# JunkyByte/easy_ViTPose

Hardware: AMD Instinct MI355X
Metric: persons_per_sec (higher is better)
Workload: dtype fp16; 1 GPU; ViTPose-B coco K=17, batch 256 x 256x192 crops per GPU (f32 input resident in HBM) -> (y,x,conf) keypoints in HBM; global_batch=256, weights=seeded random init (no checkpoint offline)

## Files before the change

easy_vitpose_amd/_capi.py:

```python
from __future__ import annotations

import ctypes as C
import os

LIB_PATH = os.path.join(os.path.dirname(os.path.abspath(__file__)), '_lib', 'libvitpose_hip.so')

VP_OK, VP_ERR_INVALID, VP_ERR_HIP, VP_ERR_STATE, VP_ERR_MISSING_TENSOR, VP_ERR_SHAPE = range(6)
VP_DTYPE_F16, VP_DTYPE_BF16, VP_DTYPE_FP8 = 0, 1, 2
VP_INPUT_F32_NCHW, VP_INPUT_U8_NHWC = 0, 1
VP_PROF_NAMES = ['gemm_proj', 'gemm_fc1', 'gemm_qkv', 'gemm_patch', 'gemm_deconv', 'gemm_final',
                 'attention', 'layernorm', 'im2col', 'decode', 'gemm_fc2']
VP_PROF_COUNT = len(VP_PROF_NAMES)
DTYPES = {'fp16': VP_DTYPE_F16, 'f16': VP_DTYPE_F16, 'bf16': VP_DTYPE_BF16, 'fp8': VP_DTYPE_FP8}

SYMBOLS = ['vp_abi_version', 'vp_create', 'vp_load_weights', 'vp_infer', 'vp_infer_device', 'vp_infer_device_stream', 'vp_host_alloc', 'vp_host_free',
           'vp_infer_submit', 'vp_infer_wait', 'vp_group_create', 'vp_group_size', 'vp_group_member', 'vp_group_load_weights', 'vp_group_infer',
           'vp_group_infer_allgather', 'vp_group_destroy', 'vp_group_last_error', 'vp_infer_frame', 'vp_infer_flip', 'vp_infer_heatmaps',
           'vp_infer_tokens', 'vp_decode_only', 'vp_stream', 'vp_synchronize', 'vp_set_profiling',
           'vp_reset_profile', 'vp_get_profile', 'vp_profile_kernel', 'vp_group_peer_access_missing', 'vp_destroy', 'vp_last_error',
           'vp_dbg_gemm', 'vp_dbg_attention', 'vp_dbg_layernorm', 'vp_dbg_deconv', 'vp_dbg_gemm_case', 'vp_dbg_crop_prep',
           'vp_dbg_group_plan', 'vp_dbg_group_trace', 'vp_dbg_gemm8_pick', 'vp_dbg_gemm2_pick', 'vp_dbg_splitk_pick', 'vp_dbg_run_batch', 'vp_dbg_fp8_gemm', 'vp_dbg_mx_gemm', 'vp_dbg_host_e4m3', 'vp_dbg_gemm_fp8_case', 'vp_dbg_qkvattn',
           'vp_expert_info', 'vp_set_expert', 'vp_infer_experts', 'vp_dbg_expert_tile', 'vp_infer_frames', 'vp_dbg_frame_plan',
           'vp_dbg_chunk_plan', 'vp_infer_boxes_stream', 'vp_dbg_box_geometry',
           'vp_set_flip_test', 'vp_clear_flip_test', 'vp_flip_test_enabled', 'vp_group_set_flip_test', 'vp_group_clear_flip_test',
           'vp_dbg_flip_partner', 'vp_dbg_flip_layout', 'vp_dbg_decode_flip',
           'vp_infer_experts_device_stream', 'vp_infer_frames_experts', 'vp_infer_boxes_experts_stream', 'vp_dbg_mix_plan', 'vp_dbg_decode_mix',
           'vp_set_flip_test_experts', 'vp_dbg_mix_plan_flip', 'vp_dbg_decode_flip_mix']


class HipExtensionMissing(RuntimeError):
    pass


class VpError(RuntimeError):
    def __init__(self, code: int, msg: str):
        super().__init__(f'[vitpose_hip status {code}] {msg}')
        self.code = code
        self.msg = msg


class vp_config(C.Structure):
    _fields_ = [('embed_dim', C.c_int32), ('depth', C.c_int32), ('num_heads', C.c_int32),
                ('num_keypoints', C.c_int32), ('dtype', C.c_int32), ('device_id', C.c_int32),
                ('max_batch', C.c_int32)]


class vp_tensor_desc(C.Structure):
    _fields_ = [('name', C.c_char_p), ('data', C.POINTER(C.c_float)), ('numel', C.c_int64)]


class vp_frame(C.Structure):
    _fields_ = [('data', C.c_void_p), ('h', C.c_int32), ('w', C.c_int32)]


class vp_profile(C.Structure):
    _fields_ = [('ms', C.c_double * VP_PROF_COUNT), ('flops', C.c_double * VP_PROF_COUNT),
                ('bytes', C.c_double * VP_PROF_COUNT), ('launches', C.c_int64 * VP_PROF_COUNT)]


_lib = None


def load_library():
    global _lib
    if _lib is not None:
        return _lib
    lib_path = os.environ.get('VP_HIP_LIB', LIB_PATH)
    if not os.path.exists(lib_path):
        raise HipExtensionMissing(
            f'{lib_path} not found. Build it with `python -m easy_vitpose_amd.build` '
            '(needs hipcc). There is no CPU fallback for the ViTPose path.')
    try:
        lib = C.CDLL(lib_path)
    except OSError as e:
        raise HipExtensionMissing(f'cannot load {lib_path}: {e}') from e
    H = C.c_void_p
    lib.vp_abi_version.restype = C.c_int
    lib.vp_create.argtypes = [C.POINTER(H), C.POINTER(vp_config)]
    lib.vp_load_weights.argtypes = [H, C.POINTER(vp_tensor_desc), C.c_int32]
    lib.vp_infer.argtypes = [H, C.c_void_p, C.c_int32, C.c_int32, C.c_void_p, C.c_void_p]
    lib.vp_infer_device.argtypes = [H, C.c_void_p, C.c_int32, C.c_int32, C.c_void_p, C.c_void_p, C.c_int32]
    lib.vp_infer_device_stream.argtypes = [H, C.c_void_p, C.c_int32, C.c_int32, C.c_void_p, C.c_void_p, C.c_void_p]
    lib.vp_host_alloc.argtypes = [C.c_size_t]
    lib.vp_host_alloc.restype = C.c_void_p
    lib.vp_host_free.argtypes = [C.c_void_p]
    lib.vp_host_free.restype = None
    lib.vp_infer_submit.argtypes = [H, C.c_void_p, C.c_int32, C.c_int32, C.c_void_p, C.c_void_p, C.POINTER(C.c_int32)]
    lib.vp_infer_wait.argtypes = [H, C.c_int32]
    lib.vp_group_create.argtypes = [C.POINTER(H), C.POINTER(vp_config), C.POINTER(C.c_int32), C.c_int32]
    lib.vp_group_size.argtypes = [H]
    lib.vp_group_member.argtypes = [H, C.c_int32]
    lib.vp_group_member.restype = C.c_void_p
    lib.vp_group_load_weights.argtypes = [H, C.POINTER(vp_tensor_desc), C.c_int32]
    lib.vp_group_infer.argtypes = [H, C.c_void_p, C.c_int32, C.c_int32, C.c_void_p, C.c_void_p]
    lib.vp_group_infer_allgather.argtypes = [H, C.c_void_p, C.c_int32, C.c_int32, C.c_void_p, C.POINTER(C.c_void_p), C.c_void_p]
    lib.vp_group_destroy.argtypes = [H]
    lib.vp_group_last_error.argtypes = [H]
    lib.vp_group_last_error.restype = C.c_char_p
    lib.vp_infer_frame.argtypes = [H, C.c_void_p, C.c_int32, C.c_int32, C.c_void_p, C.c_int32, C.c_void_p]
    lib.vp_infer_frames.argtypes = [H, C.POINTER(vp_frame), C.c_int32, C.c_int32, C.c_void_p, C.c_int32, C.c_void_p]
    lib.vp_dbg_frame_plan.argtypes = [C.POINTER(vp_frame), C.c_int32, C.c_void_p, C.c_int32, C.c_void_p]
    lib.vp_infer_boxes_stream.argtypes = [H, C.POINTER(vp_frame), C.c_int32, C.c_void_p, C.c_int32, C.c_void_p, C.c_int32, C.c_int32,
                                          C.c_void_p, C.c_void_p, C.c_void_p, C.c_void_p]
    lib.vp_dbg_box_geometry.argtypes = [C.c_void_p, C.c_int32, C.c_void_p, C.c_void_p, C.c_int32, C.c_int32, C.c_int32, C.c_void_p, C.c_void_p]
    lib.vp_dbg_crop_prep.argtypes = [C.c_int32, C.c_void_p, C.c_int32, C.c_int32, C.c_void_p, C.c_int32, C.c_void_p]
    lib.vp_infer_heatmaps.argtypes = [H, C.c_void_p, C.c_int32, C.c_int32, C.c_void_p]
    lib.vp_infer_tokens.argtypes = [H, C.c_void_p, C.c_int32, C.c_int32, C.c_void_p]
    lib.vp_decode_only.argtypes = [C.c_int32, C.c_void_p, C.c_int32, C.c_int32, C.c_void_p, C.c_void_p]
    lib.vp_stream.argtypes = [H]
    lib.vp_stream.restype = C.c_void_p
    lib.vp_synchronize.argtypes = [H]
    lib.vp_set_profiling.argtypes = [H, C.c_int32]
    lib.vp_reset_profile.argtypes = [H]
    lib.vp_get_profile.argtypes = [H, C.POINTER(vp_profile)]
    lib.vp_destroy.argtypes = [H]
    lib.vp_last_error.argtypes = [H]
    lib.vp_last_error.restype = C.c_char_p
    lib.vp_dbg_gemm.argtypes = [C.c_int32] * 6 + [C.c_void_p] * 5
    lib.vp_dbg_attention.argtypes = [C.c_int32] * 5 + [C.c_void_p] * 2
    lib.vp_dbg_layernorm.argtypes = [C.c_int32] * 4 + [C.c_void_p] * 5
    lib.vp_dbg_deconv.argtypes = [C.c_int32] * 6 + [C.c_void_p, C.POINTER(vp_tensor_desc), C.c_int32, C.c_void_p]
    lib.vp_infer_flip.argtypes = [C.c_void_p, C.c_void_p, C.c_int32, C.c_int32, C.c_void_p, C.c_void_p, C.c_int32, C.c_int32,
                                  C.c_void_p, C.c_void_p]
    lib.vp_dbg_gemm_case.argtypes = [C.c_int32] * 9 + [C.c_void_p] * 8
    if hasattr(lib, 'vp_dbg_gemm8_timeline'):
        lib.vp_dbg_gemm8_timeline.argtypes = [C.c_int32] * 9 + [C.POINTER(C.c_uint64), C.c_int32]
        lib.vp_dbg_gemm_timeline.argtypes = [C.c_int32] * 6 + [C.POINTER(C.c_uint64), C.c_int32]
        lib.vp_dbg_gemm8_timeline.restype = lib.vp_dbg_gemm_timeline.restype = C.c_int
        lib.vp_dbg_gemm_bench.argtypes = [C.c_int32] * 9 + [C.POINTER(C.c_float)]
        lib.vp_dbg_gemm_bench2.argtypes = [C.c_int32] * 10 + [C.POINTER(C.c_float)]
        lib.vp_dbg_gemm_compare.argtypes = [C.c_int32] * 13 + [C.POINTER(C.c_uint64), C.POINTER(C.c_double)]
        lib.vp_dbg_peak.argtypes = [C.c_int32, C.c_int32, C.POINTER(C.c_double)]
        for n_ in ('vp_dbg_gemm_bench', 'vp_dbg_gemm_bench2', 'vp_dbg_gemm_compare', 'vp_dbg_peak'):
            getattr(lib, n_).restype = C.c_int
    lib.vp_profile_kernel.argtypes = [H, C.c_int32, C.c_char_p, C.c_int32]
    lib.vp_group_peer_access_missing.argtypes = [H]
    lib.vp_dbg_group_plan.argtypes = [C.c_int32] * 3 + [C.c_void_p, C.c_void_p, C.c_int32]
    lib.vp_dbg_gemm8_pick.argtypes = [C.c_int32] * 4 + [C.c_void_p]
    lib.vp_dbg_gemm2_pick.argtypes = [C.c_int32] * 4 + [C.c_void_p]
    lib.vp_dbg_splitk_pick.argtypes = [C.c_int32] * 3 + [C.c_void_p]
    lib.vp_dbg_run_batch.argtypes = [C.c_int32] * 3
    lib.vp_dbg_group_trace.argtypes = [C.c_int32] * 3 + [C.c_void_p, C.c_int32]
    lib.vp_dbg_fp8_gemm.argtypes = [C.c_int32] * 4 + [C.c_void_p] * 7
    lib.vp_dbg_mx_gemm.argtypes = [C.c_int32] * 4 + [C.c_void_p] * 7
    lib.vp_dbg_host_e4m3.argtypes = [C.c_void_p, C.c_void_p, C.c_int64]
    lib.vp_dbg_gemm_fp8_case.argtypes = [C.c_int32] * 5 + [C.c_void_p] * 8
    lib.vp_expert_info.argtypes = [H, C.c_void_p, C.c_void_p, C.c_void_p]
    lib.vp_set_expert.argtypes = [H, C.c_int32]
    lib.vp_infer_experts.argtypes = [H, C.c_void_p, C.c_int32, C.c_int32, C.c_void_p, C.c_void_p, C.c_void_p]
    lib.vp_dbg_expert_tile.argtypes = [C.c_int32] * 4 + [C.c_void_p, C.c_int32]
    lib.vp_infer_experts_device_stream.argtypes = [H, C.c_void_p, C.c_int32, C.c_int32, C.c_void_p, C.c_void_p, C.c_void_p, C.c_void_p]
    lib.vp_infer_frames_experts.argtypes = [H, C.POINTER(vp_frame), C.c_int32, C.c_int32, C.c_void_p, C.c_int32, C.c_void_p, C.c_void_p]
    lib.vp_infer_boxes_experts_stream.argtypes = [H, C.POINTER(vp_frame), C.c_int32, C.c_void_p, C.c_int32, C.c_void_p, C.c_int32, C.c_int32,
                                                  C.c_void_p, C.c_void_p, C.c_void_p, C.c_void_p, C.c_void_p]
    lib.vp_dbg_mix_plan.argtypes = [C.c_void_p, C.c_int32, C.c_int32, C.c_int32] + [C.c_void_p] * 6
    lib.vp_dbg_decode_mix.argtypes = [C.c_int32, C.c_void_p, C.c_int32, C.c_int32, C.c_int32, C.c_void_p, C.c_void_p, C.c_void_p]
    lib.vp_dbg_chunk_plan.argtypes = [C.POINTER(vp_config), C.c_int32, C.c_void_p, C.c_int32]
    lib.vp_dbg_qkvattn.argtypes = [C.c_int32] * 5 + [C.c_void_p] * 4
    lib.vp_set_flip_test.argtypes = [H, C.c_void_p, C.c_int32, C.c_int32]
    lib.vp_clear_flip_test.argtypes = [H]
    lib.vp_flip_test_enabled.argtypes = [H]
    lib.vp_group_set_flip_test.argtypes = [H, C.c_void_p, C.c_int32, C.c_int32]
    lib.vp_group_clear_flip_test.argtypes = [H]
    lib.vp_set_flip_test_experts.argtypes = [H, C.c_void_p, C.c_void_p, C.c_int32]
    lib.vp_dbg_mix_plan_flip.argtypes = [C.c_void_p, C.c_int32, C.c_int32, C.c_int32] + [C.c_void_p] * 6
    lib.vp_dbg_decode_flip_mix.argtypes = [C.c_int32, C.c_void_p, C.c_int32, C.c_int32, C.c_int32, C.c_void_p, C.c_void_p, C.c_int32, C.c_int32, C.c_void_p, C.c_void_p]
    lib.vp_dbg_flip_partner.argtypes = [C.c_int32, C.c_void_p, C.c_int32, C.c_void_p]
    lib.vp_dbg_flip_layout.argtypes = [C.c_int32, C.c_int32, C.c_void_p, C.c_void_p]
    lib.vp_dbg_decode_flip.argtypes = [C.c_int32, C.c_void_p, C.c_int32, C.c_int32, C.c_void_p, C.c_int32, C.c_int32, C.c_void_p, C.c_void_p]
    for name in SYMBOLS:
        if name not in ('vp_stream', 'vp_last_error', 'vp_host_alloc', 'vp_host_free', 'vp_group_member', 'vp_group_last_error'):
            getattr(lib, name).restype = C.c_int
    _lib = lib
    return lib


def last_error(handle=None) -> str:
    lib = load_library()
    s = lib.vp_last_error(handle)
    return s.decode('utf-8', 'replace') if s else ''


def check(code: int, handle=None):
    if code != VP_OK:
        raise VpError(code, last_error(handle))
```

easy_vitpose_amd/csrc/api_internal.h:

```cpp
#pragma once
#include <hip/hip_runtime.h>

#include <algorithm>
#include <cmath>
#include <cstdio>
#include <cstdlib>
#include <cstring>
#include <string>
#include <unordered_map>
#include <vector>

#include "../../include/vitpose_hip.h"
#ifdef VP_TOOLS
#include "../../include/vitpose_hip_tools.h"
#endif
#include "kernels.h"
#include "mx8.h"

namespace vpi {

struct Block {
    float *ln1_g, *ln1_b, *ln2_g, *ln2_b;
    uint16_t *w_qkv, *w_proj, *w_fc1, *w_fc2;
    float *b_qkv, *b_proj, *b_fc1, *b_fc2;
    float *s_qkv, *s_fc1;
    uint16_t* w_qkvh = nullptr;
    float *b_qkvh = nullptr, *s_qkvh = nullptr;
    uint8_t *w_qkv8 = nullptr, *w_fc18 = nullptr, *w_fc28 = nullptr, *w_proj8 = nullptr;
    float *ws_qkv = nullptr, *ws_fc1 = nullptr, *ws_fc2 = nullptr, *ws_proj = nullptr;
};

struct Switches {
    int g8_stagger = 0;
    int gemm8_mask = 0x7;
    long g8_min_tiles = 448;
    bool persist_gemm = true;
    int order_mask = 8;
    bool blocked_hid = true;
    bool blocked_qkv = true;
    bool fuse_ln = true;
    bool fuse_qkv_attn = true;
    bool qa_min_set = false;
    long qa_min_tiles = 108;
    long qa80_min_tiles = 192;
    int qa80_group = 8;
    int attn_qsplit = 128;
    int g8_bm192 = 3;
    bool pad_batch = true;
    bool g8_cost_model = true;
    bool deconv_parity_fast = true;
    bool fuse_head = true;
    bool fp8_proj16 = false;
    int graph_max_n = 16;
    bool graph_null = true;
    int caller_stream_max_n = 16;
    bool fold_rule = true;
    int graph_max_n_stats = 8;
    bool splitk_on = true;
    int splitk_force[2][2] = {{0, 0}, {0, 0}};
    int gemm_variant[VP_PROF_COUNT] = {-1, -1, -1, -1, -1, -1, -1, -1, -1, -1, -1};
    int gemm_group_m[VP_PROF_COUNT] = {0};
    int fam_ablate[VP_PROF_COUNT] = {0};
};

}

namespace vpi {
struct MixPlan {
    int nb = 0;
    std::vector<int32_t> order, ids;
    std::vector<int> seg_e, seg_s;
    uint64_t pattern = 0;
};
}

struct vp_ctx {
    vp_config cfg;
    vpi::Switches sw;
    int D, L, heads, Kp, dtype, maxb;
    hipStream_t stream = nullptr;
    std::string err;
    bool loaded = false;
    std::vector<void*> allocs;
    uint16_t* w_patch = nullptr;
    float* pos = nullptr;
    std::vector<vpi::Block> blocks;
    float *lnf_g = nullptr, *lnf_b = nullptr;
    uint16_t *w_d1 = nullptr, *w_d2 = nullptr, *w_fin = nullptr;
    size_t fin_rows = 0;
    float *b_d1 = nullptr, *b_d2 = nullptr, *b_fin = nullptr, *b_zero = nullptr;
    uint16_t* zero = nullptr;
    void* in_stage = nullptr;
    int32_t* wh_stage = nullptr;
    float* x = nullptr;
    uint16_t *y = nullptr, *qkv = nullptr, *hid = nullptr, *d1 = nullptr, *d2 = nullptr;
    float *hm = nullptr, *kp = nullptr, *tok = nullptr;
    float* hm_keep = nullptr;
    int32_t* partner = nullptr;
    bool flip_on = false;
    int flip_shift = 0;
    uint32_t flip_gen = 0, flip_counter = 0;
    int32_t* flip_table = nullptr;
    std::vector<int32_t> flip_pairs;
    bool flip_ex = false;
    int32_t* flip_tables = nullptr;
    float *ln_part = nullptr, *rowstat = nullptr;
    bool fp8 = false;
    size_t Mp = 0;
    uint8_t *x8 = nullptr, *xs8 = nullptr, *hs8 = nullptr;
    uint8_t *y8 = nullptr, *ys8 = nullptr;
    struct Slot {
        void* in = nullptr; int32_t* wh = nullptr; float* kp = nullptr; hipEvent_t h2d = nullptr, done = nullptr, out = nullptr; bool busy = false;
        float* host_kp = nullptr; float* user_out = nullptr; size_t out_bytes = 0;
        char* host_in = nullptr; size_t host_in_cap = 0;
    };
    Slot slots[2];
    hipStream_t copy_stream = nullptr;
    hipStream_t d2h_stream = nullptr;
    int next_slot = 0;
    struct GraphKey {
        int n = 0, fmt = -1;
        const void* src = nullptr; const int32_t* wh = nullptr; float* out = nullptr;
        int expert = 0;
        const int32_t* post = nullptr;
        uint32_t flip = 0;
        uint64_t mix = 0;
        bool wide = false;
        bool operator==(const GraphKey& o) const {
            return n == o.n && fmt == o.fmt && src == o.src && wh == o.wh && out == o.out && expert == o.expert && post == o.post && flip == o.flip &&
                   mix == o.mix && wide == o.wide;
        }
    };
    struct GraphEntry { GraphKey key; hipGraphExec_t exec = nullptr; bool no_graph = false; };
    GraphEntry graphs[4];
    int graph_victim = 0;
    float* splitk_ws = nullptr;
    size_t splitk_rows = 0;
    hipEvent_t ev_in = nullptr, ev_out = nullptr;
    hipStream_t own_stream = nullptr;
    const void* last_stream_id = nullptr;
    bool foreign_pending = false;
    hipEvent_t ev_sw = nullptr;
    uint8_t* frame_stage = nullptr;
    size_t frame_cap = 0;
    vp::CropRec* crecs = nullptr;
    int32_t* box_aux = nullptr;
    struct Head { uint16_t *w_d1 = nullptr, *w_d2 = nullptr, *w_fin = nullptr; float *b_d1 = nullptr, *b_d2 = nullptr, *b_fin = nullptr; size_t fin_rows = 0; int K = 0; };
    int Kmax = 0;
    int n_experts = 0, part_features = 0, expert = 0;
    size_t fc2_w_stride = 0, fc2_b_stride = 0;
    std::vector<Head> ex_heads;
    int32_t* expert_ids = nullptr;
    void* mix_stage = nullptr;
    size_t mix_stage_cap = 0;
    const int32_t* mix_expert = nullptr;
    std::vector<int> mix_bounds;
    int32_t* mix_slot = nullptr;
    vp::MixRec* mix_recs = nullptr;
    vp::MixRecFlip* mix_recs_flip = nullptr;
    const vpi::MixPlan* mix = nullptr;
    vpi::MixPlan mix_host;
    std::vector<int32_t> mix_ks, mix_first, mix_k;
    uint32_t prof = 0;
    int gemm_ablate = 0;
    struct Ev { hipEvent_t a, b; int fam; double flops, bytes; };
    std::vector<Ev> evs;
    std::vector<std::pair<hipEvent_t, hipEvent_t>> ev_pool;
    vp_profile acc{};
    std::string kernel_desc[VP_PROF_COUNT];
};

namespace vpi {

extern thread_local std::string g_create_error;

int fail(vp_ctx* c, int code, const std::string& msg);
int need_weights(vp_ctx* c);
bool slots_busy(const vp_ctx* c);
int slots_idle(vp_ctx* c, const char* who);
int quiesce(vp_ctx* c);
inline size_t crop_bytes(int fmt) { return (size_t)3 * 256 * 192 * (fmt == VP_INPUT_F32_NCHW ? 4 : 1); }

#define HIPCHK(c, expr)                                                                         \
    do {                                                                                        \
        hipError_t e__ = (expr);                                                                \
        if (e__ != hipSuccess)                                                                  \
            return fail((c), VP_ERR_HIP, std::string(#expr) + ": " + hipGetErrorString(e__));   \
    } while (0)

template <class T> int dalloc(vp_ctx* c, T** p, size_t count) {
    void* q = nullptr;
    HIPCHK(c, hipMalloc(&q, count * sizeof(T) + 256));
    c->allocs.push_back(q);
    *p = (T*)q;
    return VP_OK;
}

uint16_t host_to_bits(float v, int dtype);
float host_from_bits(uint16_t h, int dtype);
size_t pad128(size_t n);
int upload_f32(vp_ctx* c, float** dst, const float* src, size_t n, size_t npad = 0);
int upload_mat(vp_ctx* c, uint16_t** dst, const float* src, size_t rows, size_t cols, size_t rows_pad);
int upload_final(vp_ctx* c, uint16_t** dst, const float* src, size_t kp, size_t cols, size_t* rows_phys);
int upload_ln_folded(vp_ctx* c, uint16_t** w_out, float** s_out, float** c_out, const float* W, const float* b,
                     const float* gamma, const float* beta, size_t N, size_t K);
int upload_fp8_rows(vp_ctx* c, uint8_t** w_out, float** ws_out, float** c_out, const float* W, const float* b, const float* gamma,
                    const float* beta, size_t N, size_t K);

struct Lookup {
    std::unordered_map<std::string, const vp_tensor_desc*> map;
    vp_ctx* c;
    int get(const std::string& name, int64_t numel, const float** out) {
        auto it = map.find(name);
        if (it == map.end()) return fail(c, VP_ERR_MISSING_TENSOR, "missing key in state dict: " + name);
        if (it->second->numel != numel || it->second->data == nullptr)
            return fail(c, VP_ERR_SHAPE, "size mismatch for " + name + ": expected " + std::to_string(numel) +
                                             " elements, got " + std::to_string(it->second->numel));
        *out = it->second->data;
        return VP_OK;
    }
    bool has(const std::string& name) const { return map.count(name) != 0; }
    int64_t numel(const std::string& name) const { auto it = map.find(name); return it == map.end() ? -1 : it->second->numel; }
};

size_t final_rows(size_t kp);
int pack_deconv(vp_ctx* c, Lookup& lk, int idx, int Cin, uint16_t** w_out, float** b_out, const std::string& head = "keypoint_head");
void use_expert(vp_ctx* c, int e);

int flip_partner_table(int K, const int32_t* pairs, int n_pairs, int32_t* partner, std::string* why);
inline const int32_t* flip_table_now(const vp_ctx* c) { return c->flip_ex ? c->flip_tables + (size_t)c->expert * c->Kmax : c->flip_table; }
bool prof_begin(vp_ctx* c, int fam, double flops, double bytes);
void prof_end(vp_ctx* c, bool on);
void prof_collect(vp_ctx* c);
void read_switches(Switches& s);
void apply_gemm_tuning(Switches& s);

int frame_plan(const vp_frame* frames, int n_frames, const int32_t* p9, int n, int32_t* bands, std::string* why);
int stage_frames(vp_ctx* c, const vp_frame* frames, int n_frames, bool on_device, const int32_t* p9, int n, const int32_t* bands,
                 std::vector<vp::CropRec>& recs);
int box_args(int n_frames, const int32_t* frame_hw, int hw_stride, int row_stride, int n, int pad, std::string* why);
constexpr uint64_t MIX_NO_GRAPH = ~(uint64_t)0;
int mix_check_ids(const int32_t* ids, int n, int n_experts, std::string* why);
void mix_plan(const int32_t* ids, int nb, int n_experts, MixPlan& p);
uint64_t mix_pattern(const std::vector<int>& seg_e, const std::vector<int>& seg_s, int n_experts);
void mix_records(const MixPlan& p, const int32_t* k_per_expert, int Kmax, int32_t* first, int32_t* K);
void mix_records_flip(const MixPlan& p, const int32_t* k_per_expert, int Kmax, int32_t* first, int32_t* K);
int submit_impl(vp_ctx* c, const void* crops, int32_t fmt, int32_t n, const int32_t* org_wh, float* out, int32_t* slot_out, bool stage_out);

#define LAUNCH(c, fam, flops, bytes, expr)   \
    do {                                     \
        const bool on__ = prof_begin((c), (fam), (flops), (bytes)); \
        hipError_t e__ = (expr);             \
        prof_end((c), on__);                 \
        if (e__ != hipSuccess)               \
            return fail((c), VP_ERR_HIP, std::string(#expr) + ": " + hipGetErrorString(e__)); \
    } while (0)

struct LnFuse {
    bool a_blocked = false, out_blocked = false, reverse = false;
    size_t plane = 0;
    float* stats_out = nullptr;
    const float* rowstat = nullptr;
    const float* ln_s = nullptr;
    const float* ln_part = nullptr;
    int ln_tiles = 0;
    int* tiles_out = nullptr;
};

constexpr int SPLITK_MAX_S = 8, SPLITK_MAX_CROPS = 32;
struct GemmPick { int variant = -1, group_m = 0, persist = 0, stagger = 0, splitk = 1, splitk_variant = 0; };
GemmPick resolve_gemm(const Switches& s, int fam, int epi, int M, int N, int K, bool ln_part = false, size_t splitk_rows = 0,
                      const std::vector<int>* mix_bounds = nullptr);
GemmPick resolve_gemm_fp8(int fam, int epi, int Mp, int N);
enum QkvPath { QKV_GEMM = 0, QKV_ATTN64 = 1, QKV_ATTN80 = 2 };
struct HeadPlan {
    bool fused = false;
    GemmPick deconv1, deconv2, final;
};
struct ChunkPlan {
    int n = 0;
    bool fold1 = false, fold2 = false;
    int qkv_path = QKV_GEMM;
    bool attn_qsplit = false;
    bool proj_fp8 = false;
    GemmPick gemm[VP_PROF_COUNT];
    HeadPlan head;
};
ChunkPlan plan_chunk(const Switches& s, int D, int heads, int max_batch, bool fp8, int n_in, size_t fin_rows, const std::vector<int>* mix_bounds = nullptr);
HeadPlan plan_head(const Switches& s, int D, int nh, size_t fin_rows);

int gemm(vp_ctx* c, int fam, int epi, const GemmPick& pk, const uint16_t* A, const uint16_t* W, const float* bias, void* out,
         const float* aux, int M, int N, int K, int ldo, int Hin = 0, int Win = 0, int Cin = 0, const LnFuse* ln = nullptr);
int gemm_fp8(vp_ctx* c, int fam, int epi, const GemmPick& pk, const uint8_t* A8, const uint8_t* a_scales, const uint8_t* W8, const float* w_scale, const float* bias,
             void* out, uint8_t* out_scales, const float* aux, int M, int N, int K, const LnFuse* ln);
struct FwdOpts {
    bool tokens = false;
    bool mirror = false;
    bool head = true;
    int twin_src = 0;
};
int forward_chunk(vp_ctx* c, const void* d_crops, int fmt, int n_in, const FwdOpts& o = FwdOpts());
int head_chunk(vp_ctx* c, const uint16_t* y, int nh, float* hm, const HeadPlan& hp);
int decode_chunk(vp_ctx* c, const int32_t* d_wh, float* d_out, int n, bool twin);
int chunk_cap(const vp_ctx* c);
int chunk_rows(const vp_ctx* c, int nb);
int forward_mode_chunk(vp_ctx* c, const void* d_src, int fmt, int nb);
int run_chunk(vp_ctx* c, const void* d_src, int fmt, int nb, const int32_t* d_wh, float* d_out, const int32_t* post = nullptr);

}
```

easy_vitpose_amd/csrc/debug_taps.hip:

```cpp
#include "dbg_util.h"

using namespace vpi;


extern "C" {

VP_API int vp_dbg_gemm(int32_t device, int32_t dtype, int32_t epi, int32_t M, int32_t N, int32_t K, const float* A,
                       const float* W, const float* bias, const float* aux, float* out) {
    if (epi < 0 || epi > 3 || M <= 0 || N <= 0 || K <= 0 || K % 64) return fail(nullptr, VP_ERR_INVALID, "bad gemm test shape");
    vp_ctx* c = dbg_ctx(device, dtype);
    if (!c) return VP_ERR_HIP;
    uint16_t *dA, *dW, *dO16 = nullptr;
    float *dB, *dAux = nullptr, *dO32 = nullptr;
    int rc;
    const size_t MN = (size_t)M * N;
    if ((rc = upload_mat(c, &dA, A, M, K, M))) return dbg_finish(c, rc);
    if ((rc = upload_mat(c, &dW, W, N, K, pad128(N)))) return dbg_finish(c, rc);
    if ((rc = upload_f32(c, &dB, bias, N, pad128(N)))) return dbg_finish(c, rc);
    if (epi >= 2) {
        if ((rc = upload_f32(c, &dAux, aux, epi == 2 ? MN : (size_t)192 * N))) return dbg_finish(c, rc);
        if ((rc = dalloc(c, &dO32, MN))) return dbg_finish(c, rc);
    } else if ((rc = dalloc(c, &dO16, MN))) return dbg_finish(c, rc);
    if ((rc = dalloc(c, &c->zero, (size_t)256))) return dbg_finish(c, rc);
    rc = gemm(c, 0, epi, resolve_gemm(c->sw, 0, epi, M, N, K), dA, dW, dB, epi >= 2 ? (void*)dO32 : (void*)dO16, dAux, M, N, K, N);
    if (!rc && hipDeviceSynchronize() != hipSuccess) rc = fail(c, VP_ERR_HIP, "gemm kernel failed");
    if (!rc) {
        if (epi >= 2) { if (hipMemcpy(out, dO32, MN * 4, hipMemcpyDeviceToHost) != hipSuccess) rc = fail(c, VP_ERR_HIP, "D2H"); }
        else rc = download16(c, dO16, out, MN);
    }
    return dbg_finish(c, rc);
}

VP_API int vp_dbg_attention(int32_t device, int32_t dtype, int32_t B, int32_t D, int32_t heads, const float* qkv, float* out) {
    vp_ctx* c = dbg_ctx(device, dtype);
    if (!c) return VP_ERR_HIP;
    uint16_t *dq, *dout;
    int rc;
    const size_t M = (size_t)B * 192;
    if ((rc = upload_mat(c, &dq, qkv, M, 3 * (size_t)D, M))) return dbg_finish(c, rc);
    if ((rc = dalloc(c, &dout, M * D))) return dbg_finish(c, rc);
    const char* qs = getenv("VP_ATTN_QSPLIT");
    hipError_t e = vp::attention_launch(c->dtype, dq, dout, B, D, heads, nullptr, (long)B * heads <= (qs ? atol(qs) : Switches{}.attn_qsplit));
    if (e == hipSuccess) e = hipDeviceSynchronize();
    if (e != hipSuccess) return dbg_finish(c, fail(c, VP_ERR_HIP, std::string("attention: ") + hipGetErrorString(e)));
    return dbg_finish(c, download16(c, dout, out, M * D));
}

VP_API int vp_dbg_qkvattn(int32_t device, int32_t dtype, int32_t npairs, int32_t D, int32_t heads, const float* x, const float* W, const float* bias, float* out) {
    if (npairs <= 0 || D <= 0 || heads <= 0 || !x || !W || !bias || !out) return fail(nullptr, VP_ERR_INVALID, "bad qkvattn test shape");
    vp_ctx* c = dbg_ctx(device, dtype);
    if (!c) return VP_ERR_HIP;
    const size_t M = (size_t)npairs * 384;
    uint16_t *dx, *dw, *dwh, *dy;
    float *db, *dbh, *ds, *dsh, *drow;
    int rc;
    std::vector<float> zeros(3 * (size_t)D, 0.f), row(2 * M);
    for (size_t m = 0; m < M; ++m) { row[2 * m] = 0.f; row[2 * m + 1] = 1.f; }
    if ((rc = upload_mat(c, &dx, x, M, D, M)) || (rc = upload_mat(c, &dw, W, 3 * (size_t)D, D, pad128(3 * (size_t)D))) || (rc = upload_f32(c, &db, bias, 3 * (size_t)D)) ||
        (rc = upload_f32(c, &ds, zeros.data(), 3 * (size_t)D)) || (rc = upload_f32(c, &drow, row.data(), 2 * M)) || (rc = dalloc(c, &dwh, 3 * (size_t)D * D)) ||
        (rc = dalloc(c, &dbh, 3 * (size_t)D)) || (rc = dalloc(c, &dsh, 3 * (size_t)D)) || (rc = dalloc(c, &dy, M * D)))
        return dbg_finish(c, rc);
    if (heads * 80 == D) {
        uint16_t* dwh80; float *dbh80, *dsh80;
        const size_t rows = (size_t)heads * 256;
        if ((rc = dalloc(c, &dwh80, rows * D)) || (rc = dalloc(c, &dbh80, rows)) || (rc = dalloc(c, &dsh80, rows))) return dbg_finish(c, rc);
        hipError_t e8 = vp::qkv_head_major80_launch(dw, db, ds, dwh80, dbh80, dsh80, D, D, heads, nullptr);
        vp::GemmArgs g80{};
        g80.A = dx; g80.W = dwh80; g80.bias = dbh80; g80.ln_s = dsh80; g80.rowstat = drow; g80.out = dy;
        g80.M = (int)M; g80.N = heads * 256; g80.K = D; g80.ldo = D; g80.w_rows = heads * 256; g80.variant = 18;
        g80.attn_scale_log2e = (1.0f / sqrtf(80.0f)) * 1.4426950408889634f;
        if (e8 == hipSuccess && !vp::gemm8_supported(vp::EPI_QKV_ATTN, g80, 256, 192)) return dbg_finish(c, fail(c, VP_ERR_INVALID, "shape not supported by the fused qkv + attention tile (head dim 80)"));
        if (e8 == hipSuccess) e8 = vp::gemm_launch(c->dtype, vp::EPI_QKV_ATTN, g80, nullptr);
        if (e8 == hipSuccess) e8 = hipDeviceSynchronize();
        if (e8 != hipSuccess) return dbg_finish(c, fail(c, VP_ERR_HIP, std::string("qkvattn (head dim 80): ") + hipGetErrorString(e8)));
        return dbg_finish(c, download16(c, dy, out, M * D));
    }
    hipError_t e = vp::qkv_head_major_launch(dw, db, ds, dwh, dbh, dsh, D, D, nullptr);
    vp::QkvAttnArgs qa{};
    qa.x_hi = dx; qa.wh = dwh; qa.bh = dbh; qa.sh = dsh; qa.rowstat = drow; qa.y = dy; qa.npairs = npairs; qa.ncrops = 2 * npairs; qa.heads = heads; qa.D = D;
    const float scale = 1.0f / sqrtf(64.0f);
    qa.scale_log2e = scale * 1.4426950408889634f;
    if (e == hipSuccess && !vp::qkvattn_supported(qa)) return dbg_finish(c, fail(c, VP_ERR_INVALID, "shape not supported by the fused qkv + attention kernel"));
    if (e == hipSuccess) e = vp::qkvattn_launch(c->dtype, qa, nullptr, nullptr, 0);
    if (e == hipSuccess) e = hipDeviceSynchronize();
    if (e != hipSuccess) return dbg_finish(c, fail(c, VP_ERR_HIP, std::string("qkvattn: ") + hipGetErrorString(e)));
    return dbg_finish(c, download16(c, dy, out, M * D));
}

VP_API int vp_dbg_layernorm(int32_t device, int32_t dtype, int32_t M, int32_t D, const float* x, const float* gamma,
                            const float* beta, float* out16, float* out32) {
    vp_ctx* c = dbg_ctx(device, dtype);
    if (!c) return VP_ERR_HIP;
    float *dx, *dg, *db, *d32;
    uint16_t* d16;
    int rc;
    const size_t MD = (size_t)M * D;
    if ((rc = upload_f32(c, &dx, x, MD)) || (rc = upload_f32(c, &dg, gamma, D)) || (rc = upload_f32(c, &db, beta, D)) ||
        (rc = dalloc(c, &d32, MD)) || (rc = dalloc(c, &d16, MD))) return dbg_finish(c, rc);
    hipError_t e = vp::layernorm_launch(c->dtype, dx, dg, db, d16, d32, M, D, nullptr);
    if (e == hipSuccess) e = hipDeviceSynchronize();
    if (e == hipSuccess) e = hipMemcpy(out32, d32, MD * 4, hipMemcpyDeviceToHost);
    if (e != hipSuccess) return dbg_finish(c, fail(c, VP_ERR_HIP, std::string("layernorm: ") + hipGetErrorString(e)));
    return dbg_finish(c, download16(c, d16, out16, MD));
}

VP_API int vp_dbg_deconv(int32_t device, int32_t dtype, int32_t B, int32_t Hin, int32_t Win, int32_t Cin, const float* x,
                         const vp_tensor_desc* tensors, int32_t n_tensors, float* out) {
    vp_ctx* c = dbg_ctx(device, dtype);
    if (!c) return VP_ERR_HIP;
    Lookup lk;
    lk.c = c;
    for (int i = 0; i < n_tensors; ++i) lk.map[tensors[i].name] = &tensors[i];
    uint16_t *dx, *dw, *dout;
    float* db;
    int rc;
    const size_t Min = (size_t)B * Hin * Win;
    if ((rc = pack_deconv(c, lk, 0, Cin, &dw, &db))) return dbg_finish(c, rc);
    if ((rc = upload_mat(c, &dx, x, Min, Cin, Min))) return dbg_finish(c, rc);
    if ((rc = dalloc(c, &dout, Min * 4 * 256))) return dbg_finish(c, rc);
    if ((rc = dalloc(c, &c->zero, (size_t)256))) return dbg_finish(c, rc);
    if (hipMemset(c->zero, 0, 512) != hipSuccess) return dbg_finish(c, fail(c, VP_ERR_HIP, "memset"));
    rc = gemm(c, 0, vp::EPI_DECONV, resolve_gemm(c->sw, 0, vp::EPI_DECONV, (int)Min, 256, 4 * Cin), dx, dw, db, dout, nullptr, (int)Min, 256, 4 * Cin, 256, Hin, Win, Cin);
    if (!rc && hipDeviceSynchronize() != hipSuccess) rc = fail(c, VP_ERR_HIP, "deconv kernel failed");
    if (!rc) rc = download16(c, dout, out, Min * 4 * 256);
    return dbg_finish(c, rc);
}


VP_API int vp_dbg_gemm_case(int32_t device, int32_t dtype, int32_t epi, int32_t variant, int32_t group_m, int32_t flags, int32_t M,
                            int32_t N, int32_t K, const float* A, const float* W, const float* bias, const float* aux, const float* rowstat,
                            const float* ln_s, float* out, float* stats) {
    if (M <= 0 || N <= 0 || K <= 0 || K % 64 || !A || !W || !bias || !out) return fail(nullptr, VP_ERR_INVALID, "bad gemm case");
    vp_ctx* c = dbg_ctx(device, dtype);
    if (!c) return VP_ERR_HIP;
    c->Kp = N;
    int r;
    const size_t MN = (size_t)M * N, wrows = pad128(N);
    const bool ablk = (flags & 4) != 0, oblk = (flags & 2) != 0;
    uint16_t *dA, *dW;
    float *dB, *dAux32 = nullptr, *dRow = nullptr, *dS = nullptr, *dStats = nullptr;
    uint16_t* dAux16 = nullptr;
    void* dOut = nullptr;
    {
        std::vector<uint16_t> ha((size_t)M * K);
        for (size_t m = 0; m < (size_t)M; ++m)
            for (size_t k = 0; k < (size_t)K; ++k) {
                const size_t dst = ablk ? ((((m >> 6) * (K >> 6) + (k >> 6)) << 12) + ((m & 63) << 6) + (k & 63)) : m * K + k;
                ha[dst] = host_to_bits(A[m * K + k], c->dtype);
            }
        if ((r = dalloc(c, &dA, (size_t)M * K))) return dbg_finish(c, r);
        if (hipMemcpy(dA, ha.data(), ha.size() * 2, hipMemcpyHostToDevice) != hipSuccess) return dbg_finish(c, fail(c, VP_ERR_HIP, "H2D"));
    }
    size_t fin_rows = 0;
    if (epi == vp::EPI_HEATMAP) { if ((r = upload_final(c, &dW, W, N, K, &fin_rows))) return dbg_finish(c, r); }
    else if ((r = upload_mat(c, &dW, W, N, K, wrows))) return dbg_finish(c, r);
    if ((r = upload_f32(c, &dB, bias, N, wrows)) || (r = dalloc(c, &c->zero, (size_t)256))) return dbg_finish(c, r);
    vp::GemmArgs g{};
    g.A = dA; g.W = dW; g.bias = dB; g.M = M; g.N = N; g.K = K; g.ldo = N; g.zero = c->zero; g.Kp = N;
    g.w_rows = (int)wrows; g.variant = variant; g.group_m = group_m;
    g.persist = (flags & 1) != 0; g.out_blocked = oblk; g.a_blocked = ablk; g.reverse = (flags & 8) != 0;
    if (rowstat && ln_s) {
        if ((r = upload_f32(c, &dRow, rowstat, (size_t)M * 2)) || (r = upload_f32(c, &dS, ln_s, N, wrows))) return dbg_finish(c, r);
        g.rowstat = dRow; g.ln_s = dS;
    }
    size_t out_bytes = 0;
    const bool prod = epi == vp::EPI_BIAS_RESID_LN || epi == vp::EPI_POS_LN;
    if (epi == vp::EPI_BIAS || epi == vp::EPI_BIAS_GELU) out_bytes = MN * 2;
    else if (epi == vp::EPI_BIAS_RESID || epi == vp::EPI_POS || prod) out_bytes = MN * 4;
    else if (epi == vp::EPI_HEATMAP) { out_bytes = MN * 4; g.N = (int)fin_rows; g.ldo = 0; g.w_rows = (int)pad128(fin_rows); }
    else return dbg_finish(c, fail(c, VP_ERR_INVALID, "unsupported epilogue"));
    if (epi == vp::EPI_BIAS_RESID || epi == vp::EPI_POS || epi == vp::EPI_POS_LN) {
        if (!aux) return dbg_finish(c, fail(c, VP_ERR_INVALID, "aux required"));
        if ((r = upload_f32(c, &dAux32, aux, epi == vp::EPI_BIAS_RESID ? MN : (size_t)192 * N))) return dbg_finish(c, r);
        g.aux = dAux32;
    }
    if (epi == vp::EPI_BIAS_RESID_LN) {
        if (!aux) return dbg_finish(c, fail(c, VP_ERR_INVALID, "aux required"));
        std::vector<uint16_t> hp(2 * MN);
        for (size_t i = 0; i < MN; ++i) {
            const uint16_t hi = host_to_bits(aux[i], c->dtype);
            hp[i] = hi;
            hp[MN + i] = host_to_bits(aux[i] - host_from_bits(hi, c->dtype), c->dtype);
        }
        if ((r = dalloc(c, &dAux16, 2 * MN))) return dbg_finish(c, r);
        if (hipMemcpy(dAux16, hp.data(), hp.size() * 2, hipMemcpyHostToDevice) != hipSuccess) return dbg_finish(c, fail(c, VP_ERR_HIP, "H2D"));
        g.aux = (const float*)dAux16;
    }
    if (prod) {
        g.plane = MN;
        if ((r = dalloc(c, &dStats, (size_t)M * (N / 64) * 2))) return dbg_finish(c, r);
        g.stats_out = dStats;
    }
    char* o;
    if ((r = dalloc(c, &o, out_bytes))) return dbg_finish(c, r);
    dOut = o;
    hipMemset(dOut, 0xff, out_bytes);
    g.out = dOut;
    const int splitk = (flags >> 8) & 15;
    hipError_t e;
    if (splitk > 1) {
        if (epi != vp::EPI_BIAS_RESID_LN) return dbg_finish(c, fail(c, VP_ERR_INVALID, "split-K is a residual-GEMM path (epi 6)"));
        float* ws = nullptr;
        if ((r = dalloc(c, &ws, (size_t)splitk * MN))) return dbg_finish(c, r);
        hipMemset(ws, 0xff, (size_t)splitk * MN * 4);
        vp::GemmArgs p = g;
        p.out = ws; p.aux = nullptr; p.bias = nullptr; p.stats_out = nullptr; p.plane = 0; p.splitk = splitk; p.persist = 0;
        e = vp::gemm_launch(c->dtype, vp::EPI_PARTIAL, p, nullptr);
        if (e == hipSuccess) e = vp::splitk_reduce_launch(c->dtype, ws, splitk, dB, dAux16, MN, dStats, M, N, nullptr);
        dOut = dAux16;
    } else {
        e = vp::gemm_launch(c->dtype, epi, g, nullptr);
    }
    if (e == hipSuccess) e = hipDeviceSynchronize();
    if (e != hipSuccess) return dbg_finish(c, fail(c, VP_ERR_HIP, std::string("gemm case: ") + hipGetErrorString(e)));
    if (epi == vp::EPI_BIAS || epi == vp::EPI_BIAS_GELU) {
        std::vector<float> t(MN);
        if ((r = download16(c, (const uint16_t*)dOut, t.data(), MN))) return dbg_finish(c, r);
        for (size_t m = 0; m < (size_t)M; ++m)
            for (size_t n = 0; n < (size_t)N; ++n) {
                const size_t src = oblk ? ((((m >> 6) * ((size_t)N >> 6) + (n >> 6)) << 12) + ((m & 63) << 6) + (n & 63)) : m * N + n;
                out[m * N + n] = t[src];
            }
    } else if (prod) {
        std::vector<float> hi(MN), lo(MN);
        if ((r = download16(c, (const uint16_t*)dOut, hi.data(), MN)) || (r = download16(c, (const uint16_t*)dOut + MN, lo.data(), MN))) return dbg_finish(c, r);
        for (size_t i = 0; i < MN; ++i) out[i] = hi[i] + lo[i];
        if (stats && hipMemcpy(stats, dStats, (size_t)M * (N / 64) * 8, hipMemcpyDeviceToHost) != hipSuccess) return dbg_finish(c, fail(c, VP_ERR_HIP, "D2H"));
    } else {
        if (hipMemcpy(out, dOut, out_bytes, hipMemcpyDeviceToHost) != hipSuccess) return dbg_finish(c, fail(c, VP_ERR_HIP, "D2H"));
    }
    return dbg_finish(c, VP_OK);
}

VP_API int vp_dbg_crop_prep(int32_t device, const uint8_t* frame, int32_t fh, int32_t fw, const int32_t* crop_params, int32_t n, uint8_t* out) {
    if (!frame || !crop_params || !out || n <= 0 || fh <= 0 || fw <= 0) return fail(nullptr, VP_ERR_INVALID, "bad argument");
    const vp_frame fr{frame, fh, fw};
    std::vector<int32_t> p9((size_t)n * 9, 0);
    for (int i = 0; i < n; ++i) std::memcpy(&p9[9 * (size_t)i + 1], crop_params + 8 * (size_t)i, 32);
// ... 145 lines not shown
```

easy_vitpose_amd/csrc/forward.hip:

```cpp
#include "api_internal.h"
#include "tiles.h"

using namespace vpi;

namespace vpi {

static void note_kernel(vp_ctx* c, int fam, const char* desc) {
    if (desc[0] && c->kernel_desc[fam] != desc) c->kernel_desc[fam] = desc;
}

int gemm(vp_ctx* c, int fam, int epi, const GemmPick& pk, const uint16_t* A, const uint16_t* W, const float* bias, void* out,
         const float* aux, int M, int N, int K, int ldo, int Hin, int Win, int Cin, const LnFuse* ln) {
    vp::GemmArgs g{};
    g.A = A; g.W = W; g.bias = bias; g.out = out; g.aux = aux;
    g.M = M; g.N = N; g.K = K; g.ldo = ldo;
    g.Hin = Hin; g.Win = Win; g.Cin = Cin; g.zero = c->zero; g.Kp = c->Kp;
    g.w_rows = (int)pad128((size_t)N);
    g.variant = pk.variant; g.group_m = pk.group_m; g.persist = pk.persist; g.stagger = pk.stagger;
    g.ablate = c->gemm_ablate | c->sw.fam_ablate[fam];
    g.parity_fast = c->sw.deconv_parity_fast;
    if (c->mix_expert && fam == VP_PROF_GEMM_FC2) g.expert = c->mix_expert;
    if (ln) {
        g.a_blocked = ln->a_blocked; g.out_blocked = ln->out_blocked; g.reverse = ln->reverse;
        g.plane = ln->plane; g.stats_out = ln->stats_out; g.rowstat = ln->rowstat; g.ln_s = ln->ln_s;
        g.ln_part = ln->ln_part; g.ln_tiles = ln->ln_tiles; g.ln_inv_d = 1.0f / (float)K;
        if (ln->tiles_out) *ln->tiles_out = N / 64;
    }
    if (epi == vp::EPI_DECONV_FINAL) { g.W2 = c->w_fin; g.bias2 = c->b_fin; g.out2 = (float*)out; g.out = nullptr; }
    const bool deconv = epi == vp::EPI_DECONV || epi == vp::EPI_DECONV_FINAL;
    const double par = deconv ? 4.0 : 1.0;
    const double Nalg = (epi == vp::EPI_HEATMAP) ? (double)c->Kp : (double)N;
    double flops = 2.0 * M * Nalg * K * par;
    const bool resid = epi == vp::EPI_BIAS_RESID || epi == vp::EPI_BIAS_RESID_LN;
    const bool f32out = resid || epi == vp::EPI_POS || epi == vp::EPI_POS_LN || epi == vp::EPI_HEATMAP;
    const double out_b = f32out ? 4.0 : 2.0;
    double bytes = 2.0 * M * (double)(deconv ? Cin : K) + 2.0 * N * (double)K * par + out_b * M * Nalg * par;
    if (epi == vp::EPI_DECONV_FINAL) {
        flops += 2.0 * M * par * (double)c->Kp * N;
        bytes += (4.0 * c->Kp - out_b * N) * M * par + 2.0 * c->fin_rows * N;
    }
    if (resid) bytes += 4.0 * M * (double)N;
    if (epi == vp::EPI_BIAS_RESID_LN || epi == vp::EPI_POS_LN) bytes += 8.0 * M * (double)(N / 64);
    char desc[192];
    desc[0] = 0;
    g.desc = desc; g.desc_cap = (int)sizeof(desc);
    if (pk.splitk > 1) {
        if (out != (void*)aux || (size_t)M > c->splitk_rows || !c->splitk_ws) return fail(c, VP_ERR_INVALID, "split-K: a residual GEMM in place within the workspace only");
        vp::GemmArgs p = g;
        p.out = c->splitk_ws; p.aux = nullptr; p.bias = nullptr; p.stats_out = nullptr; p.plane = 0;
        p.variant = pk.splitk_variant; p.group_m = 0; p.splitk = pk.splitk; p.ldo = N; p.persist = 0;
        LAUNCH(c, fam, flops, bytes, vp::gemm_launch(c->dtype, vp::EPI_PARTIAL, p, c->stream));
        if (desc[0]) {
            char d2[224];
            snprintf(d2, sizeof(d2), "%s x split-K %d + splitk_reduce_kernel", desc, pk.splitk);
            note_kernel(c, fam, d2);
        }
        LAUNCH(c, fam, 0.0, 0.0, vp::splitk_reduce_launch(c->dtype, c->splitk_ws, pk.splitk, bias, (uint16_t*)out, g.plane, g.stats_out, M, N, c->stream));
        return VP_OK;
    }
    LAUNCH(c, fam, flops, bytes, vp::gemm_launch(c->dtype, epi, g, c->stream));
    note_kernel(c, fam, desc);
    return VP_OK;
}

int gemm_fp8(vp_ctx* c, int fam, int epi, const GemmPick& pk, const uint8_t* A8, const uint8_t* a_scales, const uint8_t* W8, const float* w_scale, const float* bias,
             void* out, uint8_t* out_scales, const float* aux, int M, int N, int K, const LnFuse* ln) {
    vp::GemmArgs g{};
    g.A = (const uint16_t*)A8; g.W = (const uint16_t*)W8; g.bias = bias; g.out = out; g.aux = aux;
    g.M = M; g.N = N; g.K = K; g.ldo = N;
    g.a_scales = a_scales; g.w_scale = w_scale; g.out_scales = out_scales;
    g.w_rows = (int)pad128((size_t)N);
    if (ln) {
        g.out_blocked = ln->out_blocked; g.reverse = ln->reverse;
        g.plane = ln->plane; g.stats_out = ln->stats_out;
        if (ln->tiles_out) *ln->tiles_out = N / 64;
    }
    const int bn = vp::tile8_bn(pk.variant);
    g.group_m = pk.group_m;
    if (!vp::gemm8f_supported(epi, g, bn))
        return fail(c, VP_ERR_SHAPE, "fp8 mode: GEMM shape " + std::to_string(M) + " x " + std::to_string(N) + " x " + std::to_string(K) + " not supported by the MXFP8 kernel");
    const double flops = 2.0 * M * (double)N * K;
    double bytes = 1.0 * M * (double)K + M * (double)(K / 32) + 1.0 * N * (double)K;
    bytes += epi == vp::EPI_BIAS ? 2.0 * M * (double)N : epi == vp::EPI_BIAS_GELU ? (1.0 + 1.0 / 32) * M * (double)N : 8.0 * M * (double)N + 8.0 * M * (double)(N / 64);
    char desc[192];
    desc[0] = 0;
    g.desc = desc; g.desc_cap = (int)sizeof(desc);
    LAUNCH(c, fam, flops, bytes, vp::gemm8f_launch(epi, g, bn, c->stream));
    note_kernel(c, fam, desc);
    return VP_OK;
}

static const uint16_t* fc2_w(const vp_ctx* c, const vpi::Block& b) { return c->mix_expert ? b.w_fc2 : b.w_fc2 + (size_t)c->expert * c->fc2_w_stride; }
static const float* fc2_b(const vp_ctx* c, const vpi::Block& b) { return c->mix_expert ? b.b_fc2 : b.b_fc2 + (size_t)c->expert * c->fc2_b_stride; }

int forward_chunk(vp_ctx* c, const void* d_crops, int fmt, int n_in, const FwdOpts& o) {
    const int D = c->D;
    const ChunkPlan pl = plan_chunk(c->sw, D, c->heads, c->maxb, c->fp8, n_in, c->fin_rows, c->mix_expert ? &c->mix_bounds : nullptr);
    const GemmPick* pk = pl.gemm;
    const int n = pl.n;
    const int M = n * 192;
    const double in_b = (fmt == VP_INPUT_F32_NCHW ? 4.0 : 1.0) * n_in * 3.0 * 256 * 192;
    if (o.twin_src) LAUNCH(c, VP_PROF_IM2COL, 0.0, 0.5 * in_b + 2.0 * M * 768, vp::im2col_twin_launch(c->dtype, d_crops, fmt, c->hid, n, o.twin_src, c->stream));
    else LAUNCH(c, VP_PROF_IM2COL, 0.0, in_b + 2.0 * M * 768, vp::im2col_launch(c->dtype, d_crops, fmt, c->hid, n, c->stream, o.mirror, n_in));
    int rc;
    size_t plane = 0;
    const bool qkv_blocked = c->sw.blocked_qkv && D / c->heads == 64;
    auto attention = [&](uint16_t* out, double bytes, uint8_t* mx_scales) -> int {
        LAUNCH(c, VP_PROF_ATTN, 4.0 * 192 * 192 * (double)D * n, bytes,
               vp::attention_launch(c->dtype, c->qkv, out, n, D, c->heads, c->stream, pl.attn_qsplit, qkv_blocked ? 1 : 0, mx_scales));
        return VP_OK;
    };
    if (c->fp8) {
        const int Mp = (int)std::max<size_t>((size_t)(M + 255) / 256 * 256, 512);
        plane = c->Mp * (size_t)D;
        uint16_t* xh = (uint16_t*)c->x;
        int tiles = 0;
        LnFuse prod; prod.plane = plane; prod.stats_out = c->ln_part; prod.tiles_out = &tiles;
        auto quant = [&]() -> int {
            LAUNCH(c, VP_PROF_LAYERNORM, 0.0, 8.0 * M * tiles + 2.0 * M * D + (1.0 + 1.0 / 32) * Mp * (double)D,
                   vp::ln_quant_launch(c->dtype, xh, c->ln_part, tiles, c->x8, c->xs8, M, Mp, D, c->stream));
            return VP_OK;
        };
        if ((rc = gemm(c, VP_PROF_GEMM_PATCH, vp::EPI_POS_LN, pk[VP_PROF_GEMM_PATCH], c->hid, c->w_patch, c->b_zero, c->x, c->pos, M, D, 768, D, 0, 0, 0, &prod))) return rc;
        for (int l = 0; l < c->L; ++l) {
            const Block& b = c->blocks[l];
            if ((rc = quant())) return rc;
            LnFuse cq; cq.out_blocked = qkv_blocked;
            if ((rc = gemm_fp8(c, VP_PROF_GEMM_QKV, vp::EPI_BIAS, pk[VP_PROF_GEMM_QKV], c->x8, c->xs8, b.w_qkv8, b.ws_qkv, b.b_qkv, c->qkv, nullptr, nullptr, Mp, 3 * D, D, &cq))) return rc;
            LnFuse pp = prod;
            if (pl.proj_fp8) {
                if ((rc = attention((uint16_t*)c->y8, 7.0 * M * D, c->ys8))) return rc;
                if ((rc = gemm_fp8(c, VP_PROF_GEMM_PROJ, vp::EPI_BIAS_RESID_LN, pk[VP_PROF_GEMM_PROJ], c->y8, c->ys8, b.w_proj8, b.ws_proj, b.b_proj, c->x, nullptr, c->x, Mp, D, D, &pp))) return rc;
            } else {
                if ((rc = attention(c->y, 8.0 * M * D, nullptr))) return rc;
                if ((rc = gemm(c, VP_PROF_GEMM_PROJ, vp::EPI_BIAS_RESID_LN, pk[VP_PROF_GEMM_PROJ], c->y, b.w_proj, b.b_proj, c->x, c->x, M, D, D, D, 0, 0, 0, &pp))) return rc;
            }
            if ((rc = quant())) return rc;
            if ((rc = gemm_fp8(c, VP_PROF_GEMM_FC1, vp::EPI_BIAS_GELU, pk[VP_PROF_GEMM_FC1], c->x8, c->xs8, b.w_fc18, b.ws_fc1, b.b_fc1, c->hid, c->hs8, nullptr, Mp, 4 * D, D, nullptr))) return rc;
            LnFuse p2 = prod;
            if ((rc = gemm_fp8(c, VP_PROF_GEMM_FC2, vp::EPI_BIAS_RESID_LN, pk[VP_PROF_GEMM_FC2], (const uint8_t*)c->hid, c->hs8, b.w_fc28, b.ws_fc2, b.b_fc2, c->x, nullptr, c->x, Mp, D, 4 * D, &p2))) return rc;
        }
    } else if (c->sw.fuse_ln) {
        plane = (size_t)M * D;
        uint16_t* xh = (uint16_t*)c->x;
        int tiles = 0;
        LnFuse prod; prod.plane = plane; prod.stats_out = c->ln_part; prod.tiles_out = &tiles;
        auto finalize = [&](bool folded) -> int {
            if (folded) return VP_OK;
            LAUNCH(c, VP_PROF_LAYERNORM, 0.0, 8.0 * M * tiles + 8.0 * M, vp::ln_finalize_launch(c->ln_part, c->rowstat, M, tiles, D, c->stream));
            return VP_OK;
        };
        const double qkv_attn_flops = 2.0 * M * 3.0 * D * D + 4.0 * 192 * 192 * (double)D * n, qkv_attn_bytes = 2.0 * M * D + 2.0 * 3 * D * (double)D + 2.0 * M * D;
        if ((rc = gemm(c, VP_PROF_GEMM_PATCH, vp::EPI_POS_LN, pk[VP_PROF_GEMM_PATCH], c->hid, c->w_patch, c->b_zero, c->x, c->pos, M, D, 768, D, 0, 0, 0, &prod))) return rc;
        if ((rc = finalize(pl.fold1))) return rc;
        for (int l = 0; l < c->L; ++l) {
            const Block& b = c->blocks[l];
            if (pl.qkv_path == QKV_ATTN80) {
                vp::GemmArgs g80{};
                g80.A = xh; g80.W = b.w_qkvh; g80.bias = b.b_qkvh; g80.ln_s = b.s_qkvh; g80.rowstat = c->rowstat; g80.out = c->y;
                g80.M = M; g80.N = c->heads * 256; g80.K = D; g80.ldo = D; g80.w_rows = c->heads * 256; g80.variant = 18;
                g80.group_m = c->sw.qa80_group;
                g80.attn_scale_log2e = (1.0f / sqrtf(80.0f)) * 1.4426950408889634f;
                g80.ablate = c->gemm_ablate | c->sw.fam_ablate[VP_PROF_GEMM_QKV];
                char desc[192];
                desc[0] = 0;
                g80.desc = desc; g80.desc_cap = (int)sizeof(desc);
                LAUNCH(c, VP_PROF_GEMM_QKV, qkv_attn_flops, qkv_attn_bytes, vp::gemm_launch(c->dtype, vp::EPI_QKV_ATTN, g80, c->stream));
                note_kernel(c, VP_PROF_GEMM_QKV, desc);
            } else if (pl.qkv_path == QKV_ATTN64) {
                vp::QkvAttnArgs qa{};
                qa.x_hi = xh; qa.wh = b.w_qkvh; qa.bh = b.b_qkvh; qa.sh = b.s_qkvh; qa.rowstat = c->rowstat; qa.y = c->y;
                qa.npairs = (n + 1) / 2; qa.ncrops = n; qa.heads = c->heads; qa.D = D;
                qa.scale_log2e = (1.0f / sqrtf(64.0f)) * 1.4426950408889634f;
                char desc[96];
                desc[0] = 0;
                LAUNCH(c, VP_PROF_GEMM_QKV, qkv_attn_flops, qkv_attn_bytes, vp::qkvattn_launch(c->dtype, qa, c->stream, desc, (int)sizeof(desc)));
                note_kernel(c, VP_PROF_GEMM_QKV, desc);
            } else {
                LnFuse cq; cq.rowstat = c->rowstat; cq.ln_s = b.s_qkv; cq.reverse = (c->sw.order_mask & 1) != 0; cq.out_blocked = qkv_blocked;
                if (pl.fold1) { cq.rowstat = nullptr; cq.ln_part = c->ln_part; cq.ln_tiles = D / 64; }
                if ((rc = gemm(c, VP_PROF_GEMM_QKV, vp::EPI_BIAS, pk[VP_PROF_GEMM_QKV], xh, b.w_qkv, b.b_qkv, c->qkv, nullptr, M, 3 * D, D, 3 * D, 0, 0, 0, &cq))) return rc;
                if ((rc = attention(c->y, 8.0 * M * D, nullptr))) return rc;
            }
            LnFuse pp = prod; pp.reverse = (c->sw.order_mask & 2) != 0;
            if ((rc = gemm(c, VP_PROF_GEMM_PROJ, vp::EPI_BIAS_RESID_LN, pk[VP_PROF_GEMM_PROJ], c->y, b.w_proj, b.b_proj, c->x, c->x, M, D, D, D, 0, 0, 0, &pp))) return rc;
            if ((rc = finalize(pl.fold2))) return rc;
            LnFuse c1; c1.rowstat = c->rowstat; c1.ln_s = b.s_fc1; c1.out_blocked = c->sw.blocked_hid; c1.reverse = (c->sw.order_mask & 4) != 0;
            if (pl.fold2) { c1.rowstat = nullptr; c1.ln_part = c->ln_part; c1.ln_tiles = D / 64; }
            if ((rc = gemm(c, VP_PROF_GEMM_FC1, vp::EPI_BIAS_GELU, pk[VP_PROF_GEMM_FC1], xh, b.w_fc1, b.b_fc1, c->hid, nullptr, M, 4 * D, D, 4 * D, 0, 0, 0, &c1))) return rc;
            LnFuse p2 = prod; p2.a_blocked = c->sw.blocked_hid; p2.reverse = (c->sw.order_mask & 8) != 0;
            if ((rc = gemm(c, VP_PROF_GEMM_FC2, vp::EPI_BIAS_RESID_LN, pk[VP_PROF_GEMM_FC2], c->hid, fc2_w(c, b), fc2_b(c, b), c->x, c->x, M, D, 4 * D, D, 0, 0, 0, &p2))) return rc;
            if (l + 1 < c->L && (rc = finalize(pl.fold1))) return rc;
        }
    } else {
    if ((rc = gemm(c, VP_PROF_GEMM_PATCH, vp::EPI_POS, pk[VP_PROF_GEMM_PATCH], c->hid, c->w_patch, c->b_zero, c->x, c->pos, M, D, 768, D))) return rc;
    for (int l = 0; l < c->L; ++l) {
        const Block& b = c->blocks[l];
        LAUNCH(c, VP_PROF_LAYERNORM, 0.0, 6.0 * M * D,
               vp::layernorm_launch(c->dtype, c->x, b.ln1_g, b.ln1_b, c->y, nullptr, M, D, c->stream));
        LnFuse q0; q0.out_blocked = qkv_blocked;
        if ((rc = gemm(c, VP_PROF_GEMM_QKV, vp::EPI_BIAS, pk[VP_PROF_GEMM_QKV], c->y, b.w_qkv, b.b_qkv, c->qkv, nullptr, M, 3 * D, D, 3 * D, 0, 0, 0, &q0))) return rc;
        if ((rc = attention(c->y, 8.0 * M * D, nullptr))) return rc;
        if ((rc = gemm(c, VP_PROF_GEMM_PROJ, vp::EPI_BIAS_RESID, pk[VP_PROF_GEMM_PROJ], c->y, b.w_proj, b.b_proj, c->x, c->x, M, D, D, D))) return rc;
        LAUNCH(c, VP_PROF_LAYERNORM, 0.0, 6.0 * M * D,
               vp::layernorm_launch(c->dtype, c->x, b.ln2_g, b.ln2_b, c->y, nullptr, M, D, c->stream));
        if ((rc = gemm(c, VP_PROF_GEMM_FC1, vp::EPI_BIAS_GELU, pk[VP_PROF_GEMM_FC1], c->y, b.w_fc1, b.b_fc1, c->hid, nullptr, M, 4 * D, D, 4 * D))) return rc;
        if ((rc = gemm(c, VP_PROF_GEMM_FC2, vp::EPI_BIAS_RESID, pk[VP_PROF_GEMM_FC2], c->hid, fc2_w(c, b), fc2_b(c, b), c->x, c->x, M, D, 4 * D, D))) return rc;
    }
    }
    const int nh = n_in, Mh = nh * 192;
    LAUNCH(c, VP_PROF_LAYERNORM, 0.0, 6.0 * Mh * D,
           vp::layernorm_launch(c->dtype, c->x, c->lnf_g, c->lnf_b, c->y, o.tokens ? c->tok : nullptr, Mh, D, c->stream, plane));
    return o.head ? head_chunk(c, c->y, nh, c->hm, pl.head) : VP_OK;
}

int head_chunk(vp_ctx* c, const uint16_t* y, int nh, float* hm, const HeadPlan& hp) {
    const int D = c->D;
    int rc;
    if ((rc = gemm(c, VP_PROF_GEMM_DECONV, vp::EPI_DECONV, hp.deconv1, y, c->w_d1, c->b_d1, c->d1, nullptr, nh * 192, 256, 4 * D, 256, 16, 12, D))) return rc;
    if (hp.fused) {
        return gemm(c, VP_PROF_GEMM_DECONV, vp::EPI_DECONV_FINAL, hp.deconv2, c->d1, c->w_d2, c->b_d2, hm, nullptr, nh * 768, 256, 1024, 256, 32, 24, 256);
    }
    if ((rc = gemm(c, VP_PROF_GEMM_DECONV, vp::EPI_DECONV, hp.deconv2, c->d1, c->w_d2, c->b_d2, c->d2, nullptr, nh * 768, 256, 1024, 256, 32, 24, 256))) return rc;
    if ((rc = gemm(c, VP_PROF_GEMM_FINAL, vp::EPI_HEATMAP, hp.final, c->d2, c->w_fin, c->b_fin, hm, nullptr, nh * 3072, (int)c->fin_rows, 256, 0))) return rc;
    return VP_OK;
}

int decode_chunk(vp_ctx* c, const int32_t* d_wh, float* d_out, int n, bool twin) {
    if (twin)
        LAUNCH(c, VP_PROF_DECODE, 0.0, 8.0 * n * c->Kp * 3072.0 + 12.0 * n * c->Kp,
               vp::decode_flip_launch(c->hm, flip_table_now(c), c->flip_shift, d_wh, d_out, n, c->Kp, c->stream));
    else
        LAUNCH(c, VP_PROF_DECODE, 0.0, 4.0 * n * c->Kp * 3072.0 + 12.0 * n * c->Kp,
               vp::decode_launch(c->hm, d_wh, d_out, n, c->Kp, c->stream));
    return VP_OK;
}

int chunk_cap(const vp_ctx* c) { return c->flip_on ? c->maxb / 2 : c->maxb; }
int chunk_rows(const vp_ctx* c, int nb) { return c->flip_on ? 2 * nb : nb; }

int forward_mode_chunk(vp_ctx* c, const void* d_src, int fmt, int nb) {
    FwdOpts o;
    if (c->flip_on) o.twin_src = nb;
    return forward_chunk(c, d_src, fmt, chunk_rows(c, nb), o);
}

using GraphKey = vp_ctx::GraphKey;
using GraphEntry = vp_ctx::GraphEntry;

static int offsets_chunk(vp_ctx* c, const int32_t* aux, float* d_out, int n) {
    LAUNCH(c, VP_PROF_DECODE, 0.0, 24.0 * n * c->Kp + 16.0 * n, vp::box_offsets_launch(aux, d_out, n, c->Kp, c->stream));
    return VP_OK;
}

static int mix_chunk_body(vp_ctx* c, const GraphKey& k) {
    const MixPlan& m = *c->mix;
    const int nseg = (int)m.seg_e.size(), D = c->D;
    const int tw = c->flip_ex ? 2 : 1;
    int rc;
    if (nseg == 1) {
        use_expert(c, m.seg_e[0]);
        if ((rc = forward_mode_chunk(c, k.src, k.fmt, k.n))) return rc;
    } else {
        const void* src = k.src;
        if (src != c->in_stage) {
            const size_t B = (size_t)((c->maxb + 3) / 4 * 4);
            HIPCHK(c, vp::gather_crops_launch(src, c->in_stage, c->expert_ids + B, k.n, crop_bytes(k.fmt), c->stream));
            src = c->in_stage;
        }
        FwdOpts encoder_only;
        encoder_only.head = false;
        if (tw == 2) encoder_only.twin_src = k.n;
        c->mix_expert = c->expert_ids;
        c->mix_bounds.clear();
        for (int s = 1; s < nseg; ++s) c->mix_bounds.push_back(tw * m.seg_s[s]);
        rc = forward_chunk(c, src, k.fmt, tw * k.n, encoder_only);
        c->mix_expert = nullptr;
        c->mix_bounds.clear();
        if (rc) return rc;
        for (int s = 0; s < nseg; ++s) {
            const int s0 = tw * m.seg_s[s], cnt = tw * (m.seg_s[s + 1] - m.seg_s[s]);
            use_expert(c, m.seg_e[s]);
            if ((rc = head_chunk(c, c->y + (size_t)s0 * 192 * D, cnt, c->hm + (size_t)s0 * c->Kmax * 3072, plan_head(c->sw, D, cnt, c->fin_rows)))) return rc;
        }
    }
    if (tw == 2)
        LAUNCH(c, VP_PROF_DECODE, 0.0, 8.0 * k.n * c->Kmax * 3072.0 + 12.0 * k.n * c->Kmax,
               vp::decode_flip_mix_launch(c->hm, c->mix_recs_flip, c->flip_tables, c->flip_shift, k.wh, k.out, k.n, c->Kmax, c->stream));
    else
        LAUNCH(c, VP_PROF_DECODE, 0.0, 4.0 * k.n * c->Kmax * 3072.0 + 12.0 * k.n * c->Kmax,
               vp::decode_mix_launch(c->hm, c->mix_recs, k.wh, k.out, k.n, c->Kmax, c->stream));
    if (k.post) LAUNCH(c, VP_PROF_DECODE, 0.0, 24.0 * k.n * c->Kmax + 16.0 * k.n, vp::box_offsets_launch(k.post, k.out, k.n, c->Kmax, c->stream, c->mix_slot, c->mix_recs));
    return VP_OK;
}

static int chunk_body(vp_ctx* c, const GraphKey& k) {
    int rc;
    if (k.wide) return mix_chunk_body(c, k);
    if ((rc = forward_mode_chunk(c, k.src, k.fmt, k.n))) return rc;
    if ((rc = decode_chunk(c, k.wh, k.out, k.n, c->flip_on))) return rc;
    return k.post ? offsets_chunk(c, k.post, k.out, k.n) : VP_OK;
}

static GraphEntry* graph_lookup(vp_ctx* c, const GraphKey& key) {
    for (auto& g : c->graphs)
        if (g.key == key) return &g;
    return nullptr;
}

static int graph_remember(vp_ctx* c, const GraphKey& key) {
    GraphEntry& ge = c->graphs[c->graph_victim++ & 3];
    if (ge.exec) {
        HIPCHK(c, hipStreamSynchronize(c->stream));
        hipGraphExecDestroy(ge.exec);
    }
    ge = GraphEntry{};
    ge.key = key;
    return VP_OK;
}

static hipGraphExec_t graph_capture(vp_ctx* c, const GraphKey& key) {
    hipStream_t target = c->stream;
    c->stream = c->own_stream;
    hipGraph_t graph = nullptr;
    hipGraphExec_t exec = nullptr;
    hipError_t e = hipStreamBeginCapture(c->stream, hipStreamCaptureModeThreadLocal);
    if (e == hipSuccess) {
        const int rc = chunk_body(c, key);
        e = hipStreamEndCapture(c->stream, &graph);
        if (rc) c->err.clear();
        if (rc || (e == hipSuccess && !graph)) e = hipErrorUnknown;
        if (e == hipSuccess) e = hipGraphInstantiate(&exec, graph, nullptr, nullptr, 0);
        if (graph) hipGraphDestroy(graph);
    }
    c->stream = target;
    return e == hipSuccess ? exec : nullptr;
}

static int graph_give_up(vp_ctx* c, GraphEntry* ge) {
    (void)hipGetLastError();
    if (ge->exec) hipGraphExecDestroy(ge->exec);
    ge->exec = nullptr;
    ge->no_graph = true;
    return chunk_body(c, ge->key);
}
// ... 29 lines not shown
```

easy_vitpose_amd/csrc/gemm8.hip:

```cpp
#include <cstdio>

#include <cstdlib>
#include "gemm8_common.h"
#ifndef VP_G8_RESD
#define VP_G8_RESD 1
#endif
#ifndef VP_G8_RESD192
#define VP_G8_RESD192 1
#endif



namespace vp {

namespace {
__device__ __forceinline__ u32x2 lds_tr16(const char* p) {
    typedef __attribute__((__vector_size__(4 * sizeof(__fp16)))) __fp16 h4;
    typedef __attribute__((address_space(3))) h4* lds_h4;
    const h4 v = __builtin_amdgcn_ds_read_tr16_b64_v4f16((lds_h4)(p));
    return __builtin_bit_cast(u32x2, v);
}
}

template <class T, int EPI, class C, bool EXPERT = false>
// ... 51 lines not shown
                if (which == 0) { if (!wr) glds16(src + xrow(64 + wave * 8), dst + 8192); }
                else { if (wr) glds16(src + xrow(C::XR + (wave + 4) * 8), dst + C::XH + 4096); }
            }
        } else if (which == 2) {
            const char* src = wb + ((size_t)wu0 * K + (size_t)kt * 64) * 2 + vw;
            glds16(src, dst + C::OFF_W0);
            glds16(src + (size_t)32 * C::TI * K * 2, dst + C::OFF_W0 + 8192);
        } else {
            const char* src = wb + ((size_t)wu1 * K + (size_t)kt * 64) * 2 + vw;
            glds16(src, dst + C::OFF_W1);
            if (C::NW1 == 2) glds16(src + (size_t)32 * C::TI * K * 2, dst + C::OFF_W1 + 8192);
        }
    };

    const int frow = lane & 15, fg = lane >> 4;
    const int foff = frow * 128 + ((fg ^ ((frow >> 1) & 7)) << 4);
    const int xoff = wr * (C::XR / 2) * 128 + foff;
    const int w0off = wc * 32 * 128 + foff;
    const int w1off = wc * 16 * C::NF1 * 128 + foff;

    constexpr int MJ = C::MJ, TJ = C::TJ;
    f32x4 acc[C::TI][TJ];
    u32x4 xs[MJ][2], fa[2][2], fb[2][2];
    auto rowJ = [](int J) { return (J / MJ) * C::XR + (J % MJ) * 16; };

    auto zero_acc = [&]() {
#pragma unroll
        for (int f = 0; f < C::TI; ++f)
#pragma unroll
            for (int j = 0; j < TJ; ++j) acc[f][j] = f32x4{0.f, 0.f, 0.f, 0.f};
    };

#ifndef VP_G8_ABL
#define VP_G8_ABL 0
#endif
#define KBAR() do { if (!(VP_G8_ABL & 2)) bar(); } while (0)
#if (VP_G8_ABL & 16)
    unsigned long long sec[12];
#pragma unroll
    for (int i = 0; i < 12; ++i) sec[i] = 0;
    bool stamp_now = false;
#define SEC(i) do { if (stamp_now) sec[i] = __builtin_readcyclecounter(); } while (0)
#else
#define SEC(i) do { } while (0)
#endif
    constexpr int NKEEP = C::NKEEP;
    auto wait_lb = [&]() {
        if constexpr (C::BM == 256) wait_vm<C::INFLIGHT>();
        else { if (wr) wait_vm<3 + C::NW1>(); else wait_vm<4 + C::NW1>(); }
    };
    auto ktile = [&](auto Bc, auto Mc, int kA, int kB, bool swB, int nm0, int nn0) {
        constexpr int B = decltype(Bc)::value;
        constexpr int MODE = decltype(Mc)::value;
        const char* sb = smem + B * C::BUF;
        SEC(0);
#pragma unroll
        for (int p = 0; p < 2; ++p)
#pragma unroll
            for (int kk = 0; kk < 2; ++kk) if (MODE == 1 || !(VP_G8_ABL & 1)) fa[p][kk] = *(const u32x4*)(sb + C::OFF_W0 + ((w0off + p * 2048) ^ (kk << 6)));
#pragma unroll
        for (int p = 0; p < C::NF1; ++p)
#pragma unroll
            for (int kk = 0; kk < 2; ++kk) if (MODE == 1 || !(VP_G8_ABL & 1)) fb[p][kk] = *(const u32x4*)(sb + C::OFF_W1 + ((w1off + p * 2048) ^ (kk << 6)));
#pragma unroll
        for (int j = 0; j < MJ; ++j)
#pragma unroll
            for (int kk = 0; kk < 2; ++kk) if (MODE == 1 || !(VP_G8_ABL & 1)) xs[j][kk] = *(const u32x4*)(sb + C::OFF_X0 + ((xoff + j * 2048) ^ (kk << 6)));
        __builtin_amdgcn_sched_barrier(0);
        SEC(1);
        if constexpr (MODE != 4) issue(1, B ^ 1, kA);
        SEC(2);
        if constexpr (MODE == 4) wait_vm<0>();
        else if constexpr (MODE != 1) wait_vm<NKEEP>();
        wait_lgkm<0>();
        SEC(3);
        KBAR();
        SEC(4);
        __builtin_amdgcn_s_setprio(1);
#pragma unroll
        for (int kk = 0; kk < 2; ++kk) {
#pragma unroll
            for (int p = 0; p < 2; ++p)
#pragma unroll
                for (int j = 0; j < MJ; ++j) if (!(VP_G8_ABL & 4)) acc[p][j] = mfma16<T>(fa[p][kk], xs[j][kk], acc[p][j]);
#pragma unroll
            for (int p = 0; p < C::NF1; ++p)
#pragma unroll
                for (int j = 0; j < MJ; ++j) if (!(VP_G8_ABL & 4)) acc[2 + p][j] = mfma16<T>(fb[p][kk], xs[j][kk], acc[2 + p][j]);
        }
        __builtin_amdgcn_s_setprio(0);
        SEC(5);
        KBAR();
        SEC(6);
#pragma unroll
        for (int j = 0; j < MJ; ++j)
#pragma unroll
            for (int kk = 0; kk < 2; ++kk) if (!(VP_G8_ABL & 1)) xs[j][kk] = *(const u32x4*)(sb + C::OFF_X1 + ((xoff + j * 2048) ^ (kk << 6)));
        __builtin_amdgcn_sched_barrier(0);
        if constexpr (MODE < 3) {
            if (swB) set_tile(nm0, nn0);
            issue(2, B, kB);
            issue(0, B, kB);
            issue(3, B, kB);
        }
        SEC(7);
        if constexpr (MODE == 2) wait_lb();
        else if constexpr (MODE == 3) { if (wr) wait_vm<2>(); else wait_vm<1>(); }
        else if constexpr (MODE < 3) wait_vm<NKEEP>();
        wait_lgkm<0>();
        SEC(8);
        KBAR();
        SEC(9);
        __builtin_amdgcn_s_setprio(1);
#pragma unroll
        for (int kk = 0; kk < 2; ++kk) {
#pragma unroll
            for (int p = 0; p < 2; ++p)
#pragma unroll
                for (int j = 0; j < MJ; ++j) if (!(VP_G8_ABL & 4)) acc[p][MJ + j] = mfma16<T>(fa[p][kk], xs[j][kk], acc[p][MJ + j]);
#pragma unroll
            for (int p = 0; p < C::NF1; ++p)
#pragma unroll
                for (int j = 0; j < MJ; ++j) if (!(VP_G8_ABL & 4)) acc[2 + p][MJ + j] = mfma16<T>(fb[p][kk], xs[j][kk], acc[2 + p][MJ + j]);
        }
        __builtin_amdgcn_s_setprio(0);
        SEC(10);
        KBAR();
        SEC(11);
    };
#undef KBAR
#undef SEC
    using M0 = std::integral_constant<int, 0>;
    using M1 = std::integral_constant<int, 1>;
    using M2 = std::integral_constant<int, 2>;
    using M3 = std::integral_constant<int, 3>;
    using M4 = std::integral_constant<int, 4>;
    using B0 = std::integral_constant<int, 0>;
    using B1 = std::integral_constant<int, 1>;
    auto ring_start = [&]() {
        issue(2, 0, 0, true); issue(0, 0, 0, true); issue(3, 0, 0, true); issue(1, 0, 0, true);
        issue(2, 1, 1, true); issue(0, 1, 1, true); issue(3, 1, 1, true);
        wait_lb();
        bar();
        if (wr) bar();
    };

    if (VP_STAGGER(g) > 0) {
        const bool short_list = (tw.cnt - tw.j0 + tw.nloc - 1) / tw.nloc < (tw.cnt + tw.nloc - 1) / tw.nloc;
        const int n = (VP_STAGGER(g) >= 300) ? (short_list ? VP_STAGGER(g) - 300 : 0)
                    : (VP_STAGGER(g) >= 200) ? ((blockIdx.x >> 3) & 1) * (VP_STAGGER(g) - 200)
                    : (VP_STAGGER(g) >= 100) ? (blockIdx.x >> 3) * (VP_STAGGER(g) - 100) : (blockIdx.x & 7) * VP_STAGGER(g);
        for (int i = 0; i < n; ++i) __builtin_amdgcn_s_sleep(16);
    }
    int t = tw.j0, m0, n0;
    tw.origin(t, g.reverse, C::BM, C::BN, m0, n0);
    set_tile(m0, n0);
    ring_start();

    for (;;) {
        zero_acc();
        const float* tbias = g.bias;
        if constexpr (EXPERT) tbias += (size_t)g.expert[m0 / 192] * g.w_rows;
        const bool has_next = t + tw.nloc < tw.cnt;
        int nm0 = m0, nn0 = n0;
        if (has_next) tw.origin(t + tw.nloc, g.reverse, C::BM, C::BN, nm0, nn0);
        const bool tl = (VP_ABLATE(g) & 32) != 0;
        unsigned long long ts0 = 0, ts1 = 0;
        if (tl) ts0 = __builtin_readcyclecounter();
        ktile(B0{}, M1{}, 1, 2, false, 0, 0);
        ktile(B1{}, M0{}, 2, 3, false, 0, 0);
        for (int kt = 2; kt < nk - 2; kt += 2) {
#if (VP_G8_ABL & 16)
            stamp_now = tl && kt == 4 && (t - tw.j0) / tw.nloc == 1;
#endif
            ktile(B0{}, M0{}, kt + 1, kt + 2, false, 0, 0);
#if (VP_G8_ABL & 16)
            stamp_now = false;
#endif
            ktile(B1{}, M0{}, kt + 2, kt + 3, false, 0, 0);
        }
        if constexpr (QKVA) {
            ktile(B0{}, M3{}, nk - 1, 0, false, 0, 0);
            ktile(B1{}, M4{}, 0, 0, false, 0, 0);
        } else {
            ktile(B0{}, M0{}, nk - 1, 0, true, nm0, nn0);
            ktile(B1{}, M2{}, 0, 1, false, 0, 0);
        }
        if (tl) ts1 = __builtin_readcyclecounter();

        int frow_e = frow, fg_e = fg;
        asm volatile("" : "+v"(frow_e), "+v"(fg_e));
        if constexpr (!DRAIN) { if (!wr) bar(); }
        if constexpr (QKVA) {
            constexpr int HD = 80, QSTR = HD * 2, VSUB = 192 * 32, DT = HD / 16, KS = 3;
            constexpr int Q_OFF = 160 * 1024 - 2 * 192 * QSTR - DT * VSUB, K_OFF = Q_OFF + 192 * QSTR, V_OFF = K_OFF + 192 * QSTR;
            static_assert(Q_OFF >= C::BUF + C::XH && Q_OFF % 16 == 0, "q / k / v behind ring buffer 0 and the X0 slot of buffer 1");
            const int nbq = n0 + wc * 64 + fg_e * 8;
            const int mrow = m0 + wr * (C::XR / 2) + frow_e;
            f32x4 b4[4], s4[4];
            float2 st[TJ];
#pragma unroll
            for (int f = 0; f < 4; ++f) {
                b4[f] = *(const f32x4*)(g.bias + nbq + (f >> 1) * 32 + (f & 1) * 4);
                s4[f] = *(const f32x4*)(g.ln_s + nbq + (f >> 1) * 32 + (f & 1) * 4);
            }
#pragma unroll
            for (int J = 0; J < TJ; ++J) st[J] = *(const float2*)(g.rowstat + 2 * (size_t)(mrow + rowJ(J)));
            wait_vm<0>();
            if (!wr) bar();
            __syncthreads();
            if (has_next) {
                set_tile(nm0, nn0);
                issue(2, 0, 0, true); issue(0, 0, 0, true); issue(3, 0, 0, true); issue(1, 0, 0, true);
                issue(0, 1, 1, true);
            }
            if (!(VP_ABLATE(g) & 2)) {
                const int lrow = wr * (C::XR / 2) + frow_e;
#pragma unroll
                for (int fp = 0; fp < 2; ++fp) {
                    const int c0 = wc * 64 + fp * 32 + fg_e * 8;
                    const int seg = (c0 >= HD) + (c0 >= 2 * HD) + (c0 >= 3 * HD);
                    const int d0 = c0 - seg * HD;
                    const int rmul = seg < 2 ? QSTR : 32;
                    const int base = seg < 2 ? (seg ? K_OFF : Q_OFF) + d0 * 2 : V_OFF + (d0 >> 4) * VSUB + (d0 & 15) * 2;
#pragma unroll
                    for (int J = 0; J < TJ; ++J) {
                        u32x4 o;
#pragma unroll
                        for (int h = 0; h < 2; ++h) {
                            const int f = 2 * fp + h;
                            f32x4 v;
#pragma unroll
                            for (int e = 0; e < 4; ++e) v[e] = ln_fold(acc[f][J][e], st[J].x, s4[f][e], st[J].y, b4[f][e]);
                            o[2 * h] = pack2<T>(v[0], v[1]);
                            o[2 * h + 1] = pack2<T>(v[2], v[3]);
                        }
                        if (seg < 3) *(u32x4*)(smem + base + (lrow + rowJ(J)) * rmul) = o;
                    }
                }
            }
            wait_lgkm<0>();
            bar();
            if (!(VP_ABLATE(g) & 16)) {
                const char* Qs = smem + Q_OFF;
                const char* Ks = smem + K_OFF;
                const char* Vs = smem + V_OFF;
                int fr = frow, fgq = fg;
                asm volatile("" : "+v"(fr), "+v"(fgq));
                const bool live2 = fgq < 2;
                const int slot2 = (live2 ? 8 + fgq : 6 + fgq) * 16;
                const char* vfrag = Vs + (fgq * 4 + (fr >> 2)) * 32 + (fr & 3) * 8;
                uint16_t* ybase = (uint16_t*)g.out + (size_t)m0 * K + (n0 >> 8) * HD;
                const float scale_log2e = g.attn_scale_log2e;
                for (int pass = 0; pass < 2; ++pass) {
                    const int qt = pass * 8 + wave;
                    if (qt >= 12) break;
                    u32x4 qf[KS];
                    {
                        const char* qrow = Qs + (qt * 16 + fr) * QSTR;
                        qf[0] = *(const u32x4*)(qrow + fgq * 16);
                        qf[1] = *(const u32x4*)(qrow + (4 + fgq) * 16);
                        qf[2] = *(const u32x4*)(qrow + slot2);
                        if (!live2) qf[2] = u32x4{0u, 0u, 0u, 0u};
                    }
                    f32x4 sc[12];
#pragma unroll
                    for (int kt = 0; kt < 12; ++kt) sc[kt] = f32x4{0.f, 0.f, 0.f, 0.f};
#pragma unroll
                    for (int kt = 0; kt < 12; ++kt) {
                        const char* krow = Ks + (kt * 16 + fr) * QSTR;
                        const u32x4 k0 = *(const u32x4*)(krow + fgq * 16);
                        const u32x4 k1 = *(const u32x4*)(krow + (4 + fgq) * 16);
                        const u32x4 k2 = *(const u32x4*)(krow + slot2);
                        sc[kt] = mfma16<T>(k0, qf[0], sc[kt]);
                        sc[kt] = mfma16<T>(k1, qf[1], sc[kt]);
                        sc[kt] = mfma16<T>(k2, qf[2], sc[kt]);
                    }
                    float mx = -3.0e38f;
#pragma unroll
                    for (int kt = 0; kt < 12; ++kt)
#pragma unroll
                        for (int r = 0; r < 4; ++r) mx = fmaxf(mx, sc[kt][r]);
                    mx = fmaxf(mx, __shfl_xor(mx, 16, 64));
                    mx = fmaxf(mx, __shfl_xor(mx, 32, 64));
                    float l = 0.f;
                    const float mb = mx * scale_log2e;
#pragma unroll
                    for (int kt = 0; kt < 12; ++kt)
#pragma unroll
                        for (int r = 0; r < 4; ++r) {
                            const float pv = softmax_p(sc[kt][r], scale_log2e, mb);
                            sc[kt][r] = pv;
                            l += pv;
                        }
                    l += __shfl_xor(l, 16, 64);
                    l += __shfl_xor(l, 32, 64);
                    const float inv_l = 1.0f / l;
                    u32x4 pf[6];
#pragma unroll
                    for (int kb = 0; kb < 6; ++kb) {
                        pf[kb][0] = pack2_nosat<T>(sc[2 * kb][0], sc[2 * kb][1]);
                        pf[kb][1] = pack2_nosat<T>(sc[2 * kb][2], sc[2 * kb][3]);
                        pf[kb][2] = pack2_nosat<T>(sc[2 * kb + 1][0], sc[2 * kb + 1][1]);
                        pf[kb][3] = pack2_nosat<T>(sc[2 * kb + 1][2], sc[2 * kb + 1][3]);
                    }
                    uint16_t* dst = ybase + (size_t)(qt * 16 + fr) * K;
#pragma unroll
                    for (int dp = 0; dp < DT; ++dp) {
                        f32x4 o = f32x4{0.f, 0.f, 0.f, 0.f};
#pragma unroll
                        for (int kb = 0; kb < 6; ++kb) {
                            const char* vp_ = vfrag + dp * VSUB + kb * 1024;
                            const u32x2 lo = lds_tr16(vp_);
                            const u32x2 hi = lds_tr16(vp_ + 512);
                            o = mfma16<T>(u32x4{lo[0], lo[1], hi[0], hi[1]}, pf[kb], o);
                        }
                        u32x2 w;
                        w[0] = pack2_nosat<T>(o[0] * inv_l, o[1] * inv_l);
                        w[1] = pack2_nosat<T>(o[2] * inv_l, o[3] * inv_l);
                        if (!(VP_ABLATE(g) & 8)) *(u32x2*)(dst + dp * 16 + fgq * 4) = w;
                    }
                }
            }
            wait_lgkm<0>();
            bar();
            if (has_next) {
                issue(2, 1, 1, true); issue(3, 1, 1, true);
                if (VP_ABLATE(g) & (8 | 16)) { if (wr) wait_vm<5>(); else wait_vm<6>(); }
                else { if (wr) wait_vm<10>(); else wait_vm<16>(); }
                bar();
                if (wr) bar();
            }
        } else if constexpr (RESID && !RESID_LDS) {
            const int nb = n0 + wc * 64 + fg_e * 16;
            const int mrow = m0 + wr * (C::XR / 2) + frow_e;
            uint16_t* out_hi = (uint16_t*)g.out;
            uint16_t* out_lo = out_hi + g.plane;
            const uint16_t* aux_hi = (const uint16_t*)g.aux;
            const uint16_t* aux_lo = aux_hi + g.plane;
            f32x4 bias4[4];
#pragma unroll
            for (int f = 0; f < 4; ++f) bias4[f] = *(const f32x4*)(tbias + nb + f * 4);
            const bool store = !(VP_ABLATE(g) & 8);
            const int gran = g.N >> 6;
            constexpr int RD = C::BM == 192 ? VP_G8_RESD192 : VP_G8_RESD;
            u32x4 res[RD + 1][4];
            auto load_res = [&](int J, u32x4(&r)[4]) {
                const size_t o = (size_t)(mrow + rowJ(J)) * g.ldo + nb;
                r[0] = *(const u32x4*)(aux_hi + o);
                r[1] = *(const u32x4*)(aux_hi + o + 8);
                r[2] = *(const u32x4*)(aux_lo + o);
                r[3] = *(const u32x4*)(aux_lo + o + 8);
            };
#pragma unroll
            for (int J = 0; J < RD; ++J) load_res(J, res[J]);
#pragma unroll
            for (int J = 0; J < TJ; ++J) {
                if (J + RD < TJ) load_res(J + RD, res[(J + RD) % (RD + 1)]);
                const u32x4(&r)[4] = res[J % (RD + 1)];
                const int m = mrow + rowJ(J);
                const size_t o = (size_t)m * g.ldo + nb;
                float v[16];
#pragma unroll
                for (int f = 0; f < 4; ++f) {
                    const f32x4 st = acc[f][J] + bias4[f];
#pragma unroll
                    for (int e = 0; e < 4; ++e) {
                        const int c = f * 4 + e;
                        const uint32_t wh = r[c >> 3][(c & 7) >> 1], wl = r[2 + (c >> 3)][(c & 7) >> 1];
                        const int sh = (c & 1) * 16;
                        v[c] = st[e] + (from_bits<T>((uint16_t)(wh >> sh)) + from_bits<T>((uint16_t)(wl >> sh)));
                    }
                }
                u32x4 oh[2], ol[2];
#pragma unroll
                for (int c = 0; c < 16; c += 2) {
                    uint32_t h_, l_;
                    split_planes2<T>(v[c], v[c + 1], h_, l_);
                    oh[c >> 3][(c & 7) >> 1] = h_;
                    ol[c >> 3][(c & 7) >> 1] = l_;
                }
                if (store) {
                    *(u32x4*)(out_hi + o) = oh[0];
                    *(u32x4*)(out_hi + o + 8) = oh[1];
                    *(u32x4*)(out_lo + o) = ol[0];
                    *(u32x4*)(out_lo + o + 8) = ol[1];
                }
                float sa = ((v[0] + v[1]) + (v[2] + v[3])) + ((v[4] + v[5]) + (v[6] + v[7]));
                float sb = ((v[8] + v[9]) + (v[10] + v[11])) + ((v[12] + v[13]) + (v[14] + v[15]));
                float s1 = sa + sb;
                s1 += __shfl_xor(s1, 16, 64);
                s1 += __shfl_xor(s1, 32, 64);
                const float mg = s1 * (1.0f / 64.0f);
                float qa = 0.f, qb = 0.f;
#pragma unroll
                for (int e = 0; e < 8; ++e) {
                    const float da = v[e] - mg, db = v[8 + e] - mg;
                    qa = fmaf(da, da, qa);
                    qb = fmaf(db, db, qb);
                }
                float s2 = qa + qb;
                s2 += __shfl_xor(s2, 16, 64);
                s2 += __shfl_xor(s2, 32, 64);
                if (fg_e == 0 && store) *(float2*)(g.stats_out + ((size_t)m * gran + (nb >> 6)) * 2) = float2{s1, s2};
            }
        } else if constexpr (!RESID) {
            const int nb = SPLIT ? n0 + wc * 64 + fg_e * 8 : n0 + wc * 16 * C::TI + fg_e * 4 * C::TI;
            auto fcol = [&](int f) { return SPLIT ? (f >> 1) * 32 + (f & 1) * 4 : f * 4; };
            const int mrow = m0 + wr * (C::XR / 2) + frow_e;
            auto epilogue = [&](auto LNc) {
                constexpr bool LN = decltype(LNc)::value;
                f32x4 bias4[C::TI], s4[LN ? C::TI : 1];
                float2 st[LN ? TJ : 1];
#pragma unroll
                for (int f = 0; f < C::TI; ++f) bias4[f] = *(const f32x4*)(tbias + nb + fcol(f));
                if constexpr (LN) {
#pragma unroll
                    for (int f = 0; f < C::TI; ++f) s4[f] = *(const f32x4*)(g.ln_s + nb + fcol(f));
#pragma unroll
                    for (int J = 0; J < TJ; ++J) st[J] = *(const float2*)(g.rowstat + 2 * (size_t)(mrow + rowJ(J)));
                }
                uint16_t* obase = g.out_blocked
                    ? (uint16_t*)g.out + (((size_t)(mrow >> 6) * (g.ldo >> 6) + (nb >> 6)) << 12) + ((mrow & 63) << 6) + (nb & 63)
                    : (uint16_t*)g.out + (size_t)mrow * g.ldo + nb;
                const size_t step16 = g.out_blocked ? (size_t)16 * 64 : (size_t)16 * g.ldo;
                const size_t step128 = g.out_blocked ? ((size_t)2 * (g.ldo >> 6) << 12) : (size_t)C::XR * g.ldo;
                const bool store = !(VP_ABLATE(g) & 8);
#pragma unroll
                for (int J = 0; J < TJ; ++J) {
                    uint32_t o[2 * C::TI];
#pragma unroll
                    for (int f = 0; f < C::TI; ++f) {
                        f32x4 v = acc[f][J];
                        if constexpr (LN) {
#pragma unroll
                            for (int r = 0; r < 4; ++r) v[r] = ln_fold(v[r], st[J].x, s4[f][r], st[J].y, bias4[f][r]);
                        } else {
                            v += bias4[f];
                        }
                        if (EPI == EPI_BIAS_GELU) {
#pragma unroll
                            for (int r = 0; r < 4; ++r) v[r] = gelu_sat<T>(v[r]);
                            o[2 * f] = pack2_nosat<T>(v[0], v[1]);
                            o[2 * f + 1] = pack2_nosat<T>(v[2], v[3]);
                        } else {
                            o[2 * f] = pack2<T>(v[0], v[1]);
                            o[2 * f + 1] = pack2<T>(v[2], v[3]);
                        }
                    }
                    uint16_t* dst = obase + (size_t)(J / MJ) * step128 + (size_t)(J % MJ) * step16;
                    if constexpr (C::BM != 256) {
                        if (g.out_blocked) {
                            const int row = mrow + rowJ(J);
                            dst = (uint16_t*)g.out + (((size_t)(row >> 6) * (g.ldo >> 6) + (nb >> 6)) << 12) + ((row & 63) << 6) + (nb & 63);
                        }
                    }
                    if (store) {
                        if constexpr (C::TI == 4) {
                            if (VP_ABLATE(g) & 64) {
                                __builtin_nontemporal_store(u32x4{o[0], o[1], o[2], o[3]}, (u32x4*)dst);
                                __builtin_nontemporal_store(u32x4{o[4], o[5], o[6], o[7]}, (u32x4*)(dst + 32));
                            } else {
                                *(u32x4*)dst = u32x4{o[0], o[1], o[2], o[3]};
                                *(u32x4*)(dst + 32) = u32x4{o[4], o[5], o[6], o[7]};
                            }
                        } else {
                            *(u32x2*)dst = u32x2{o[0], o[1]};
                            *(u32x2*)(dst + 4) = u32x2{o[2], o[3]};
                            *(u32x2*)(dst + 8) = u32x2{o[4], o[5]};
                        }
                    }
                }
            };
            if (g.rowstat != nullptr) epilogue(std::true_type{});
            else epilogue(std::false_type{});
            if (tl && lane == 0 && (wave & 3) == 0) {
                const int ti = (t - tw.j0) / tw.nloc;
                if (ti < 16) {
                    unsigned long long* sp = (unsigned long long*)g.stats_out + (((size_t)blockIdx.x * 2 + wr) * 16 + ti) * 8;
                    sp[0] = ts0; sp[1] = ts1; sp[2] = __builtin_readcyclecounter();
#if (VP_G8_ABL & 16)
                    if (ti == 1) {
                        unsigned long long* sq = (unsigned long long*)g.stats_out + (((size_t)blockIdx.x * 2 + wr) * 16 + 8) * 8;
#pragma unroll
                        for (int i = 0; i < 12; ++i) sq[i] = sec[i];
                    }
#endif
                }
            }
        } else {
            static_assert(C::BM == 256, "the LDS-staged residual epilogue is written for 256-row tiles");
            constexpr int ROWBYTES = C::BN * 4 + 16;
            constexpr int JPP = (C::BN == 256) ? 2 : 4;
            constexpr int CR = 32 * JPP;
            constexpr int NPASS = 256 / CR;
            constexpr int CPR = C::BN / 8;
            constexpr int NCH = CR * CPR / C::NT;
            constexpr int GR = C::BN / 64;
            static_assert(NCH * C::NT == CR * CPR, "chunks must split evenly over threads");
            static_assert(CR * ROWBYTES + C::BM * GR * 8 <= 160 * 1024, "LDS");
            float* statbuf = (float*)(smem + CR * ROWBYTES);
            uint16_t* out_hi = (uint16_t*)g.out;
            uint16_t* out_lo = out_hi + g.plane;
            const uint16_t* aux_hi = (const uint16_t*)g.aux;
            const uint16_t* aux_lo = aux_hi + g.plane;
            const int nl = wc * 16 * C::TI + fg_e * 4 * C::TI;
            f32x4 bias4[C::TI];
#pragma unroll
            for (int f = 0; f < C::TI; ++f) bias4[f] = *(const f32x4*)(tbias + n0 + nl + f * 4);
            unsigned long long rs[6] = {ts0, ts1, 0, 0, 0, 0};
            auto tile_row = [&](int p, int lr) {
                return (p / (4 / JPP)) * 128 + (lr / (16 * JPP)) * 64 + ((p % (4 / JPP)) * JPP + (lr / 16) % JPP) * 16 + (lr & 15);
            };
            wait_vm<0>();
            if (!wr) bar();
            __syncthreads();
            if (tl) rs[2] = __builtin_readcyclecounter();
#pragma unroll
            for (int p = 0; p < NPASS; ++p) {
                size_t orow_q[NCH];
                u32x4 ra[NCH], rb[NCH];
#pragma unroll
                for (int q = 0; q < NCH; ++q) {
                    const int c = tid + q * C::NT;
                    const int lr = c / CPR, ch = c - lr * CPR;
                    const int m = m0 + tile_row(p, lr);
                    orow_q[q] = (size_t)m * g.ldo;
                    ra[q] = *(const u32x4*)(aux_hi + orow_q[q] + n0 + ch * 8);
                    rb[q] = *(const u32x4*)(aux_lo + orow_q[q] + n0 + ch * 8);
                }
#pragma unroll
                for (int jj = 0; jj < JPP; ++jj) {
                    char* lrow = smem + (wr * 16 * JPP + jj * 16 + frow_e) * ROWBYTES + nl * 4;
                    const int J = (p / (4 / JPP)) * 4 + (p % (4 / JPP)) * JPP + jj;
#pragma unroll
                    for (int f = 0; f < C::TI; ++f) *(f32x4*)(lrow + f * 16) = acc[f][J] + bias4[f];
                }
                __syncthreads();
#pragma unroll
                for (int q = 0; q < NCH; ++q) {
                    const int c = tid + q * C::NT;
                    const int lr = c / CPR, ch = c - lr * CPR;
                    float v[8];
                    const f32x4 s0 = *(const f32x4*)(smem + lr * ROWBYTES + ch * 32);
                    const f32x4 s1 = *(const f32x4*)(smem + lr * ROWBYTES + ch * 32 + 16);
#pragma unroll
                    for (int e = 0; e < 8; ++e) {
                        const float st = e < 4 ? s0[e] : s1[e - 4];
                        const int sh = (e & 1) * 16;
                        const float r = from_bits<T>((uint16_t)(ra[q][e >> 1] >> sh)) + from_bits<T>((uint16_t)(rb[q][e >> 1] >> sh));
                        v[e] = st + r;
                    }
                    u32x4 oh, ol;
#pragma unroll
                    for (int e = 0; e < 8; e += 2) { uint32_t h_, l_; split_planes2<T>(v[e], v[e + 1], h_, l_); oh[e >> 1] = h_; ol[e >> 1] = l_; }
                    if (!(VP_ABLATE(g) & 8)) {
                        size_t so = orow_q[q] + n0 + ch * 8;
                        if (VP_ABLATE(g) & 128) so &= (size_t)0xFFFF8;
                        *(u32x4*)(out_hi + so) = oh;
                        *(u32x4*)(out_lo + so) = ol;
                    }
                    float s1s = ((v[0] + v[1]) + (v[2] + v[3])) + ((v[4] + v[5]) + (v[6] + v[7]));
                    s1s = row8_sum8(s1s);
                    const float mg = s1s * (1.0f / 64.0f);
                    float s2 = 0.f;
#pragma unroll
                    for (int e = 0; e < 8; ++e) {
                        const float d = v[e] - mg;
                        s2 = fmaf(d, d, s2);
                    }
                    s2 = row8_sum8(s2);
                    if ((ch & 7) == 0) *(float2*)(statbuf + (tile_row(p, lr) * GR + (ch >> 3)) * 2) = float2{s1s, s2};
                }
                __syncthreads();
            }
            if (tl) rs[3] = __builtin_readcyclecounter();
            for (int i = tid; i < C::BM * GR; i += C::NT) {
                const int trow = i / GR, gi = i - trow * GR;
                if (!(VP_ABLATE(g) & 8))
                    *(float2*)(g.stats_out + ((size_t)(m0 + trow) * (g.N / 64) + ((n0 >> 6) + gi)) * 2) = *(const float2*)(statbuf + i * 2);
            }
            __syncthreads();
            if (tl) rs[4] = __builtin_readcyclecounter();
            if (has_next) ring_start();
            if (tl && g.ln_part && lane == 0 && (wave & 3) == 0) {
                const int ti = (t - tw.j0) / tw.nloc;
                if (ti < 16) {
                    unsigned long long* sp = (unsigned long long*)g.ln_part + (((size_t)blockIdx.x * 2 + wr) * 16 + ti) * 8;
                    rs[5] = __builtin_readcyclecounter();
#pragma unroll
                    for (int i = 0; i < 6; ++i) sp[i] = rs[i];
                }
            }
        }
        if constexpr (!DRAIN) { if (wr) bar(); }
        if (!has_next) break;
        t += tw.nloc;
        m0 = nm0;
        n0 = nn0;
    }
    wait_vm<0>();
    if constexpr (!DRAIN) {
        if (!wr) bar();
    }
}

template <class T, int EPI, class C>
static hipError_t launch8(const GemmArgs& a, hipStream_t s) {
    auto kern = gemm8_kernel<T, EPI, C>;
    int ex = 0;
    if constexpr (EPI == EPI_BIAS_RESID_LN)
        if (a.expert) { kern = gemm8_kernel<T, EPI, C, true>; ex = 1; }
    constexpr int LDS = (EPI == EPI_QKV_ATTN) ? 160 * 1024 : (EPI == EPI_BIAS_RESID_LN && C::BN != 256) ? ((128 * (C::BN * 4 + 16) + C::BM * (C::BN / 64) * 8) > C::RING ? (128 * (C::BN * 4 + 16) + C::BM * (C::BN / 64) * 8) : C::RING) : C::RING;
    static bool attr_done[2][64] = {};
    int dev = 0;
    (void)hipGetDevice(&dev);
    if (dev < 0 || dev >= 64 || !attr_done[ex][dev]) {
        hipError_t e = hipFuncSetAttribute((const void*)kern, hipFuncAttributeMaxDynamicSharedMemorySize, LDS);
        if (e != hipSuccess) return e;
        if (dev >= 0 && dev < 64) attr_done[ex][dev] = true;
    }
    const int tiles = (a.M / C::BM) * (a.N / C::BN);
    int grid = tiles < 256 ? tiles : 256;
#ifdef VP_TOOLS
    static const int max_wgs = [] { const char* e = getenv("VP_G8_WGS"); return e ? atoi(e) : 256; }();
    if (grid > max_wgs) grid = max_wgs;
#endif
    if (grid >= 256) grid &= ~7;
    if (grid < 8) return hipErrorInvalidValue;
    if (a.desc) snprintf(a.desc, a.desc_cap, "gemm8_kernel<%s, %d, G8<%d, %d>%s>", std::is_same<T, F16>::value ? "F16" : "BF16", EPI, C::BN, C::BM, ex ? ", true" : "");
    hipLaunchKernelGGL(kern, dim3(grid), dim3(C::NT), LDS, s, a);
    return hipGetLastError();
}

bool gemm8_shape_ok(int epi, int M, int N, int K, int ldo, int w_rows, int bn, int bm) {
    if (epi == EPI_QKV_ATTN)
        return bn == 256 && bm == 192 && M % 192 == 0 && N % 256 == 0 && (N >> 8) * 80 == K && K % 128 == 0 && K >= 256 && ldo == K &&
               (size_t)M * K * 2 < (1ull << 32) && (size_t)w_rows * K * 2 < (1ull << 32) && (M / 192) * (N / 256) >= 8;
    if (epi != EPI_BIAS && epi != EPI_BIAS_GELU && epi != EPI_BIAS_RESID_LN) return false;
    if (bn != 256 && bn != 192) return false;
    if (bm != 256 && !(bm == 192 && bn == 256)) return false;
    if (M % bm || N % bn || K % 128 || K < 256) return false;
    if ((size_t)M * K * 2 >= (1ull << 32) || (size_t)w_rows * K * 2 >= (1ull << 32)) return false;
    if ((M / bm) * (N / bn) < 8) return false;
    if (epi == EPI_BIAS_RESID_LN) return ldo == N;
    if ((size_t)M * N >= (1ull << 31)) return false;
    return bn == 256 && ldo == N;
}

bool gemm8_supported(int epi, const GemmArgs& a, int bn, int bm) {
    if (!gemm8_shape_ok(epi, a.M, a.N, a.K, a.ldo, a.w_rows, bn, bm)) return false;
    if (epi == EPI_QKV_ATTN) return a.rowstat && a.ln_s && !a.a_blocked && !a.out_blocked && !a.reverse;
    if (epi == EPI_BIAS_RESID_LN) return a.plane && a.stats_out && !a.out_blocked;
    return true;
}

hipError_t gemm8_launch(int dtype, int epi, const GemmArgs& a, int bn, hipStream_t s, int bm) {
    if (!gemm8_supported(epi, a, bn, bm)) return hipErrorInvalidValue;
#define VP_G8(TY)                                                                                                       \
    do {                                                                                                                \
        if (epi == EPI_QKV_ATTN) return launch8<TY, EPI_QKV_ATTN, G8<256, 192>>(a, s);                                  \
        if (epi == EPI_BIAS) return bm == 192 ? launch8<TY, EPI_BIAS, G8<256, 192>>(a, s) : launch8<TY, EPI_BIAS, G8<256>>(a, s);                \
        if (epi == EPI_BIAS_GELU) return bm == 192 ? launch8<TY, EPI_BIAS_GELU, G8<256, 192>>(a, s) : launch8<TY, EPI_BIAS_GELU, G8<256>>(a, s);  \
        if (bm == 192) return launch8<TY, EPI_BIAS_RESID_LN, G8<256, 192>>(a, s);                                       \
        if (bn == 256) return launch8<TY, EPI_BIAS_RESID_LN, G8<256>>(a, s);                                            \
        return launch8<TY, EPI_BIAS_RESID_LN, G8<192>>(a, s);                                                           \
    } while (0)
    if (dtype == DT_F16) VP_G8(F16);
    VP_G8(BF16);
#undef VP_G8
}

}
```

easy_vitpose_amd/csrc/gemm8_common.h:

```cpp
#pragma once
#include <type_traits>
#include <utility>

#include "common.h"
#include "kernels.h"

namespace vp {
namespace {

template <int BN_, int BM_ = 256> struct G8 {
    static constexpr int BM = BM_, BN = BN_, NT = 512;
    static constexpr int XR = BM / 2;
    static constexpr int MJ = XR / 32;
    static constexpr int WH1 = BN - 128;
    static constexpr int NF1 = WH1 / 64;
    static constexpr int TI = 2 + NF1, TJ = 2 * MJ;
    static constexpr int HALF = 128 * 128;
    static constexpr int XH = XR * 128;
    static constexpr int OFF_X0 = 0, OFF_X1 = XH, OFF_W0 = 2 * XH, OFF_W1 = 2 * XH + HALF;
    static constexpr int BUF = 2 * XH + HALF + WH1 * 128;
    static constexpr int RING = 2 * BUF;
    static constexpr int NW1 = WH1 / 64;
    static constexpr int INFLIGHT = 4 + NW1;
    static constexpr int NKEEP = (BM == 256 ? 6 : 5) + NW1;
    static_assert(BN == 256 || BN == 192, "BN");
    static_assert(BM == 256 || (BM == 192 && BN == 256), "BM");
};

template <int N> __device__ __forceinline__ void wait_vm() { asm volatile("s_waitcnt vmcnt(%0)" ::"n"(N) : "memory"); }
template <int N> __device__ __forceinline__ void wait_lgkm() { asm volatile("s_waitcnt lgkmcnt(%0)" ::"n"(N) : "memory"); }
__device__ __forceinline__ void bar() {
    __builtin_amdgcn_sched_barrier(0);
    __builtin_amdgcn_s_barrier();
    __builtin_amdgcn_sched_barrier(0);
}


__device__ __forceinline__ float row8_sum8(float x) {
    x += __builtin_bit_cast(float, __builtin_amdgcn_update_dpp(0, __builtin_bit_cast(int, x), 0xB1, 0xF, 0xF, true));
    x += __builtin_bit_cast(float, __builtin_amdgcn_update_dpp(0, __builtin_bit_cast(int, x), 0x4E, 0xF, 0xF, true));
    x += __builtin_bit_cast(float, __builtin_amdgcn_update_dpp(0, __builtin_bit_cast(int, x), 0x141, 0xF, 0xF, true));
    return x;
}

struct TileWalk {
    int tiles_m, tiles_n, group_m, base, cnt, j0, nloc;
    __device__ __forceinline__ void init(const GemmArgs& g, int BM, int BN) {
        tiles_n = (g.N + BN - 1) / BN;
        tiles_m = (g.M + BM - 1) / BM;
        group_m = g.group_m;
        const int ntiles = tiles_m * tiles_n;
        const int xcd = blockIdx.x & 7;
        j0 = blockIdx.x >> 3;
        nloc = (gridDim.x >> 3) + (xcd < (int)(gridDim.x & 7) ? 1 : 0);
        const int q = ntiles >> 3, r8 = ntiles & 7;
        base = (xcd < r8) ? xcd * (q + 1) : r8 * (q + 1) + (xcd - r8) * q;
        cnt = q + (xcd < r8 ? 1 : 0);
    }
    __device__ __forceinline__ void origin(int t, int reverse, int BM, int BN, int& m0, int& n0) const {
        int bid = base + t;
        if (reverse) bid = tiles_m * tiles_n - 1 - bid;
        int tm, tn;
        if (group_m > 1) {
            const int per_group = group_m * tiles_n;
            const int grp = bid / per_group, first_m = grp * group_m;
            const int gsz = min(tiles_m - first_m, group_m);
            const int r = bid - grp * per_group;
            tm = first_m + r % gsz;
            tn = r / gsz;
        } else {
            tm = bid / tiles_n;
            tn = bid - tm * tiles_n;
        }
        m0 = tm * BM;
        n0 = tn * BN;
    }
};

}
}
```

easy_vitpose_amd/csrc/handle.hip:

```cpp
#include "api_internal.h"

using namespace vpi;

namespace vpi {

thread_local std::string g_create_error;

int fail(vp_ctx* c, int code, const std::string& msg) {
    if (c) c->err = msg; else g_create_error = msg;
    return code;
}

int need_weights(vp_ctx* c) {
    if (!c) return VP_ERR_INVALID;
    return c->loaded ? (int)VP_OK : fail(c, VP_ERR_STATE, "weights not loaded: call vp_load_weights first");
}

bool slots_busy(const vp_ctx* c) { return c->slots[0].busy || c->slots[1].busy; }

int slots_idle(vp_ctx* c, const char* who) {
    return slots_busy(c) ? fail(c, VP_ERR_STATE, std::string(who) + " with a vp_infer_submit in flight: call vp_infer_wait first") : (int)VP_OK;
}

int quiesce(vp_ctx* c) {
    if (c->foreign_pending && c->ev_sw) HIPCHK(c, hipEventSynchronize(c->ev_sw));
    if (c->stream) HIPCHK(c, hipStreamSynchronize(c->stream));
    return VP_OK;
}

bool prof_begin(vp_ctx* c, int fam, double flops, double bytes) {
    if (!((c->prof >> fam) & 1u)) return false;
    std::pair<hipEvent_t, hipEvent_t> p;
    if (!c->ev_pool.empty()) {
        p = c->ev_pool.back();
        c->ev_pool.pop_back();
    } else {
        hipEventCreate(&p.first);
        hipEventCreate(&p.second);
    }
    hipEventRecord(p.first, c->stream);
    c->evs.push_back({p.first, p.second, fam, flops, bytes});
    return true;
}
void prof_end(vp_ctx* c, bool on) {
    if (on) hipEventRecord(c->evs.back().b, c->stream);
}
void prof_collect(vp_ctx* c) {
    for (auto& e : c->evs) {
        float ms = 0.f;
        if (hipEventElapsedTime(&ms, e.a, e.b) == hipSuccess) {
            c->acc.ms[e.fam] += ms;
            c->acc.flops[e.fam] += e.flops;
            c->acc.bytes[e.fam] += e.bytes;
            c->acc.launches[e.fam] += 1;
        }
        c->ev_pool.push_back({e.a, e.b});
    }
    c->evs.clear();
}

void apply_gemm_tuning(Switches& s) {
#ifndef VP_TOOLS
    (void)s;
#else
    if (const char* t = getenv("VP_GEMM_TUNE")) {
        int f, v, gm, used = 0;
        while (sscanf(t, "%d:%d:%d%n", &f, &v, &gm, &used) == 3) {
            if (f >= 0 && f < VP_PROF_COUNT) { s.gemm_variant[f] = v; s.gemm_group_m[f] = gm; }
            t += used;
            if (*t == ',') ++t; else break;
        }
    }
#endif
}

void read_switches(Switches& s) {
    auto on = [](const char* name, bool& dst) { if (const char* f = getenv(name)) dst = atoi(f) != 0; };
    auto num = [](const char* name, auto& dst) { if (const char* f = getenv(name)) dst = atol(f); };
    on("VP_FUSE_LN", s.fuse_ln);
    on("VP_PERSIST", s.persist_gemm);
    if (const char* f = getenv("VP_GRAPH")) s.graph_max_n = atoi(f) == 1 ? 16 : atoi(f);
    on("VP_GRAPH_NULL", s.graph_null);
    if (const char* f = getenv("VP_CALLER_STREAM")) s.caller_stream_max_n = atoi(f) == 1 ? 16 : atoi(f);
    on("VP_FUSE_HEAD", s.fuse_head);
    if (const char* f = getenv("VP_FOLD_STATS")) { s.graph_max_n_stats = atoi(f); s.fold_rule = false; }
    on("VP_BLOCKED_QKV", s.blocked_qkv);
    on("VP_FUSE_QKV_ATTN", s.fuse_qkv_attn);
    s.qa_min_set = getenv("VP_QA_MIN_TILES") != nullptr;
    num("VP_QA_MIN_TILES", s.qa_min_tiles);
    num("VP_QA80_MIN_TILES", s.qa80_min_tiles);
    num("VP_QA80_GROUP", s.qa80_group);
    num("VP_ATTN_QSPLIT", s.attn_qsplit);
    on("VP_DECONV_PARITY_FAST", s.deconv_parity_fast);
    on("VP_G8_COST", s.g8_cost_model);
    on("VP_PAD_BATCH", s.pad_batch);
    num("VP_G8_BM192", s.g8_bm192);
    if (const char* f = getenv("VP_SPLITK")) {
        if (!strchr(f, ':')) s.splitk_on = atoi(f) != 0;
        else {
            const char* t = f;
            while (*t) {
                const int which = !strncmp(t, "fc2:", 4) ? 1 : !strncmp(t, "proj:", 5) ? 0 : -1;
                if (which < 0) break;
                t = strchr(t, ':') + 1;
                int S = 0, v = 0, used = 0;
                if (sscanf(t, "%d:%d%n", &S, &v, &used) != 2) break;
                s.splitk_force[which][0] = S; s.splitk_force[which][1] = v;
                t += used;
                if (*t == ',') ++t;
            }
        }
    }
    num("VP_GEMM8", s.gemm8_mask);
    s.fp8_proj16 = getenv("VP_FP8_PROJ16") != nullptr;
#ifdef VP_TOOLS
    num("VP_G8_MIN_TILES", s.g8_min_tiles);
    on("VP_BLOCKED_HID", s.blocked_hid);
    num("VP_ORDER", s.order_mask);
    num("VP_G8_STAGGER", s.g8_stagger);
    if (const char* t = getenv("VP_ABLATE_FAM")) {
        int f, b, used = 0;
        while (sscanf(t, "%d:%d%n", &f, &b, &used) == 2) {
            if (f >= 0 && f < VP_PROF_COUNT) s.fam_ablate[f] = b;
            t += used;
            if (*t == ',') ++t; else break;
        }
    }
#endif
    apply_gemm_tuning(s);
}

int flip_partner_table(int K, const int32_t* pairs, int n_pairs, int32_t* partner, std::string* why) {
    auto bad = [&](const std::string& m) { if (why) *why = m; return VP_ERR_INVALID; };
    if (K <= 0 || !partner) return bad("no joints");
    if (n_pairs < 0) return bad("negative n_pairs");
    if (n_pairs > 0 && !pairs) return bad("null flip_pairs with n_pairs > 0");
    for (int k = 0; k < K; ++k) partner[k] = k;
    for (int i = 0; i < n_pairs; ++i) {
        const int a = pairs[2 * i], b = pairs[2 * i + 1];
        if (a < 0 || b < 0 || a >= K || b >= K)
            return bad("flip pair " + std::to_string(i) + " = (" + std::to_string(a) + ", " + std::to_string(b) + ") outside the head's " + std::to_string(K) + " joints");
        partner[a] = b;
        partner[b] = a;
    }
    return VP_OK;
}

}

extern "C" {

int vp_abi_version(void) { return VP_ABI_VERSION; }

int vp_create(vp_handle* out, const vp_config* cfg) {
    if (!out || !cfg) return fail(nullptr, VP_ERR_INVALID, "null argument");
    *out = nullptr;
    const int D = cfg->embed_dim, h = cfg->num_heads;
    if (D <= 0 || h <= 0 || D % h != 0 || D % 128 != 0 || D > 1280)
        return fail(nullptr, VP_ERR_INVALID, "embed_dim must be a multiple of 128 (<= 1280) and divisible by num_heads");
    const int hd = D / h;
    if (hd != 32 && hd != 64 && hd != 80) return fail(nullptr, VP_ERR_INVALID, "head_dim must be 32, 64 or 80");
    if (cfg->depth <= 0 || cfg->num_keypoints <= 0 || cfg->num_keypoints > 1024 || cfg->max_batch <= 0)
        return fail(nullptr, VP_ERR_INVALID, "depth, num_keypoints and max_batch must be positive");
    if (cfg->dtype != VP_DTYPE_F16 && cfg->dtype != VP_DTYPE_BF16 && cfg->dtype != VP_DTYPE_FP8) return fail(nullptr, VP_ERR_INVALID, "unknown dtype");
    if (cfg->dtype == VP_DTYPE_FP8 && (D % 256 != 0 || D < 768))
        return fail(nullptr, VP_ERR_INVALID, "the fp8 mode needs embed_dim >= 768 and a multiple of 256 (K-tiles of 128, an even number of them; >= 8 tiles per GEMM at the smallest batch): ViTPose-B / -L / -H");
    int ndev = 0;
    hipError_t e = hipGetDeviceCount(&ndev);
    if (e != hipSuccess || ndev <= 0)
        return fail(nullptr, VP_ERR_HIP, std::string("no HIP device available (this library has no CPU fallback): ") +
                                             (e != hipSuccess ? hipGetErrorString(e) : "device count 0"));
    if (cfg->device_id < 0 || cfg->device_id >= ndev) return fail(nullptr, VP_ERR_INVALID, "device_id out of range");
    vp_ctx* c = new vp_ctx();
    c->cfg = *cfg;
    c->D = D; c->L = cfg->depth; c->heads = h; c->Kp = cfg->num_keypoints; c->Kmax = c->Kp;
    c->dtype = cfg->dtype == VP_DTYPE_BF16 ? vp::DT_BF16 : vp::DT_F16;
    c->fp8 = cfg->dtype == VP_DTYPE_FP8;
    c->maxb = cfg->max_batch;
    read_switches(c->sw);
    auto bail = [&](int rc) { g_create_error = c->err; vp_destroy(c); return rc; };
    if ((e = hipSetDevice(cfg->device_id)) != hipSuccess) { c->err = hipGetErrorString(e); return bail(VP_ERR_HIP); }
    if ((e = hipStreamCreateWithFlags(&c->stream, hipStreamNonBlocking)) != hipSuccess) { c->err = hipGetErrorString(e); return bail(VP_ERR_HIP); }
    c->own_stream = c->stream;
    const size_t B = (size_t)((c->maxb + 3) / 4 * 4);
    c->Mp = std::max<size_t>((B * 192 + 255) / 256 * 256, 512);
    const size_t M = c->fp8 ? c->Mp : B * 192;
    int rc = 0;
    void* stage = nullptr;
    if ((rc = dalloc(c, (char**)&stage, B * crop_bytes(VP_INPUT_F32_NCHW)))) return bail(rc);
    c->in_stage = stage;
    if ((rc = dalloc(c, &c->wh_stage, B * 2))) return bail(rc);
    if ((rc = dalloc(c, &c->x, M * D))) return bail(rc);
    if ((rc = dalloc(c, &c->y, M * D))) return bail(rc);
    if (c->fp8 && !c->sw.fuse_ln) { c->err = "the fp8 mode is built on the fused-LayerNorm path (unset VP_FUSE_LN)"; return bail(VP_ERR_INVALID); }
    if (c->sw.fuse_ln) {
        if ((rc = dalloc(c, &c->ln_part, M * (size_t)(D / 64) * 2))) return bail(rc);
        if ((rc = dalloc(c, &c->rowstat, M * 2))) return bail(rc);
    }
    if (c->fp8) {
        if ((rc = dalloc(c, &c->x8, M * D)) || (rc = dalloc(c, &c->xs8, M * (size_t)(D / 32))) || (rc = dalloc(c, &c->hs8, M * (size_t)(4 * D / 32)))) return bail(rc);
        if (hipMemset(c->x, 0, M * D * 4) != hipSuccess) { c->err = "hipMemset"; return bail(VP_ERR_HIP); }
        if (hd == 64 && !c->sw.fp8_proj16) {
            if ((rc = dalloc(c, &c->y8, M * D)) || (rc = dalloc(c, &c->ys8, M * (size_t)(D / 32)))) return bail(rc);
            if (hipMemset(c->y8, 0, M * D) != hipSuccess || hipMemset(c->ys8, 0, M * (size_t)(D / 32)) != hipSuccess) { c->err = "hipMemset"; return bail(VP_ERR_HIP); }
        }
    }
    if ((rc = dalloc(c, &c->qkv, M * 3 * D))) return bail(rc);
    if ((rc = dalloc(c, &c->hid, M * 4 * D))) return bail(rc);
    if ((rc = dalloc(c, &c->d1, B * 768 * 256))) return bail(rc);
    if ((rc = dalloc(c, &c->d2, B * 3072 * 256))) return bail(rc);
    if ((rc = dalloc(c, &c->hm, B * c->Kp * 3072))) return bail(rc);
    if ((rc = dalloc(c, &c->kp, B * c->Kp * 3))) return bail(rc);
    if (c->sw.fuse_ln && !c->fp8 && c->sw.splitk_on) {
        c->splitk_rows = (size_t)std::min<int>(c->maxb, SPLITK_MAX_CROPS) * 192;
        if ((rc = dalloc(c, &c->splitk_ws, (size_t)SPLITK_MAX_S * c->splitk_rows * D))) return bail(rc);
    }
    if ((rc = dalloc(c, &c->zero, (size_t)256))) return bail(rc);
    if (hipMemset(c->zero, 0, 512) != hipSuccess) { c->err = "hipMemset"; return bail(VP_ERR_HIP); }
    *out = c;
    return VP_OK;
}

void* vp_host_alloc(size_t bytes) {
    void* p = nullptr;
    if (hipHostMalloc(&p, bytes ? bytes : 1, hipHostMallocDefault) != hipSuccess) return nullptr;
    return p;
}
void vp_host_free(void* p) { if (p) hipHostFree(p); }

int vp_set_flip_test(vp_handle c, const int32_t* flip_pairs, int32_t n_pairs, int32_t shift_heatmap) {
    int rc = need_weights(c);
    if (rc) return rc;
    std::vector<int32_t> partner((size_t)c->Kmax);
    std::string why;
    if (flip_partner_table(c->Kp, flip_pairs, n_pairs, partner.data(), &why)) return fail(c, VP_ERR_INVALID, "vp_set_flip_test: " + why);
    for (int k = c->Kp; k < c->Kmax; ++k) partner[k] = k;
    if (c->maxb < 2)
        return fail(c, VP_ERR_STATE, "vp_set_flip_test: a crop and its mirror image share the forward batch, which needs max_batch >= 2 (this handle has 1)");
// ... 163 lines not shown
```

easy_vitpose_amd/csrc/kernels.h:

```cpp
#pragma once
#include <hip/hip_runtime.h>
#include <stdint.h>

#ifdef VP_TOOLS
#define VP_ABLATE(g) ((g).ablate)
#define VP_STAGGER(g) ((g).stagger)
namespace vp {
hipError_t peak_bench(int kind, double* result);
hipError_t hwid_probe_launch(uint32_t* d_out, int blocks, int threads, int lds_bytes, int spin, hipStream_t s);
}
#else
#define VP_ABLATE(g) 0
#define VP_STAGGER(g) 0
#endif

namespace vp {

enum { DT_F16 = 0, DT_BF16 = 1 };

enum GemmEpi {
    EPI_BIAS = 0,
    EPI_BIAS_GELU = 1,
    EPI_BIAS_RESID = 2,
    EPI_POS = 3,
    EPI_DECONV = 4,
    EPI_HEATMAP = 5,
    EPI_BIAS_RESID_LN = 6,
    EPI_POS_LN = 7,
    EPI_DECONV_FINAL = 8,
    EPI_QKV_ATTN = 9,
    EPI_PARTIAL = 10,
};
enum GemmAMode { A_DENSE = 0, A_DECONV = 1 };

struct GemmArgs {
    const uint16_t* A;
    const uint16_t* W;
    const float* bias;
    void* out;
    const float* aux;
    int M, N, K, ldo;
    int Hin, Win, Cin;
    const uint16_t* zero;
    int Kp;
    const uint16_t* W2;
    const float* bias2;
    float* out2;
    int w_rows;
    int variant;
    int group_m;
    size_t w_parity_stride;
    size_t plane;
    float* stats_out;
    const float* rowstat;
    const float* ln_s;
    const float* ln_part;
    int ln_tiles;
    float ln_inv_d;
    int a_blocked, out_blocked;
    int reverse;
    int persist;
    int stagger;
    int ablate;
    char* desc;
    int desc_cap;
    float attn_scale_log2e;
    int splitk;
    int parity_fast;
    union {
        const uint8_t* a_scales;
        const int32_t* expert;
    };
    const float* w_scale;
    uint8_t* out_scales;
};
hipError_t gemm_launch(int dtype, int epi, const GemmArgs& a, hipStream_t s);
bool gemm8_supported(int epi, const GemmArgs& a, int bn, int bm = 256);
bool gemm8_shape_ok(int epi, int M, int N, int K, int ldo, int w_rows, int bn, int bm);
hipError_t gemm8_launch(int dtype, int epi, const GemmArgs& a, int bn, hipStream_t s, int bm = 256);

bool gemm8f_supported(int epi, const GemmArgs& a, int bn);
hipError_t gemm8f_launch(int epi, const GemmArgs& a, int bn, hipStream_t s);
hipError_t ln_quant_launch(int dtype, const uint16_t* x_hi, const float* ln_part, int tiles, uint8_t* codes, uint8_t* scales, int M, int Mp, int D,
                           hipStream_t s);
hipError_t mx_quantize_launch(const float* src, uint8_t* codes, uint8_t* scales, int M, int K, hipStream_t s);

hipError_t fill_random16(int dtype, uint16_t* p, size_t n, uint32_t seed, hipStream_t s);

hipError_t ln_finalize_launch(const float* partials, float* rowstat, int M, int tiles, int D, hipStream_t s);
hipError_t splitk_reduce_launch(int dtype, const float* partials, int S, const float* bias, uint16_t* x_hi, size_t plane, float* stats_out, int M, int N,
                                hipStream_t s);

hipError_t fp8_probe_launch(const float* dA, const float* dW, const float* dAs, const float* dWs, uint8_t* dA8, uint8_t* dW8, float* dOut,
                            int M, int N, int K, hipStream_t s);

hipError_t mx_probe_launch(const float* dA, const float* dW, const float* dWs, uint8_t* dA8, uint8_t* dAs, uint8_t* dW8, float* dOut,
                           int M, int N, int K, hipStream_t s);

hipError_t attention_launch(int dtype, const uint16_t* qkv, uint16_t* out, int B, int D, int heads, hipStream_t s, bool qsplit, int qkv_blocked = 0,
                            uint8_t* mx_scales = nullptr);

struct QkvAttnArgs {
    const uint16_t* x_hi;
    const uint16_t* wh;
    const float* bh;
    const float* sh;
    const float* rowstat;
    uint16_t* y;
    int npairs, heads, D;
    int ncrops;
    float scale_log2e;
    int ablate;
};
bool qkvattn_supported(const QkvAttnArgs& a);
hipError_t qkvattn_launch(int dtype, const QkvAttnArgs& a, hipStream_t s, char* desc, int desc_cap);
hipError_t qkv_head_major_launch(const uint16_t* w, const float* b, const float* s, uint16_t* wh, float* bh, float* sh, int D, int K, hipStream_t st);
hipError_t qkv_head_major80_launch(const uint16_t* w, const float* b, const float* s, uint16_t* wh, float* bh, float* sh, int D, int K, int heads, hipStream_t st);

hipError_t layernorm_launch(int dtype, const float* x, const float* gamma, const float* beta,
                            uint16_t* out16, float* out32, int M, int D, hipStream_t s, size_t plane = 0);
hipError_t im2col_launch(int dtype, const void* crops, int input_format, uint16_t* out, int B, hipStream_t s, bool flip = false, int n_src = 0);
hipError_t gather_crops_launch(const void* src, void* dst, const int32_t* idx, int n, size_t crop_bytes, hipStream_t s);
hipError_t flip_merge_launch(float* hm, const float* hm_flipped, const int32_t* partner, int N, int K, int shift, hipStream_t s, int interleaved = 0);
hipError_t im2col_twin_launch(int dtype, const void* crops, int input_format, uint16_t* out, int B, int n_src, hipStream_t s);
void flip_twin_layout(int bo, int n_src, int* src, int* mirror);

struct CropRec {
    const uint8_t* src;
    int64_t pitch;
    int32_t cw, ch, left, top, pw, ph;
};
hipError_t crop_resize_launch(const CropRec* recs, uint8_t* out, int n, hipStream_t s);

constexpr int BOX_FRAMES_PER_LAUNCH = 128;
struct BoxFrames {
    const uint8_t* data[BOX_FRAMES_PER_LAUNCH];
    int32_t h[BOX_FRAMES_PER_LAUNCH], w[BOX_FRAMES_PER_LAUNCH];
    int32_t f0, count, n_frames;
};
hipError_t box_geometry_launch(const BoxFrames& fr, const float* xyxy, int row_stride, const int32_t* frame_idx, int n, int pad, const uint8_t* zero_px,
                               CropRec* recs, int32_t* wh, int32_t* aux, int32_t* p9_out, int32_t* status_out, hipStream_t s, const int32_t* slot = nullptr);

hipError_t decode_launch(const float* hm, const int32_t* org_wh, float* out, int N, int K, hipStream_t s);
hipError_t decode_flip_launch(const float* hm, const int32_t* partner, int shift, const int32_t* org_wh, float* out, int N, int K, hipStream_t s);

struct MixRec {
    int32_t first, K, dst;
};
hipError_t decode_mix_launch(const float* hm, const MixRec* recs, const int32_t* org_wh, float* out, int N, int Kmax, hipStream_t s);
struct MixRecFlip {
    int32_t first, K, dst, e;
};
hipError_t decode_flip_mix_launch(const float* hm, const MixRecFlip* recs, const int32_t* partners, int shift, const int32_t* org_wh, float* out, int N, int Kmax,
                                  hipStream_t s);
hipError_t box_offsets_launch(const int32_t* aux, float* out, int n, int K, hipStream_t s, const int32_t* slot = nullptr, const MixRec* recs = nullptr);

constexpr int MIX_CROPS_PER_LAUNCH = 128;
struct MixTable {
    int32_t id[MIX_CROPS_PER_LAUNCH], order[MIX_CROPS_PER_LAUNCH], first[MIX_CROPS_PER_LAUNCH], K[MIX_CROPS_PER_LAUNCH];
    int32_t base, count, pad_to;
};
hipError_t mix_tables_launch(const MixTable& t, int32_t* ids, int32_t* order, int32_t* slot, MixRec* recs, hipStream_t s);
hipError_t mix_tables_flip_launch(const MixTable& t, int32_t* ids, int32_t* order, int32_t* slot, MixRec* recs, MixRecFlip* recs_flip, hipStream_t s);

}
```

easy_vitpose_amd/csrc/qkvattn.hip:

```cpp
#include <cstdio>
#include <cstdlib>

#include "gemm8_common.h"

namespace vp {

namespace {
struct QA {
    static constexpr int NT = 512;
    static constexpr int XS = 192 * 128;
    static constexpr int W0S = 128 * 128, W1S = 64 * 128;
    static constexpr int OFF_X0 = 0, OFF_X1 = XS, OFF_W0 = 2 * XS, OFF_W1 = 2 * XS + W0S;
    static constexpr int BUF = 2 * XS + W0S + W1S;
    static constexpr int RING = 2 * BUF;
    static constexpr int VSUB = 192 * 32;
    static constexpr int V_BASE = 4 * XS;
    static_assert(6 * XS == RING && BUF <= 3 * XS && BUF + XS <= 4 * XS, "the attention phase reuses exactly the ring; buffer 0 + X0 of buffer 1 inside Q0 K0 Q1 K1");
};

__device__ __forceinline__ u32x2 lds_read_tr16(const char* p) {
    typedef __attribute__((__vector_size__(4 * sizeof(__fp16)))) __fp16 h4;
    typedef __attribute__((address_space(3))) h4* lds_h4;
    const h4 v = __builtin_amdgcn_ds_read_tr16_b64_v4f16((lds_h4)(p));
    return __builtin_bit_cast(u32x2, v);
}
}

template <class T>
__global__ __launch_bounds__(512, 2) void qkvattn_kernel(QkvAttnArgs g) {
    constexpr int QT = 3;
    extern __shared__ __attribute__((aligned(16))) char smem[];
    const int tid = threadIdx.x, lane = tid & 63;
    const int wave = __builtin_amdgcn_readfirstlane(tid >> 6);
    const int wr = wave >> 2, wc = wave & 3;
    const int K = g.D, nk = K >> 6;
    const int ntiles = g.npairs * g.heads;
    const int xcd = blockIdx.x & 7, j0 = blockIdx.x >> 3;
    const int nloc = (gridDim.x >> 3) + (xcd < (int)(gridDim.x & 7) ? 1 : 0);
    const int tq = ntiles >> 3, tr8 = ntiles & 7;
    const int tbase = (xcd < tr8) ? xcd * (tq + 1) : tr8 * (tq + 1) + (xcd - tr8) * tq;
    const int tcnt = tq + (xcd < tr8 ? 1 : 0);
    if (j0 >= tcnt) return;

    const int rip = lane >> 3, pslot = lane & 7;
    const int slog = pslot ^ (((wave & 1) << 2) | (rip >> 1));
    const uint32_t voff = (uint32_t)(rip * K + slog * 8) * 2u;
    const size_t r64 = (size_t)64 * K * 2;
    const char* xb = nullptr;
    const char* wb = nullptr;
    size_t xb1off = 0;
    int pair = 0, head = 0;
    int ipair = 0, ihead = 0;
    auto set_tile = [&](int t) {
        const int tile = tbase + t;
        ipair = tile / g.heads;
        ihead = tile - ipair * g.heads;
        xb = (const char*)(g.x_hi + ((size_t)ipair * 384 + wave * 8) * K);
        xb1off = (2 * ipair + 1 < g.ncrops) ? (size_t)192 * K * 2 : 0;
        wb = (const char*)(g.wh + ((size_t)ihead * 192 + wave * 8) * K);
    };
    auto issue = [&](int which, int B, int kt) {
        char* dst = smem + B * QA::BUF + wave * 1024;
        uint32_t v = voff;
        asm volatile("" : "+v"(v));
        if (which < 2) {
            const char* src = xb + (which ? xb1off : 0) + (size_t)kt * 128 + v;
            glds16(src, dst + which * QA::XS);
            glds16(src + r64, dst + which * QA::XS + 8192);
            glds16(src + 2 * r64, dst + which * QA::XS + 16384);
        } else if (which == 2) {
            const char* src = wb + (size_t)kt * 128 + v;
            glds16(src, dst + QA::OFF_W0);
            glds16(src + r64, dst + QA::OFF_W0 + 8192);
        } else {
            const char* src = wb + 2 * r64 + (size_t)kt * 128 + v;
            glds16(src, dst + QA::OFF_W1);
        }
    };

    const int frow = lane & 15, fg = lane >> 4;
    const int foff = frow * 128 + ((fg ^ ((frow >> 1) & 7)) << 4);
    const int xadd = wr * 96 * 128, w0add = wc * 32 * 128, w1add = wc * 16 * 128;

    f32x4 acc[3][12];
    u32x4 xs[6][2], fa[2][2], fb[2];

    constexpr int NKEEP = 9;
    auto ktile = [&](auto Bc, auto Mc, int kA, int kB) {
        constexpr int B = decltype(Bc)::value;
        constexpr int MODE = decltype(Mc)::value;
        const char* sb = smem + B * QA::BUF;
        int fo = foff;
        asm volatile("" : "+v"(fo));
        const int xoff = xadd + fo, w0off = w0add + fo, w1off = w1add + fo;
#pragma unroll
        for (int p = 0; p < 2; ++p)
#pragma unroll
            for (int kk = 0; kk < 2; ++kk) fa[p][kk] = *(const u32x4*)(sb + QA::OFF_W0 + ((w0off + p * 2048) ^ (kk << 6)));
#pragma unroll
        for (int kk = 0; kk < 2; ++kk) fb[kk] = *(const u32x4*)(sb + QA::OFF_W1 + (w1off ^ (kk << 6)));
#pragma unroll
        for (int j = 0; j < 6; ++j)
#pragma unroll
            for (int kk = 0; kk < 2; ++kk) xs[j][kk] = *(const u32x4*)(sb + QA::OFF_X0 + ((xoff + j * 2048) ^ (kk << 6)));
        __builtin_amdgcn_sched_barrier(0);
        if constexpr (MODE != 3) issue(1, B ^ 1, kA);
        if constexpr (MODE == 3) wait_vm<0>();
        else if constexpr (MODE != 1) wait_vm<NKEEP>();
        wait_lgkm<0>();
        bar();
        __builtin_amdgcn_s_setprio(1);
#pragma unroll
        for (int kk = 0; kk < 2; ++kk)
#pragma unroll
            for (int j = 0; j < 6; ++j) {
                acc[0][j] = mfma16<T>(fa[0][kk], xs[j][kk], acc[0][j]);
                acc[1][j] = mfma16<T>(fa[1][kk], xs[j][kk], acc[1][j]);
                acc[2][j] = mfma16<T>(fb[kk], xs[j][kk], acc[2][j]);
            }
        __builtin_amdgcn_s_setprio(0);
        bar();
#pragma unroll
        for (int j = 0; j < 6; ++j)
#pragma unroll
            for (int kk = 0; kk < 2; ++kk) xs[j][kk] = *(const u32x4*)(sb + QA::OFF_X1 + ((xoff + j * 2048) ^ (kk << 6)));
        __builtin_amdgcn_sched_barrier(0);
        if constexpr (MODE < 2) {
            issue(2, B, kB);
            issue(0, B, kB);
            issue(3, B, kB);
            wait_vm<NKEEP>();
        } else if constexpr (MODE == 2) {
            wait_vm<3>();
        }
        wait_lgkm<0>();
        bar();
        __builtin_amdgcn_s_setprio(1);
#pragma unroll
        for (int kk = 0; kk < 2; ++kk)
#pragma unroll
            for (int j = 0; j < 6; ++j) {
                acc[0][6 + j] = mfma16<T>(fa[0][kk], xs[j][kk], acc[0][6 + j]);
                acc[1][6 + j] = mfma16<T>(fa[1][kk], xs[j][kk], acc[1][6 + j]);
                acc[2][6 + j] = mfma16<T>(fb[kk], xs[j][kk], acc[2][6 + j]);
            }
        __builtin_amdgcn_s_setprio(0);
        bar();
    };
    using M0 = std::integral_constant<int, 0>;
    using M1 = std::integral_constant<int, 1>;
    using M2 = std::integral_constant<int, 2>;
    using M3 = std::integral_constant<int, 3>;
    using B0 = std::integral_constant<int, 0>;
    using B1 = std::integral_constant<int, 1>;
    auto ring_start = [&]() {
        issue(2, 0, 0); issue(0, 0, 0); issue(3, 0, 0); issue(1, 0, 0);
        issue(2, 1, 1); issue(0, 1, 1); issue(3, 1, 1);
        wait_vm<6>();
        bar();
        if (wr) bar();
    };

    int t = j0;
    set_tile(t);
    ring_start();
    for (;;) {
        pair = ipair;
        head = ihead;
        const bool has_next = t + nloc < tcnt;
        bool prefetched = false;
#pragma unroll
        for (int f = 0; f < 3; ++f)
#pragma unroll
            for (int j = 0; j < 12; ++j) acc[f][j] = f32x4{0.f, 0.f, 0.f, 0.f};
        ktile(B0{}, M1{}, 1, 2);
        ktile(B1{}, M0{}, 2, 3);
        for (int kt = 2; kt < nk - 2; kt += 2) {
            if (VP_ABLATE(g) & 4) break;
            ktile(B0{}, M0{}, kt + 1, kt + 2);
            ktile(B1{}, M0{}, kt + 2, kt + 3);
        }
        ktile(B0{}, M2{}, nk - 1, 0);
        ktile(B1{}, M3{}, 0, 0);
        int frow_e = frow, fg_e = fg;
        asm volatile("" : "+v"(frow_e), "+v"(fg_e));
        const int cb = head * 192 + fg_e * 4;
        f32x4 b4[3], s4[3];
        float2 stat[12];
#pragma unroll
        for (int f = 0; f < 3; ++f) {
            const int c = cb + (f < 2 ? wc * 32 + f * 16 : 128 + wc * 16);
            b4[f] = *(const f32x4*)(g.bh + c);
            s4[f] = *(const f32x4*)(g.sh + c);
        }
        const bool twin = 2 * pair + 1 >= g.ncrops;
        const float* rs0 = g.rowstat + 2 * ((size_t)pair * 384 + wr * 96 + frow_e);
#pragma unroll
        for (int j = 0; j < 6; ++j) stat[j] = *(const float2*)(rs0 + 32 * j);
        wait_vm<0>();
        if (!wr) bar();
        __syncthreads();

        if (!(VP_ABLATE(g) & 2)) {
            const int dcol = wc * 16 + fg_e * 4;
            const int qk_byte = (fg_e & 1) * 8;
            const int qk_slot = wc * 2 + (fg_e >> 1);
            const int v_sub = 2 * (wc >> 1) + (fg_e & 1);
            const int v_byte = ((wc & 1) * 2 + (fg_e >> 1)) * 8;
            (void)dcol;
#pragma unroll
            for (int j = 6; j < 12; ++j) stat[j] = *(const float2*)(rs0 + (twin ? 0 : 384) + 32 * (j - 6));
#pragma unroll
            for (int j = 0; j < 12; ++j) {
                const int crop = j / 6;
                const int row = wr * 96 + (j % 6) * 16 + frow_e;
                const float2 st = stat[j];
                char* cb_ = smem + crop * 2 * QA::XS;
                const int rsw = (row >> 1) & 7;
#pragma unroll
                for (int f = 0; f < 3; ++f) {
                    f32x4 v;
#pragma unroll
                    for (int e = 0; e < 4; ++e) v[e] = ln_fold(acc[f][j][e], st.x, s4[f][e], st.y, b4[f][e]);
                    const u32x2 o = {pack2<T>(v[0], v[1]), pack2<T>(v[2], v[3])};
                    if (f < 2) *(u32x2*)(cb_ + f * QA::XS + row * 128 + ((qk_slot ^ rsw) << 4) + qk_byte) = o;
                    else *(u32x2*)(smem + QA::V_BASE + crop * QA::XS + v_sub * QA::VSUB + row * 32 + v_byte) = o;
                }
            }
        }
        __syncthreads();

        if (!(VP_ABLATE(g) & 1)) {
            const int crop = wave >> 2, lw = wave & 3;
            const char* Qs = smem + crop * 2 * QA::XS;
            const char* Ks = Qs + QA::XS;
            const char* Vs = smem + QA::V_BASE + crop * QA::XS;
            int fr = frow, fg = lane >> 4;
            asm volatile("" : "+v"(fr), "+v"(fg));
            const char* kfrag = Ks + fr * 128;
            const int kswz = (fr >> 1) & 7;
            const char* vfrag = Vs + (fg * 4 + (fr >> 2)) * 32 + (fr & 3) * 8;
            const size_t b = (size_t)pair * 2 + ((2 * pair + 1 < g.ncrops) ? crop : 0);
#pragma unroll
            for (int t0 = 0; t0 < 3; t0 += QT) {
                u32x4 qf[QT][2];
#pragma unroll
                for (int tq_ = 0; tq_ < QT; ++tq_)
#pragma unroll
                    for (int kk = 0; kk < 2; ++kk) qf[tq_][kk] = *(const u32x4*)(Qs + ((lw * 3 + t0 + tq_) * 16 + fr) * 128 + (((kk * 4 + fg) ^ kswz) << 4));
                f32x4 s[QT][12];
#pragma unroll
                for (int tq_ = 0; tq_ < QT; ++tq_)
#pragma unroll
                    for (int kt = 0; kt < 12; ++kt) s[tq_][kt] = f32x4{0.f, 0.f, 0.f, 0.f};
#pragma unroll
                for (int kt = 0; kt < 12; ++kt)
#pragma unroll
                    for (int kk = 0; kk < 2; ++kk) {
                        const u32x4 kf = *(const u32x4*)(kfrag + kt * 16 * 128 + (((kk * 4 + fg) ^ kswz) << 4));
#pragma unroll
                        for (int tq_ = 0; tq_ < QT; ++tq_) s[tq_][kt] = mfma16<T>(kf, qf[tq_][kk], s[tq_][kt]);
                    }
                __syncthreads();
                if (has_next) {
                    set_tile(t + nloc);
                    issue(2, 0, 0); issue(0, 0, 0); issue(3, 0, 0); issue(1, 0, 0);
                    issue(0, 1, 1);
                    prefetched = true;
                }
                u32x4 pf[QT][6];
                float inv_l[QT];
#pragma unroll
                for (int tq_ = 0; tq_ < QT; ++tq_) {
                    float mx = -3.0e38f;
#pragma unroll
                    for (int kt = 0; kt < 12; ++kt)
#pragma unroll
                        for (int r = 0; r < 4; ++r) mx = fmaxf(mx, s[tq_][kt][r]);
                    mx = fmaxf(mx, __shfl_xor(mx, 16, 64));
                    mx = fmaxf(mx, __shfl_xor(mx, 32, 64));
                    float l = 0.f;
                    const float mb = mx * g.scale_log2e;
#pragma unroll
                    for (int kt = 0; kt < 12; ++kt)
#pragma unroll
                        for (int r = 0; r < 4; ++r) {
                            const float p = softmax_p(s[tq_][kt][r], g.scale_log2e, mb);
                            s[tq_][kt][r] = p;
                            l += p;
                        }
                    l += __shfl_xor(l, 16, 64);
                    l += __shfl_xor(l, 32, 64);
                    inv_l[tq_] = 1.0f / l;
#pragma unroll
                    for (int kb = 0; kb < 6; ++kb) {
                        pf[tq_][kb][0] = pack2_nosat<T>(s[tq_][2 * kb][0], s[tq_][2 * kb][1]);
                        pf[tq_][kb][1] = pack2_nosat<T>(s[tq_][2 * kb][2], s[tq_][2 * kb][3]);
                        pf[tq_][kb][2] = pack2_nosat<T>(s[tq_][2 * kb + 1][0], s[tq_][2 * kb + 1][1]);
                        pf[tq_][kb][3] = pack2_nosat<T>(s[tq_][2 * kb + 1][2], s[tq_][2 * kb + 1][3]);
                    }
                }
#pragma unroll
                for (int dp = 0; dp < 4; dp += 2) {
                    f32x4 o[2][QT];
#pragma unroll
                    for (int u = 0; u < 2; ++u)
#pragma unroll
                        for (int tq_ = 0; tq_ < QT; ++tq_) o[u][tq_] = f32x4{0.f, 0.f, 0.f, 0.f};
#pragma unroll
                    for (int kb = 0; kb < 6; ++kb)
#pragma unroll
                        for (int u = 0; u < 2; ++u) {
                            const char* vp_ = vfrag + (dp + u) * QA::VSUB + kb * 1024;
                            const u32x2 lo = lds_read_tr16(vp_);
                            const u32x2 hi = lds_read_tr16(vp_ + 512);
                            const u32x4 vf = u32x4{lo[0], lo[1], hi[0], hi[1]};
#pragma unroll
                            for (int tq_ = 0; tq_ < QT; ++tq_) o[u][tq_] = mfma16<T>(vf, pf[tq_][kb], o[u][tq_]);
                        }
#pragma unroll
                    for (int tq_ = 0; tq_ < QT; ++tq_) {
                        const int q = (lw * 3 + t0 + tq_) * 16 + fr;
                        uint16_t* dst = g.y + (b * 192 + q) * g.D + head * 64;
                        u32x4 w;
                        w[0] = pack2_nosat<T>(o[0][tq_][0] * inv_l[tq_], o[0][tq_][1] * inv_l[tq_]);
                        w[1] = pack2_nosat<T>(o[0][tq_][2] * inv_l[tq_], o[0][tq_][3] * inv_l[tq_]);
                        w[2] = pack2_nosat<T>(o[1][tq_][0] * inv_l[tq_], o[1][tq_][1] * inv_l[tq_]);
                        w[3] = pack2_nosat<T>(o[1][tq_][2] * inv_l[tq_], o[1][tq_][3] * inv_l[tq_]);
                        *(u32x4*)(dst + dp * 16 + fg * 8) = w;
                    }
                }
            }
        }
        if (!has_next) break;
        t += nloc;
        __syncthreads();
        if (prefetched) {
            issue(2, 1, 1); issue(3, 1, 1);
            wait_vm<6>();
            bar();
            if (wr) bar();
        } else {
            set_tile(t);
            ring_start();
        }
    }
}

__global__ void qkv_head_major_kernel(const uint16_t* __restrict__ w, const float* __restrict__ b, const float* __restrict__ s, uint16_t* __restrict__ wh,
                                      float* __restrict__ bh, float* __restrict__ sh, int D, int K) {
    const int dst = blockIdx.x;
    const int h = dst / 192, r = dst - h * 192;
    int src;
    if (r < 128) {
        const int wc = r >> 5, p = (r >> 4) & 1, rho = r & 15;
        src = p * D + h * 64 + wc * 16 + rho;
    } else {
        src = 2 * D + h * 64 + (r - 128);
    }
    for (int k = threadIdx.x; k < K; k += blockDim.x) wh[(size_t)dst * K + k] = w[(size_t)src * K + k];
    if (threadIdx.x == 0) { bh[dst] = b[src]; sh[dst] = s[src]; }
}

hipError_t qkv_head_major_launch(const uint16_t* w, const float* b, const float* s, uint16_t* wh, float* bh, float* sh, int D, int K, hipStream_t st) {
    if (D % 64) return hipErrorInvalidValue;
    hipLaunchKernelGGL(qkv_head_major_kernel, dim3(3 * D), dim3(256), 0, st, w, b, s, wh, bh, sh, D, K);
    return hipGetLastError();
}

__global__ void qkv_head_major80_kernel(const uint16_t* __restrict__ w, const float* __restrict__ b, const float* __restrict__ s, uint16_t* __restrict__ wh,
                                        float* __restrict__ bh, float* __restrict__ sh, int D, int K) {
    const int dst = blockIdx.x;
    const int h = dst >> 8, r = dst & 255;
    const int src = r < 240 ? (r / 80) * D + h * 80 + r % 80 : -1;
    for (int k = threadIdx.x; k < K; k += blockDim.x) wh[(size_t)dst * K + k] = src >= 0 ? w[(size_t)src * K + k] : (uint16_t)0;
    if (threadIdx.x == 0) { bh[dst] = src >= 0 ? b[src] : 0.f; sh[dst] = src >= 0 ? s[src] : 0.f; }
}

hipError_t qkv_head_major80_launch(const uint16_t* w, const float* b, const float* s, uint16_t* wh, float* bh, float* sh, int D, int K, int heads, hipStream_t st) {
    if (heads * 80 != D) return hipErrorInvalidValue;
    hipLaunchKernelGGL(qkv_head_major80_kernel, dim3(heads * 256), dim3(256), 0, st, w, b, s, wh, bh, sh, D, K);
    return hipGetLastError();
}

bool qkvattn_supported(const QkvAttnArgs& a) {
    if (a.D % 128 || a.D < 256 || a.heads * 64 != a.D || a.npairs <= 0 || (a.ncrops != 2 * a.npairs && a.ncrops != 2 * a.npairs - 1)) return false;
    if ((size_t)a.npairs * 384 * a.D * 2 >= (1ull << 32)) return false;
    return a.npairs * a.heads >= 8;
}

hipError_t qkvattn_launch(int dtype, const QkvAttnArgs& a, hipStream_t s, char* desc, int desc_cap) {
    if (!qkvattn_supported(a)) return hipErrorInvalidValue;
    const int tiles = a.npairs * a.heads;
    const int grid = tiles < 256 ? tiles : 256;
    static bool attr_done[2][64] = {};
    int dev = 0;
    (void)hipGetDevice(&dev);
    const int di = dtype == DT_F16 ? 0 : 1;
    auto kern = dtype == DT_F16 ? qkvattn_kernel<F16> : qkvattn_kernel<BF16>;
    if (dev < 0 || dev >= 64 || !attr_done[di][dev]) {
        hipError_t e = hipFuncSetAttribute((const void*)kern, hipFuncAttributeMaxDynamicSharedMemorySize, QA::RING);
        if (e != hipSuccess) return e;
        if (dev >= 0 && dev < 64) attr_done[di][dev] = true;
    }
    if (desc) snprintf(desc, desc_cap, "qkvattn_kernel<%s>", dtype == DT_F16 ? "F16" : "BF16");
    hipLaunchKernelGGL(kern, dim3(grid), dim3(QA::NT), QA::RING, s, a);
    return hipGetLastError();
}

}
```

easy_vitpose_amd/csrc/tile_rules.hip:

```cpp
#include "api_internal.h"
#include "tiles.h"

using namespace vpi;

namespace vpi {

struct G8Pick { int variant, bm, bn; long tiles; };
struct Tile2Pick { int variant, group_m; };
using vp::is_gemm8;
struct SplitKPick { int S, variant; };

G8Pick pick_gemm8_tile(int M, int N, bool wide, int bm192_mask, long min_tiles, bool extended) {
    const bool ext = extended && M >= 7680;
    const long t2 = (long)((M + 191) / 192) * ((N + 127) / 128);
    const double cost2 = t2 <= 256 ? 24576.0 : (double)((t2 + 511) / 512) * 49152.0;
    G8Pick pk{0, 0, 0, 0};
    double best = 0.0;
    bool have256 = false;
    for (const vp::Tile8Row& cd : vp::TILES8) {
        if (M % cd.BM || N % cd.BN || (wide && cd.id == 17)) continue;
        if (cd.id == 18 && (!(bm192_mask & (wide ? 2 : 1)) || (!ext && have256))) continue;
        const long t = (long)(M / cd.BM) * (N / cd.BN);
        if (t < 8) continue;
        const long rounds = (t + 255) / 256;
// ... 84 lines not shown
}

static int pick_run_batch(const Switches& s, int n, int D, int limit) {
    const int n4 = (n + 3) / 4 * 4;
    if (n < 33 || n4 == n || n4 > limit) return n;
    auto cost = [&](int m) {
        const int M = 192 * m;
        return mlp_gemm_cost(resolve_gemm(s, VP_PROF_GEMM_FC1, vp::EPI_BIAS_GELU, M, 4 * D, D), M, 4 * D, D) +
               mlp_gemm_cost(resolve_gemm(s, VP_PROF_GEMM_FC2, vp::EPI_BIAS_RESID_LN, M, D, 4 * D), M, D, 4 * D);
    };
    const double c0 = cost(n), c1 = cost(n4);
    return (c0 > 0.0 && c1 > 0.0 && c1 < 0.95 * c0) ? n4 : n;
}

int tile_bm(int variant) {
    if (const int bm8 = vp::tile8_bm(variant)) return bm8;
    int bm = 0, bn = 0, slots = 0;
    return tile2_dims(variant, bm, bn, slots) ? bm : 0;
}

bool expert_tile_ok(int bm, const std::vector<int>& bounds) {
    if (bm <= 0) return false;
    for (int b : bounds)
        if (((long)b * 192) % bm) return false;
    return true;
}

int expert_fallback_variant(int M, int N, bool gemm8_ok, int* group_m) {
    constexpr vp::Tile8Row t8 = *vp::find_tile8(18);
    if (gemm8_ok && N % t8.BN == 0 && (long)(M / t8.BM) * (N / t8.BN) >= 448) { *group_m = 2; return t8.id; }
    *group_m = 0;
    return 11;
}

static int gemm8_group_m(int fam) { return fam == VP_PROF_GEMM_QKV ? 4 : fam == VP_PROF_GEMM_FC2 ? 2 : 8; }

GemmPick resolve_gemm(const Switches& s, int fam, int epi, int M, int N, int K, bool ln_part, size_t splitk_rows, const std::vector<int>* mix_bounds) {
    GemmPick p;
    const bool tuned = s.gemm_variant[fam] >= 0;
    const bool wide = epi == vp::EPI_BIAS || epi == vp::EPI_BIAS_GELU;
    const int w_rows = (int)pad128((size_t)N);
    if (tuned) {
        p.variant = s.gemm_variant[fam]; p.group_m = s.gemm_group_m[fam];
    } else {
        const Tile2Pick tp = pick_gemm2_tile(epi, M, N, K);
        p.variant = tp.variant; p.group_m = tp.group_m;
    }
    if (s.persist_gemm && p.variant == 8 && wide && K % 128 == 0 && M % 192 == 0 && N % 128 == 0 && (long)(M / 192) * (N / 128) >= 1024)
        p.persist = 1;
    const int g8bit = fam == VP_PROF_GEMM_FC2 ? 1 : fam == VP_PROF_GEMM_FC1 ? 2 : fam == VP_PROF_GEMM_QKV ? 4 : fam == VP_PROF_GEMM_PROJ ? 8 : 0;
    if (!tuned && (s.gemm8_mask & g8bit) && (wide || epi == vp::EPI_BIAS_RESID_LN)) {
        const G8Pick pk = pick_gemm8_tile(M, N, wide, s.g8_bm192, s.g8_min_tiles, s.g8_cost_model);
        if (pk.variant && vp::gemm8_shape_ok(epi, M, N, K, N, w_rows, pk.bn, pk.bm)) {
            p.variant = pk.variant; p.group_m = gemm8_group_m(fam); p.persist = 0; p.stagger = s.g8_stagger;
        }
    }
    if (epi == vp::EPI_DECONV_FINAL) { p.variant = 3; p.group_m = 0; p.persist = 0; }
    if (ln_part) {
        p.persist = 0;
        if (is_gemm8(p.variant)) { p.variant = 8; p.group_m = 8; }
    }
    const bool mixed = mix_bounds && fam == VP_PROF_GEMM_FC2;
    if (mixed && !expert_tile_ok(tile_bm(p.variant), *mix_bounds)) {
        const bool g8 = (s.gemm8_mask & 1) && vp::gemm8_shape_ok(epi, M, N, K, N, w_rows, vp::tile8_bn(18), vp::tile8_bm(18));
        p.variant = expert_fallback_variant(M, N, g8, &p.group_m);
        p.persist = 0;
        p.stagger = p.variant == 18 ? s.g8_stagger : 0;
    }
    if (epi == vp::EPI_BIAS_RESID_LN && !mixed && splitk_rows && (size_t)M <= splitk_rows && !tuned && !is_gemm8(p.variant) &&
        (fam == VP_PROF_GEMM_FC2 || fam == VP_PROF_GEMM_PROJ)) {
        const int which = fam == VP_PROF_GEMM_FC2 ? 1 : 0;
        SplitKPick sk = pick_splitk(M, N, K);
        if (s.splitk_force[which][0] > 0) sk = {s.splitk_force[which][0], s.splitk_force[which][1]};
        if (sk.S > 1 && sk.S <= SPLITK_MAX_S && K % (sk.S * 128) == 0) { p.splitk = sk.S; p.splitk_variant = sk.variant; }
    }
    return p;
}

GemmPick resolve_gemm_fp8(int fam, int epi, int Mp, int N) {
    int bn = 256;
    if (epi == vp::EPI_BIAS_RESID_LN) {
        double fill = -1.0;
        for (int cand : {256, 192}) {
            if (N % cand) continue;
            const long t = (long)(Mp / 256) * (N / cand);
            if (t < 8) continue;
            const double f = (double)t / (double)((t + 255) / 256 * 256);
            if (f > fill + 1e-9) { bn = cand; fill = f; }
        }
    }
    GemmPick p;
    p.variant = bn == 192 ? 17 : 16;
    p.group_m = gemm8_group_m(fam);
    return p;
}

HeadPlan plan_head(const Switches& s, int D, int nh, size_t fin_rows) {
    HeadPlan h;
    h.fused = s.fuse_head && s.gemm_variant[VP_PROF_GEMM_DECONV] < 0 && (long)nh * 12 >= 512;
    h.deconv1 = resolve_gemm(s, VP_PROF_GEMM_DECONV, vp::EPI_DECONV, nh * 192, 256, 4 * D);
    h.deconv2 = resolve_gemm(s, VP_PROF_GEMM_DECONV, h.fused ? vp::EPI_DECONV_FINAL : vp::EPI_DECONV, nh * 768, 256, 1024);
    if (!h.fused) h.final = resolve_gemm(s, VP_PROF_GEMM_FINAL, vp::EPI_HEATMAP, nh * 3072, (int)fin_rows, 256);
    return h;
}

ChunkPlan plan_chunk(const Switches& s, int D, int heads, int max_batch, bool fp8, int n_in, size_t fin_rows, const std::vector<int>* mix_bounds) {
    ChunkPlan p;
    p.n = (s.pad_batch && s.fuse_ln && !fp8) ? pick_run_batch(s, n_in, D, (max_batch + 3) / 4 * 4) : n_in;
    const int n = p.n, M = 192 * n, hd = D / heads;
    const size_t splitk_rows = (s.fuse_ln && !fp8 && s.splitk_on) ? (size_t)std::min(max_batch, SPLITK_MAX_CROPS) * 192 : 0;
    auto gemm = [&](int fam, int epi, int N, int K, bool ln_part) { return resolve_gemm(s, fam, epi, M, N, K, ln_part, splitk_rows, mix_bounds); };
    p.attn_qsplit = (long)n * heads <= s.attn_qsplit;
    p.head = plan_head(s, D, n_in, fin_rows);
    const int resid = s.fuse_ln ? vp::EPI_BIAS_RESID_LN : vp::EPI_BIAS_RESID;
    p.gemm[VP_PROF_GEMM_PATCH] = gemm(VP_PROF_GEMM_PATCH, s.fuse_ln ? vp::EPI_POS_LN : vp::EPI_POS, D, 768, false);
    p.gemm[VP_PROF_GEMM_PROJ] = gemm(VP_PROF_GEMM_PROJ, resid, D, D, false);
    if (fp8) {
        const int Mp = std::max((M + 255) / 256 * 256, 512);
        p.proj_fp8 = hd == 64 && !s.fp8_proj16;
        p.gemm[VP_PROF_GEMM_QKV] = resolve_gemm_fp8(VP_PROF_GEMM_QKV, vp::EPI_BIAS, Mp, 3 * D);
        if (p.proj_fp8) p.gemm[VP_PROF_GEMM_PROJ] = resolve_gemm_fp8(VP_PROF_GEMM_PROJ, vp::EPI_BIAS_RESID_LN, Mp, D);
        p.gemm[VP_PROF_GEMM_FC1] = resolve_gemm_fp8(VP_PROF_GEMM_FC1, vp::EPI_BIAS_GELU, Mp, 4 * D);
        p.gemm[VP_PROF_GEMM_FC2] = resolve_gemm_fp8(VP_PROF_GEMM_FC2, vp::EPI_BIAS_RESID_LN, Mp, D);
        return p;
    }
    p.gemm[VP_PROF_GEMM_FC2] = gemm(VP_PROF_GEMM_FC2, resid, D, 4 * D, false);
    if (!s.fuse_ln) {
        p.gemm[VP_PROF_GEMM_QKV] = gemm(VP_PROF_GEMM_QKV, vp::EPI_BIAS, 3 * D, D, false);
        p.gemm[VP_PROF_GEMM_FC1] = gemm(VP_PROF_GEMM_FC1, vp::EPI_BIAS_GELU, 4 * D, D, false);
        return p;
    }
    const bool fold_stats = n <= s.graph_max_n_stats;
    auto folds = [&](int fam, int epi, int N) {
        if (fold_stats) return true;
        if (!s.fold_rule || n > 64 || s.gemm_variant[fam] >= 0) return false;
        const int v = gemm(fam, epi, N, D, false).variant;
        return vp::tile_folds_stats(v);
    };
    const bool has_qkvh = s.fuse_qkv_attn && (hd == 64 || (heads * 80 == D && D % 128 == 0));
    const bool qkv_can_fold = folds(VP_PROF_GEMM_QKV, vp::EPI_BIAS, 3 * D);
    const long pair_tiles = (long)((n + 1) / 2) * heads;
    const bool want80 = has_qkvh && heads * 80 == D && (long)n * heads >= s.qa80_min_tiles;
    const bool want64 = has_qkvh && heads * 64 == D && pair_tiles >= s.qa_min_tiles && (s.qa_min_set || pair_tiles >= 128 || !qkv_can_fold);
    p.fold1 = fold_stats || (!want80 && !want64 && qkv_can_fold);
    p.fold2 = folds(VP_PROF_GEMM_FC1, vp::EPI_BIAS_GELU, 4 * D);
    vp::QkvAttnArgs qa{};
    qa.npairs = (n + 1) / 2; qa.ncrops = n; qa.heads = heads; qa.D = D;
    if (s.gemm_variant[VP_PROF_GEMM_QKV] < 0 && !p.fold1) {
        if (want80 && vp::gemm8_shape_ok(vp::EPI_QKV_ATTN, M, heads * 256, D, D, heads * 256, 256, 192)) p.qkv_path = QKV_ATTN80;
        else if (want64 && vp::qkvattn_supported(qa)) p.qkv_path = QKV_ATTN64;
    }
    p.gemm[VP_PROF_GEMM_QKV] = gemm(VP_PROF_GEMM_QKV, vp::EPI_BIAS, 3 * D, D, p.fold1);
    p.gemm[VP_PROF_GEMM_FC1] = gemm(VP_PROF_GEMM_FC1, vp::EPI_BIAS_GELU, 4 * D, D, p.fold2);
    return p;
}

}

extern "C" {

VP_API int vp_dbg_expert_tile(int32_t variant, int32_t M, int32_t N, int32_t gemm8_ok, const int32_t* bounds, int32_t n_bounds) {
    if (M <= 0 || N <= 0 || n_bounds < 0 || (n_bounds > 0 && !bounds)) return VP_ERR_INVALID;
    const std::vector<int> b(bounds, bounds + n_bounds);
    if (expert_tile_ok(tile_bm(variant), b)) return variant;
    int gm = 0;
    return expert_fallback_variant(M, N, gemm8_ok != 0, &gm);
}

VP_API int vp_dbg_run_batch(int32_t n, int32_t D, int32_t limit) {
    if (n <= 0 || D <= 0) return VP_ERR_INVALID;
    return pick_run_batch(Switches{}, n, D, limit);
}

VP_API int vp_dbg_chunk_plan(const vp_config* cfg, int32_t n, int32_t* out, int32_t cap) {
    if (!cfg || cfg->embed_dim <= 0 || cfg->num_heads <= 0 || cfg->embed_dim % cfg->num_heads || cfg->num_keypoints <= 0 || cfg->max_batch <= 0 ||
        n <= 0 || n > cfg->max_batch || cap < 0 || (cap > 0 && !out))
        return VP_ERR_INVALID;
    Switches s;
    read_switches(s);
    const ChunkPlan p = plan_chunk(s, cfg->embed_dim, cfg->num_heads, cfg->max_batch, cfg->dtype == VP_DTYPE_FP8, n, final_rows((size_t)cfg->num_keypoints));
    std::vector<int32_t> v = {p.n, p.fold1, p.fold2, p.qkv_path, p.attn_qsplit, p.head.fused, p.proj_fp8};
    for (const GemmPick& g : {p.gemm[VP_PROF_GEMM_PATCH], p.gemm[VP_PROF_GEMM_QKV], p.gemm[VP_PROF_GEMM_PROJ], p.gemm[VP_PROF_GEMM_FC1], p.gemm[VP_PROF_GEMM_FC2],
                              p.head.deconv1, p.head.deconv2, p.head.final})
        v.insert(v.end(), {g.variant, g.group_m, g.persist, g.stagger, g.splitk, g.splitk_variant});
    std::copy(v.begin(), v.begin() + std::min<size_t>(v.size(), (size_t)cap), out);
    return (int)v.size();
}


VP_API int vp_dbg_gemm8_pick(int32_t M, int32_t N, int32_t wide, int32_t bm192_mask, int32_t* tiles) {
    if (M <= 0 || N <= 0) return VP_ERR_INVALID;
    const G8Pick pk = pick_gemm8_tile(M, N, wide != 0, bm192_mask & 3, 448, !(bm192_mask & 4));
    if (tiles) *tiles = (int32_t)pk.tiles;
    return pk.variant;
}

VP_API int vp_dbg_gemm2_pick(int32_t epi, int32_t M, int32_t N, int32_t K, int32_t* group_m) {
    if (M <= 0 || N <= 0 || K <= 0) return VP_ERR_INVALID;
    const Tile2Pick tp = pick_gemm2_tile(epi, M, N, K);
    if (group_m) *group_m = tp.group_m;
    return tp.variant;
}

VP_API int vp_dbg_splitk_pick(int32_t M, int32_t N, int32_t K, int32_t* variant) {
    if (M <= 0 || N <= 0 || K <= 0) return VP_ERR_INVALID;
    const SplitKPick sk = pick_splitk(M, N, K);
    if (variant) *variant = sk.variant;
    return sk.S;
}

}
```

include/vitpose_hip.h:

```cpp
#ifndef VITPOSE_HIP_H
#define VITPOSE_HIP_H

#include <stddef.h>
#include <stdint.h>

#ifdef __cplusplus
extern "C" {
#endif

#define VP_ABI_VERSION 4
#define VP_API __attribute__((visibility("default")))

enum {
    VP_OK = 0,
    VP_ERR_INVALID = 1,
    VP_ERR_HIP = 2,
    VP_ERR_STATE = 3,
    VP_ERR_MISSING_TENSOR = 4,
    VP_ERR_SHAPE = 5
};

enum {
    VP_DTYPE_F16 = 0,
    VP_DTYPE_BF16 = 1,
// ... 22 lines not shown
    const char* name;
    const float* data;
    int64_t numel;
} vp_tensor_desc;

#define VP_PROF_GEMM_PROJ 0
#define VP_PROF_GEMM_FC1 1
#define VP_PROF_GEMM_QKV 2
#define VP_PROF_GEMM_PATCH 3
#define VP_PROF_GEMM_DECONV 4
#define VP_PROF_GEMM_FINAL 5
#define VP_PROF_ATTN 6
#define VP_PROF_LAYERNORM 7
#define VP_PROF_IM2COL 8
#define VP_PROF_DECODE 9
#define VP_PROF_GEMM_FC2 10
#define VP_PROF_COUNT 11

typedef struct vp_profile {
    double ms[VP_PROF_COUNT];
    double flops[VP_PROF_COUNT];
    double bytes[VP_PROF_COUNT];
    int64_t launches[VP_PROF_COUNT];
} vp_profile;

VP_API int vp_abi_version(void);

VP_API int vp_create(vp_handle* out, const vp_config* cfg);

VP_API int vp_load_weights(vp_handle h, const vp_tensor_desc* tensors, int32_t n_tensors);

VP_API int vp_infer(vp_handle h, const void* crops, int32_t input_format, int32_t n,
             const int32_t* org_wh, float* out);

VP_API int vp_infer_device(vp_handle h, const void* d_crops, int32_t input_format, int32_t n,
                    const int32_t* d_org_wh, float* d_out, int32_t sync);

VP_API int vp_infer_device_stream(vp_handle h, const void* d_crops, int32_t input_format, int32_t n,
                                  const int32_t* d_org_wh, float* d_out, void* caller_stream);

VP_API void* vp_host_alloc(size_t bytes);
VP_API void vp_host_free(void* p);
VP_API int vp_infer_submit(vp_handle h, const void* crops, int32_t input_format, int32_t n, const int32_t* org_wh,
                           float* out, int32_t* slot);
VP_API int vp_infer_wait(vp_handle h, int32_t slot);

VP_API int vp_group_create(vp_group_handle* out, const vp_config* cfg, const int32_t* device_ids, int32_t n_devices);
VP_API int vp_group_peer_access_missing(vp_group_handle g);
VP_API int vp_group_size(vp_group_handle g);
VP_API vp_handle vp_group_member(vp_group_handle g, int32_t i);
VP_API int vp_group_load_weights(vp_group_handle g, const vp_tensor_desc* tensors, int32_t n_tensors);
VP_API int vp_group_infer(vp_group_handle g, const void* crops, int32_t input_format, int32_t n, const int32_t* org_wh, float* out);
VP_API int vp_group_infer_allgather(vp_group_handle g, const void* crops, int32_t input_format, int32_t n, const int32_t* org_wh,
                                    float* const* d_all, float* out);
VP_API int vp_group_destroy(vp_group_handle g);
VP_API const char* vp_group_last_error(vp_group_handle g);

VP_API int vp_infer_frame(vp_handle h, const uint8_t* frame, int32_t fh, int32_t fw, const int32_t* crop_params,
                          int32_t n, float* out);

typedef struct vp_frame {
    const uint8_t* data;
    int32_t h;
    int32_t w;
} vp_frame;
VP_API int vp_infer_frames(vp_handle h, const vp_frame* frames, int32_t n_frames, int32_t frames_on_device,
                           const int32_t* crop_params, int32_t n, float* out);

VP_API int vp_infer_boxes_stream(vp_handle h, const vp_frame* frames, int32_t n_frames, const float* d_xyxy, int32_t row_stride,
                                 const int32_t* d_frame_idx, int32_t n, int32_t pad, float* d_out, int32_t* d_crop_params,
                                 int32_t* d_status, void* caller_stream);

VP_API int vp_infer_flip(vp_handle h, const void* crops, int32_t input_format, int32_t n, const int32_t* org_wh,
                         const int32_t* flip_pairs, int32_t n_pairs, int32_t shift_heatmap, float* out, float* heatmaps);

#define VP_HAS_FLIP_TEST_MODE 1
VP_API int vp_set_flip_test(vp_handle h, const int32_t* flip_pairs, int32_t n_pairs, int32_t shift_heatmap);
VP_API int vp_clear_flip_test(vp_handle h);
VP_API int vp_flip_test_enabled(vp_handle h);
VP_API int vp_group_set_flip_test(vp_group_handle g, const int32_t* flip_pairs, int32_t n_pairs, int32_t shift_heatmap);
VP_API int vp_group_clear_flip_test(vp_group_handle g);
#define VP_HAS_FLIP_TEST_EXPERTS 1
VP_API int vp_set_flip_test_experts(vp_handle h, const int32_t* flip_pairs, const int32_t* n_pairs, int32_t shift_heatmap);
VP_API int vp_dbg_flip_partner(int32_t k, const int32_t* flip_pairs, int32_t n_pairs, int32_t* partner);
VP_API int vp_dbg_flip_layout(int32_t n, int32_t rows, int32_t* src, int32_t* mirror);
VP_API int vp_dbg_decode_flip(int32_t device_id, const float* heatmaps2, int32_t n, int32_t k, const int32_t* flip_pairs, int32_t n_pairs,
                              int32_t shift_heatmap, const int32_t* org_wh, float* out);

VP_API int vp_infer_heatmaps(vp_handle h, const void* crops, int32_t input_format, int32_t n, float* heatmaps);
VP_API int vp_infer_tokens(vp_handle h, const void* crops, int32_t input_format, int32_t n, float* tokens);

VP_API int vp_expert_info(vp_handle h, int32_t* n_experts, int32_t* part_features, int32_t* k_per_expert);
VP_API int vp_set_expert(vp_handle h, int32_t e);
VP_API int vp_infer_experts(vp_handle h, const void* crops, int32_t input_format, int32_t n, const int32_t* expert_ids,
                            const int32_t* org_wh, float* out);

#define VP_HAS_EXPERT_ENTRIES 1
VP_API int vp_infer_experts_device_stream(vp_handle h, const void* d_crops, int32_t input_format, int32_t n, const int32_t* expert_ids,
                                          const int32_t* d_org_wh, float* d_out, void* caller_stream);
VP_API int vp_infer_frames_experts(vp_handle h, const vp_frame* frames, int32_t n_frames, int32_t frames_on_device, const int32_t* crop_params,
                                   int32_t n, const int32_t* expert_ids, float* out);
VP_API int vp_infer_boxes_experts_stream(vp_handle h, const vp_frame* frames, int32_t n_frames, const float* d_xyxy, int32_t row_stride,
                                         const int32_t* d_frame_idx, int32_t n, int32_t pad, const int32_t* expert_ids, float* d_out,
                                         int32_t* d_crop_params, int32_t* d_status, void* caller_stream);
VP_API int vp_dbg_mix_plan(const int32_t* expert_ids, int32_t n, int32_t n_experts, int32_t max_batch, const int32_t* k_per_expert, int32_t* order,
                           int32_t* ids_padded, int32_t* counts, int32_t* records, uint64_t* pattern);
VP_API int vp_dbg_decode_mix(int32_t device_id, const float* heatmaps, int32_t n_maps, int32_t n, int32_t kmax, const int32_t* records,
                             const int32_t* org_wh, float* out);
VP_API int vp_dbg_mix_plan_flip(const int32_t* expert_ids, int32_t n, int32_t n_experts, int32_t max_batch, const int32_t* k_per_expert, int32_t* order,
                                int32_t* row_ids, int32_t* counts, int32_t* records, uint64_t* pattern);
VP_API int vp_dbg_decode_flip_mix(int32_t device_id, const float* heatmaps, int32_t n_maps, int32_t n, int32_t kmax, const int32_t* records4,
                                  const int32_t* partners, int32_t n_experts, int32_t shift_heatmap, const int32_t* org_wh, float* out);

VP_API int vp_decode_only(int32_t device_id, const float* heatmaps, int32_t n, int32_t k,
                   const int32_t* org_wh, float* out);

VP_API void* vp_stream(vp_handle h);
VP_API int vp_synchronize(vp_handle h);

VP_API int vp_set_profiling(vp_handle h, int32_t family_mask);
VP_API int vp_reset_profile(vp_handle h);
VP_API int vp_get_profile(vp_handle h, vp_profile* out);
VP_API int vp_profile_kernel(vp_handle h, int32_t family, char* buf, int32_t cap);

VP_API int vp_destroy(vp_handle h);

VP_API const char* vp_last_error(vp_handle h);

VP_API int vp_dbg_gemm(int32_t device_id, int32_t dtype, int32_t epi, int32_t M, int32_t N, int32_t K,
                       const float* A, const float* W, const float* bias, const float* aux, float* out);
VP_API int vp_dbg_attention(int32_t device_id, int32_t dtype, int32_t B, int32_t D, int32_t heads,
                            const float* qkv, float* out);
VP_API int vp_dbg_qkvattn(int32_t device_id, int32_t dtype, int32_t npairs, int32_t D, int32_t heads, const float* x, const float* W,
                          const float* bias, float* out);
VP_API int vp_dbg_layernorm(int32_t device_id, int32_t dtype, int32_t M, int32_t D, const float* x,
                            const float* gamma, const float* beta, float* out16, float* out32);
VP_API int vp_dbg_deconv(int32_t device_id, int32_t dtype, int32_t B, int32_t Hin, int32_t Win, int32_t Cin,
                         const float* x, const vp_tensor_desc* tensors, int32_t n_tensors, float* out);
VP_API int vp_dbg_crop_prep(int32_t device_id, const uint8_t* frame, int32_t fh, int32_t fw, const int32_t* crop_params,
                            int32_t n, uint8_t* out);
VP_API int vp_dbg_gemm_case(int32_t device_id, int32_t dtype, int32_t epi, int32_t variant, int32_t group_m, int32_t flags,
                            int32_t M, int32_t N, int32_t K, const float* A, const float* W, const float* bias, const float* aux,
                            const float* rowstat, const float* ln_s, float* out, float* stats);
VP_API int vp_dbg_group_plan(int32_t n, int32_t w, int32_t maxb, int32_t* offs, int32_t* cnts, int32_t cap);
VP_API int vp_dbg_frame_plan(const vp_frame* frames, int32_t n_frames, const int32_t* params9, int32_t n, int32_t* bands);
VP_API int vp_dbg_box_geometry(const float* xyxy, int32_t row_stride, const int32_t* frame_idx, const int32_t* frame_hw, int32_t n_frames,
                               int32_t n, int32_t pad, int32_t* out9, int32_t* status);
VP_API int vp_dbg_gemm8_pick(int32_t M, int32_t N, int32_t wide, int32_t bm192_mask, int32_t* tiles);
VP_API int vp_dbg_gemm2_pick(int32_t epi, int32_t M, int32_t N, int32_t K, int32_t* group_m);
VP_API int vp_dbg_splitk_pick(int32_t M, int32_t N, int32_t K, int32_t* variant);
VP_API int vp_dbg_run_batch(int32_t n, int32_t D, int32_t limit);
VP_API int vp_dbg_expert_tile(int32_t variant, int32_t M, int32_t N, int32_t gemm8_ok, const int32_t* bounds, int32_t n_bounds);
VP_API int vp_dbg_chunk_plan(const vp_config* cfg, int32_t n, int32_t* out, int32_t cap);
VP_API int vp_dbg_group_trace(int32_t n, int32_t w, int32_t maxb, int32_t* trace, int32_t cap);
VP_API int vp_dbg_fp8_gemm(int32_t device_id, int32_t M, int32_t N, int32_t K, const float* A, const float* a_scale, const float* W,
                           const float* w_scale, float* out, uint8_t* a_codes, uint8_t* w_codes);
VP_API int vp_dbg_mx_gemm(int32_t device_id, int32_t M, int32_t N, int32_t K, const float* A, const float* W, const float* w_scale, float* out,
                          uint8_t* a_codes, uint8_t* a_scales, uint8_t* w_codes);
VP_API int vp_dbg_gemm_fp8_case(int32_t device_id, int32_t epi, int32_t M, int32_t N, int32_t K, const float* A, const float* W, const float* bias,
                                const float* aux, float* out, float* stats, float* a_deq, float* w_deq);
VP_API int vp_dbg_host_e4m3(const float* in, uint8_t* out, int64_t n);

#ifdef __cplusplus
}
#endif
#endif
```

Measured before the change: 25800 persons/s.

## Merge per-tile LayerNorm partials inside consumer GEMM and fused QKV-attention kernels

For large batches (n>64), the consumer kernels (qkv GEMM, fused qkv+attention, fc1 GEMM) now reduce the LayerNorm row partials themselves. They stage the merged mean/rstd in an LDS statistics area, so the separate ln_finalize launch and its rowstat round trip are skipped. This removes 2 small kernel launches per layer plus their global memory traffic. In exchange it adds per-tile merge work and extra LDS, and it reshuffles barriers in the gemm8 epilogue.

```diff
diff --git a/easy_vitpose_amd/_capi.py b/easy_vitpose_amd/_capi.py
--- a/easy_vitpose_amd/_capi.py
+++ b/easy_vitpose_amd/_capi.py
@@ -25,7 +25,8 @@
            'vp_set_flip_test', 'vp_clear_flip_test', 'vp_flip_test_enabled', 'vp_group_set_flip_test', 'vp_group_clear_flip_test',
            'vp_dbg_flip_partner', 'vp_dbg_flip_layout', 'vp_dbg_decode_flip',
            'vp_infer_experts_device_stream', 'vp_infer_frames_experts', 'vp_infer_boxes_experts_stream', 'vp_dbg_mix_plan', 'vp_dbg_decode_mix',
-           'vp_set_flip_test_experts', 'vp_dbg_mix_plan_flip', 'vp_dbg_decode_flip_mix']
+           'vp_set_flip_test_experts', 'vp_dbg_mix_plan_flip', 'vp_dbg_decode_flip_mix',
+           'vp_dbg_chunk_merge', 'vp_dbg_gemm8_stats', 'vp_dbg_qkvattn_stats']
 
 
 class HipExtensionMissing(RuntimeError):
@@ -157,6 +158,9 @@
     lib.vp_dbg_decode_mix.argtypes = [C.c_int32, C.c_void_p, C.c_int32, C.c_int32, C.c_int32, C.c_void_p, C.c_void_p, C.c_void_p]
     lib.vp_dbg_chunk_plan.argtypes = [C.POINTER(vp_config), C.c_int32, C.c_void_p, C.c_int32]
     lib.vp_dbg_qkvattn.argtypes = [C.c_int32] * 5 + [C.c_void_p] * 4
+    lib.vp_dbg_chunk_merge.argtypes = [C.POINTER(vp_config), C.c_int32, C.c_void_p]
+    lib.vp_dbg_gemm8_stats.argtypes = [C.c_int32] * 8 + [C.c_void_p] * 5 + [C.c_int32, C.c_void_p]
+    lib.vp_dbg_qkvattn_stats.argtypes = [C.c_int32] * 5 + [C.c_void_p] * 5 + [C.c_int32, C.c_void_p]
     lib.vp_set_flip_test.argtypes = [H, C.c_void_p, C.c_int32, C.c_int32]
     lib.vp_clear_flip_test.argtypes = [H]
     lib.vp_flip_test_enabled.argtypes = [H]
diff --git a/easy_vitpose_amd/csrc/api_internal.h b/easy_vitpose_amd/csrc/api_internal.h
--- a/easy_vitpose_amd/csrc/api_internal.h
+++ b/easy_vitpose_amd/csrc/api_internal.h
@@ -56,6 +56,7 @@
     int caller_stream_max_n = 16;
     bool fold_rule = true;
     int graph_max_n_stats = 8;
+    bool merge_stats = true;
     bool splitk_on = true;
     int splitk_force[2][2] = {{0, 0}, {0, 0}};
     int gemm_variant[VP_PROF_COUNT] = {-1, -1, -1, -1, -1, -1, -1, -1, -1, -1, -1};
@@ -280,6 +281,7 @@
 struct ChunkPlan {
     int n = 0;
     bool fold1 = false, fold2 = false;
+    bool merge1 = false, merge2 = false;
     int qkv_path = QKV_GEMM;
     bool attn_qsplit = false;
     bool proj_fp8 = false;
diff --git a/easy_vitpose_amd/csrc/debug_taps.hip b/easy_vitpose_amd/csrc/debug_taps.hip
--- a/easy_vitpose_amd/csrc/debug_taps.hip
+++ b/easy_vitpose_amd/csrc/debug_taps.hip
@@ -1,4 +1,5 @@
 #include "dbg_util.h"
+#include "tiles.h"
 
 using namespace vpi;
 
@@ -84,6 +85,75 @@
     if (e == hipSuccess) e = vp::qkvattn_launch(c->dtype, qa, nullptr, nullptr, 0);
     if (e == hipSuccess) e = hipDeviceSynchronize();
     if (e != hipSuccess) return dbg_finish(c, fail(c, VP_ERR_HIP, std::string("qkvattn: ") + hipGetErrorString(e)));
+    return dbg_finish(c, download16(c, dy, out, M * D));
+}
+
+
+VP_API int vp_dbg_gemm8_stats(int32_t device, int32_t dtype, int32_t epi, int32_t variant, int32_t group_m, int32_t M, int32_t N, int32_t K, const float* A,
+                              const float* W, const float* bias, const float* ln_s, const float* partials, int32_t merged, float* out) {
+    if ((epi != vp::EPI_BIAS && epi != vp::EPI_BIAS_GELU) || !vp::is_gemm8(variant) || M <= 0 || N <= 0 || K <= 0 || K % 64 || !A || !W || !bias || !ln_s || !partials || !out)
+        return fail(nullptr, VP_ERR_INVALID, "bad gemm8 statistics case");
+    vp_ctx* c = dbg_ctx(device, dtype);
+    if (!c) return VP_ERR_HIP;
+    const size_t MN = (size_t)M * N, wrows = pad128(N);
+    const int tiles = K / 64;
+    uint16_t *dA, *dW, *dO;
+    float *dB, *dS, *dP, *dRow;
+    int r;
+    if ((r = upload_mat(c, &dA, A, M, K, M)) || (r = upload_mat(c, &dW, W, N, K, wrows)) || (r = upload_f32(c, &dB, bias, N, wrows)) || (r = upload_f32(c, &dS, ln_s, N, wrows)) ||
+        (r = upload_f32(c, &dP, partials, (size_t)M * tiles * 2)) || (r = dalloc(c, &dRow, (size_t)M * 2)) || (r = dalloc(c, &dO, MN)))
+        return dbg_finish(c, r);
+    hipMemset(dO, 0xff, MN * 2);
+    vp::GemmArgs g{};
+    g.A = dA; g.W = dW; g.bias = dB; g.out = dO; g.M = M; g.N = N; g.K = K; g.ldo = N; g.w_rows = (int)wrows; g.variant = variant; g.group_m = group_m; g.ln_s = dS;
+    hipError_t e = hipSuccess;
+    if (merged) { g.ln_part = dP; g.ln_tiles = tiles; g.ln_inv_d = 1.0f / (float)K; }
+    else { g.rowstat = dRow; e = vp::ln_finalize_launch(dP, dRow, M, tiles, K, nullptr); }
+    if (e == hipSuccess) e = vp::gemm_launch(c->dtype, epi, g, nullptr);
+    if (e == hipSuccess) e = hipDeviceSynchronize();
+    if (e != hipSuccess) return dbg_finish(c, fail(c, VP_ERR_HIP, std::string("gemm8 statistics case: ") + hipGetErrorString(e)));
+    return dbg_finish(c, download16(c, dO, out, MN));
+}
+
+VP_API int vp_dbg_qkvattn_stats(int32_t device, int32_t dtype, int32_t ncrops, int32_t D, int32_t heads, const float* x, const float* W, const float* bias,
+                                const float* ln_s, const float* partials, int32_t merged, float* out) {
+    if (ncrops <= 0 || D <= 0 || D % 64 || heads <= 0 || !x || !W || !bias || !ln_s || !partials || !out) return fail(nullptr, VP_ERR_INVALID, "bad qkvattn statistics case");
+    vp_ctx* c = dbg_ctx(device, dtype);
+    if (!c) return VP_ERR_HIP;
+    const size_t M = (size_t)ncrops * 192, D3 = 3 * (size_t)D;
+    const bool hd80 = heads * 80 == D;
+    const size_t hrows = hd80 ? (size_t)heads * 256 : D3;
+    const int tiles = D / 64;
+    uint16_t *dx, *dw, *dwh, *dy;
+    float *db, *dbh, *ds, *dsh, *dP, *dRow;
+    int rc;
+    if ((rc = upload_mat(c, &dx, x, M, D, M)) || (rc = upload_mat(c, &dw, W, D3, D, pad128(D3))) || (rc = upload_f32(c, &db, bias, D3)) || (rc = upload_f32(c, &ds, ln_s, D3)) ||
+        (rc = upload_f32(c, &dP, partials, M * tiles * 2)) || (rc = dalloc(c, &dRow, M * 2)) || (rc = dalloc(c, &dwh, hrows * D)) || (rc = dalloc(c, &dbh, hrows)) ||
+        (rc = dalloc(c, &dsh, hrows)) || (rc = dalloc(c, &dy, M * D)))
+        return dbg_finish(c, rc);
+    hipMemset(dy, 0xff, M * D * 2);
+    hipError_t e = hd80 ? vp::qkv_head_major80_launch(dw, db, ds, dwh, dbh, dsh, D, D, heads, nullptr) : vp::qkv_head_major_launch(dw, db, ds, dwh, dbh, dsh, D, D, nullptr);
+    if (e == hipSuccess && !merged) e = vp::ln_finalize_launch(dP, dRow, (int)M, tiles, D, nullptr);
+    if (hd80) {
+        vp::GemmArgs g80{};
+        g80.A = dx; g80.W = dwh; g80.bias = dbh; g80.ln_s = dsh; g80.out = dy;
+        g80.M = (int)M; g80.N = heads * 256; g80.K = D; g80.ldo = D; g80.w_rows = heads * 256; g80.variant = 18; g80.group_m = Switches{}.qa80_group;
+        g80.attn_scale_log2e = (1.0f / sqrtf(80.0f)) * 1.4426950408889634f;
+        if (merged) { g80.ln_part = dP; g80.ln_tiles = tiles; g80.ln_inv_d = 1.0f / (float)D; }
+        else g80.rowstat = dRow;
+        if (e == hipSuccess && !vp::gemm8_supported(vp::EPI_QKV_ATTN, g80, 256, 192)) return dbg_finish(c, fail(c, VP_ERR_INVALID, "shape not supported by the fused qkv + attention tile (head dim 80)"));
+        if (e == hipSuccess) e = vp::gemm_launch(c->dtype, vp::EPI_QKV_ATTN, g80, nullptr);
+    } else {
+        vp::QkvAttnArgs qa{};
+        qa.x_hi = dx; qa.wh = dwh; qa.bh = dbh; qa.sh = dsh; qa.y = dy; qa.npairs = (ncrops + 1) / 2; qa.ncrops = ncrops; qa.heads = heads; qa.D = D;
+        qa.scale_log2e = (1.0f / sqrtf(64.0f)) * 1.4426950408889634f;
+        if (merged) { qa.ln_part = dP; qa.ln_tiles = tiles; qa.ln_inv_d = 1.0f / (float)D; }
+        else qa.rowstat = dRow;
+        if (e == hipSuccess && !vp::qkvattn_supported(qa)) return dbg_finish(c, fail(c, VP_ERR_INVALID, "shape not supported by the fused qkv + attention kernel"));
+        if (e == hipSuccess) e = vp::qkvattn_launch(c->dtype, qa, nullptr, nullptr, 0);
+    }
+    if (e == hipSuccess) e = hipDeviceSynchronize();
+    if (e != hipSuccess) return dbg_finish(c, fail(c, VP_ERR_HIP, std::string("qkvattn statistics case: ") + hipGetErrorString(e)));
     return dbg_finish(c, download16(c, dy, out, M * D));
 }
 
diff --git a/easy_vitpose_amd/csrc/forward.hip b/easy_vitpose_amd/csrc/forward.hip
--- a/easy_vitpose_amd/csrc/forward.hip
+++ b/easy_vitpose_amd/csrc/forward.hip
@@ -152,12 +152,13 @@
         };
         const double qkv_attn_flops = 2.0 * M * 3.0 * D * D + 4.0 * 192 * 192 * (double)D * n, qkv_attn_bytes = 2.0 * M * D + 2.0 * 3 * D * (double)D + 2.0 * M * D;
         if ((rc = gemm(c, VP_PROF_GEMM_PATCH, vp::EPI_POS_LN, pk[VP_PROF_GEMM_PATCH], c->hid, c->w_patch, c->b_zero, c->x, c->pos, M, D, 768, D, 0, 0, 0, &prod))) return rc;
-        if ((rc = finalize(pl.fold1))) return rc;
+        if ((rc = finalize(pl.fold1 || pl.merge1))) return rc;
         for (int l = 0; l < c->L; ++l) {
             const Block& b = c->blocks[l];
             if (pl.qkv_path == QKV_ATTN80) {
                 vp::GemmArgs g80{};
                 g80.A = xh; g80.W = b.w_qkvh; g80.bias = b.b_qkvh; g80.ln_s = b.s_qkvh; g80.rowstat = c->rowstat; g80.out = c->y;
+                if (pl.merge1) { g80.rowstat = nullptr; g80.ln_part = c->ln_part; g80.ln_tiles = D / 64; g80.ln_inv_d = 1.0f / (float)D; }
                 g80.M = M; g80.N = c->heads * 256; g80.K = D; g80.ldo = D; g80.w_rows = c->heads * 256; g80.variant = 18;
                 g80.group_m = c->sw.qa80_group;
                 g80.attn_scale_log2e = (1.0f / sqrtf(80.0f)) * 1.4426950408889634f;
@@ -172,25 +173,26 @@
                 qa.x_hi = xh; qa.wh = b.w_qkvh; qa.bh = b.b_qkvh; qa.sh = b.s_qkvh; qa.rowstat = c->rowstat; qa.y = c->y;
                 qa.npairs = (n + 1) / 2; qa.ncrops = n; qa.heads = c->heads; qa.D = D;
                 qa.scale_log2e = (1.0f / sqrtf(64.0f)) * 1.4426950408889634f;
+                if (pl.merge1) { qa.rowstat = nullptr; qa.ln_part = c->ln_part; qa.ln_tiles = D / 64; qa.ln_inv_d = 1.0f / (float)D; }
                 char desc[96];
                 desc[0] = 0;
                 LAUNCH(c, VP_PROF_GEMM_QKV, qkv_attn_flops, qkv_attn_bytes, vp::qkvattn_launch(c->dtype, qa, c->stream, desc, (int)sizeof(desc)));
                 note_kernel(c, VP_PROF_GEMM_QKV, desc);
             } else {
                 LnFuse cq; cq.rowstat = c->rowstat; cq.ln_s = b.s_qkv; cq.reverse = (c->sw.order_mask & 1) != 0; cq.out_blocked = qkv_blocked;
-                if (pl.fold1) { cq.rowstat = nullptr; cq.ln_part = c->ln_part; cq.ln_tiles = D / 64; }
+                if (pl.fold1 || pl.merge1) { cq.rowstat = nullptr; cq.ln_part = c->ln_part; cq.ln_tiles = D / 64; }
                 if ((rc = gemm(c, VP_PROF_GEMM_QKV, vp::EPI_BIAS, pk[VP_PROF_GEMM_QKV], xh, b.w_qkv, b.b_qkv, c->qkv, nullptr, M, 3 * D, D, 3 * D, 0, 0, 0, &cq))) return rc;
                 if ((rc = attention(c->y, 8.0 * M * D, nullptr))) return rc;
             }
             LnFuse pp = prod; pp.reverse = (c->sw.order_mask & 2) != 0;
             if ((rc = gemm(c, VP_PROF_GEMM_PROJ, vp::EPI_BIAS_RESID_LN, pk[VP_PROF_GEMM_PROJ], c->y, b.w_proj, b.b_proj, c->x, c->x, M, D, D, D, 0, 0, 0, &pp))) return rc;
-            if ((rc = finalize(pl.fold2))) return rc;
+            if ((rc = finalize(pl.fold2 || pl.merge2))) return rc;
             LnFuse c1; c1.rowstat = c->rowstat; c1.ln_s = b.s_fc1; c1.out_blocked = c->sw.blocked_hid; c1.reverse = (c->sw.order_mask & 4) != 0;
-            if (pl.fold2) { c1.rowstat = nullptr; c1.ln_part = c->ln_part; c1.ln_tiles = D / 64; }
+            if (pl.fold2 || pl.merge2) { c1.rowstat = nullptr; c1.ln_part = c->ln_part; c1.ln_tiles = D / 64; }
             if ((rc = gemm(c, VP_PROF_GEMM_FC1, vp::EPI_BIAS_GELU, pk[VP_PROF_GEMM_FC1], xh, b.w_fc1, b.b_fc1, c->hid, nullptr, M, 4 * D, D, 4 * D, 0, 0, 0, &c1))) return rc;
             LnFuse p2 = prod; p2.a_blocked = c->sw.blocked_hid; p2.reverse = (c->sw.order_mask & 8) != 0;
             if ((rc = gemm(c, VP_PROF_GEMM_FC2, vp::EPI_BIAS_RESID_LN, pk[VP_PROF_GEMM_FC2], c->hid, fc2_w(c, b), fc2_b(c, b), c->x, c->x, M, D, 4 * D, D, 0, 0, 0, &p2))) return rc;
-            if (l + 1 < c->L && (rc = finalize(pl.fold1))) return rc;
+            if (l + 1 < c->L && (rc = finalize(pl.fold1 || pl.merge1))) return rc;
         }
     } else {
     if ((rc = gemm(c, VP_PROF_GEMM_PATCH, vp::EPI_POS, pk[VP_PROF_GEMM_PATCH], c->hid, c->w_patch, c->b_zero, c->x, c->pos, M, D, 768, D))) return rc;
diff --git a/easy_vitpose_amd/csrc/gemm8.hip b/easy_vitpose_amd/csrc/gemm8.hip
--- a/easy_vitpose_amd/csrc/gemm8.hip
+++ b/easy_vitpose_amd/csrc/gemm8.hip
@@ -227,6 +227,17 @@
                     : (VP_STAGGER(g) >= 100) ? (blockIdx.x >> 3) * (VP_STAGGER(g) - 100) : (blockIdx.x & 7) * VP_STAGGER(g);
         for (int i = 0; i < n; ++i) __builtin_amdgcn_s_sleep(16);
     }
+    constexpr int STAT_OFF = QKVA ? C::BUF + C::XH : C::RING;
+    static_assert(RESID || STAT_OFF + C::BM * 8 <= 160 * 1024, "operand ring + statistics area within the CU's LDS");
+    int stat_m0 = -1;
+    auto merge_stats = [&](int m0) {
+        if (QKVA || m0 != stat_m0) {
+            if (C::BM == 256 || tid < C::BM)
+                *(float2*)(smem + STAT_OFF + tid * 8) = ln_merge_tiles(g.ln_part + (size_t)(m0 + tid) * g.ln_tiles * 2, g.ln_tiles, g.ln_inv_d);
+            stat_m0 = m0;
+            wait_lgkm<0>();
+        }
+    };
     int t = tw.j0, m0, n0;
     tw.origin(t, g.reverse, C::BM, C::BN, m0, n0);
     set_tile(m0, n0);
@@ -265,7 +276,7 @@
 
         int frow_e = frow, fg_e = fg;
         asm volatile("" : "+v"(frow_e), "+v"(fg_e));
-        if constexpr (!DRAIN) { if (!wr) bar(); }
+        if constexpr (!DRAIN && RESID) { if (!wr) bar(); }
         if constexpr (QKVA) {
             constexpr int HD = 80, QSTR = HD * 2, VSUB = 192 * 32, DT = HD / 16, KS = 3;
             constexpr int Q_OFF = 160 * 1024 - 2 * 192 * QSTR - DT * VSUB, K_OFF = Q_OFF + 192 * QSTR, V_OFF = K_OFF + 192 * QSTR;
@@ -279,11 +290,20 @@
                 b4[f] = *(const f32x4*)(g.bias + nbq + (f >> 1) * 32 + (f & 1) * 4);
                 s4[f] = *(const f32x4*)(g.ln_s + nbq + (f >> 1) * 32 + (f & 1) * 4);
             }
-#pragma unroll
-            for (int J = 0; J < TJ; ++J) st[J] = *(const float2*)(g.rowstat + 2 * (size_t)(mrow + rowJ(J)));
+            static_assert(STAT_OFF + C::BM * 8 <= Q_OFF, "the statistics area ends in front of Q");
+            if (g.ln_part) {
+                if (!wr) merge_stats(m0);
+            } else {
+#pragma unroll
+                for (int J = 0; J < TJ; ++J) st[J] = *(const float2*)(g.rowstat + 2 * (size_t)(mrow + rowJ(J)));
+            }
             wait_vm<0>();
             if (!wr) bar();
             __syncthreads();
+            if (g.ln_part) {
+#pragma unroll
+                for (int J = 0; J < TJ; ++J) st[J] = *(const float2*)(smem + STAT_OFF + (wr * (C::XR / 2) + frow_e + rowJ(J)) * 8);
+            }
             if (has_next) {
                 set_tile(nm0, nn0);
                 issue(2, 0, 0, true); issue(0, 0, 0, true); issue(3, 0, 0, true); issue(1, 0, 0, true);
@@ -492,8 +512,19 @@
                 if constexpr (LN) {
 #pragma unroll
                     for (int f = 0; f < C::TI; ++f) s4[f] = *(const f32x4*)(g.ln_s + nb + fcol(f));
-#pragma unroll
-                    for (int J = 0; J < TJ; ++J) st[J] = *(const float2*)(g.rowstat + 2 * (size_t)(mrow + rowJ(J)));
+                    if (g.ln_part) {
+                        if (!wr) merge_stats(m0);
+                    } else {
+#pragma unroll
+                        for (int J = 0; J < TJ; ++J) st[J] = *(const float2*)(g.rowstat + 2 * (size_t)(mrow + rowJ(J)));
+                    }
+                }
+                if (!wr) bar();
+                if constexpr (LN) {
+                    if (g.ln_part) {
+#pragma unroll
+                        for (int J = 0; J < TJ; ++J) st[J] = *(const float2*)(smem + STAT_OFF + (wr * (C::XR / 2) + frow_e + rowJ(J)) * 8);
+                    }
                 }
                 uint16_t* obase = g.out_blocked
                     ? (uint16_t*)g.out + (((size_t)(mrow >> 6) * (g.ldo >> 6) + (nb >> 6)) << 12) + ((mrow & 63) << 6) + (nb & 63)
@@ -547,7 +578,7 @@
                     }
                 }
             };
-            if (g.rowstat != nullptr) epilogue(std::true_type{});
+            if (g.rowstat != nullptr || g.ln_part != nullptr) epilogue(std::true_type{});
             else epilogue(std::false_type{});
             if (tl && lane == 0 && (wave & 3) == 0) {
                 const int ti = (t - tw.j0) / tw.nloc;
@@ -687,11 +718,13 @@
     if constexpr (EPI == EPI_BIAS_RESID_LN)
         if (a.expert) { kern = gemm8_kernel<T, EPI, C, true>; ex = 1; }
     constexpr int LDS = (EPI == EPI_QKV_ATTN) ? 160 * 1024 : (EPI == EPI_BIAS_RESID_LN && C::BN != 256) ? ((128 * (C::BN * 4 + 16) + C::BM * (C::BN / 64) * 8) > C::RING ? (128 * (C::BN * 4 + 16) + C::BM * (C::BN / 64) * 8) : C::RING) : C::RING;
+    constexpr int LN_STAT_BYTES = (EPI == EPI_BIAS || EPI == EPI_BIAS_GELU) ? C::BM * 8 : 0;
+    static_assert(LDS + LN_STAT_BYTES <= 160 * 1024, "operand ring + statistics area within the CU's LDS");
     static bool attr_done[2][64] = {};
     int dev = 0;
     (void)hipGetDevice(&dev);
     if (dev < 0 || dev >= 64 || !attr_done[ex][dev]) {
-        hipError_t e = hipFuncSetAttribute((const void*)kern, hipFuncAttributeMaxDynamicSharedMemorySize, LDS);
+        hipError_t e = hipFuncSetAttribute((const void*)kern, hipFuncAttributeMaxDynamicSharedMemorySize, LDS + LN_STAT_BYTES);
         if (e != hipSuccess) return e;
         if (dev >= 0 && dev < 64) attr_done[ex][dev] = true;
     }
@@ -704,7 +737,7 @@
     if (grid >= 256) grid &= ~7;
     if (grid < 8) return hipErrorInvalidValue;
     if (a.desc) snprintf(a.desc, a.desc_cap, "gemm8_kernel<%s, %d, G8<%d, %d>%s>", std::is_same<T, F16>::value ? "F16" : "BF16", EPI, C::BN, C::BM, ex ? ", true" : "");
-    hipLaunchKernelGGL(kern, dim3(grid), dim3(C::NT), LDS, s, a);
+    hipLaunchKernelGGL(kern, dim3(grid), dim3(C::NT), LDS + (a.ln_part ? LN_STAT_BYTES : 0), s, a);
     return hipGetLastError();
 }
 
@@ -725,9 +758,10 @@
 
 bool gemm8_supported(int epi, const GemmArgs& a, int bn, int bm) {
     if (!gemm8_shape_ok(epi, a.M, a.N, a.K, a.ldo, a.w_rows, bn, bm)) return false;
-    if (epi == EPI_QKV_ATTN) return a.rowstat && a.ln_s && !a.a_blocked && !a.out_blocked && !a.reverse;
+    const bool part_ok = !a.ln_part || (a.ln_s && a.ln_tiles * 64 == a.K);
+    if (epi == EPI_QKV_ATTN) return (a.rowstat || a.ln_part) && part_ok && a.ln_s && !a.a_blocked && !a.out_blocked && !a.reverse;
     if (epi == EPI_BIAS_RESID_LN) return a.plane && a.stats_out && !a.out_blocked;
-    return true;
+    return part_ok;
 }
 
 hipError_t gemm8_launch(int dtype, int epi, const GemmArgs& a, int bn, hipStream_t s, int bm) {
diff --git a/easy_vitpose_amd/csrc/gemm8_common.h b/easy_vitpose_amd/csrc/gemm8_common.h
--- a/easy_vitpose_amd/csrc/gemm8_common.h
+++ b/easy_vitpose_amd/csrc/gemm8_common.h
@@ -43,6 +43,29 @@
     return x;
 }
 
+__device__ __forceinline__ float2 ln_merge_tiles(const float* __restrict__ src, int tiles, float inv_d) {
+    float mean = 0.f, rstd = 1.f;
+    switch (tiles) {
+        case 6: ln_merge_row<6>(src, inv_d, mean, rstd); break;
+        case 12: ln_merge_row<12>(src, inv_d, mean, rstd); break;
+        case 16: ln_merge_row<16>(src, inv_d, mean, rstd); break;
+        case 20: ln_merge_row<20>(src, inv_d, mean, rstd); break;
+        default: ln_merge(src, tiles, inv_d, mean, rstd);
+    }
+    return float2{mean, rstd};
+}
+
+__device__ __forceinline__ void ln_merge_tiles2(const float* __restrict__ src_a, const float* __restrict__ src_b, int tiles, float inv_d, float2& a, float2& b) {
+    a = b = float2{0.f, 1.f};
+    switch (tiles) {
+        case 6: ln_merge_row<6>(src_a, inv_d, a.x, a.y); ln_merge_row<6>(src_b, inv_d, b.x, b.y); break;
+        case 12: ln_merge_row<12>(src_a, inv_d, a.x, a.y); ln_merge_row<12>(src_b, inv_d, b.x, b.y); break;
+        case 16: ln_merge_row<16>(src_a, inv_d, a.x, a.y); ln_merge_row<16>(src_b, inv_d, b.x, b.y); break;
+        case 20: ln_merge_row<20>(src_a, inv_d, a.x, a.y); ln_merge_row<20>(src_b, inv_d, b.x, b.y); break;
+        default: ln_merge(src_a, tiles, inv_d, a.x, a.y); ln_merge(src_b, tiles, inv_d, b.x, b.y);
+    }
+}
+
 struct TileWalk {
     int tiles_m, tiles_n, group_m, base, cnt, j0, nloc;
     __device__ __forceinline__ void init(const GemmArgs& g, int BM, int BN) {
diff --git a/easy_vitpose_amd/csrc/handle.hip b/easy_vitpose_amd/csrc/handle.hip
--- a/easy_vitpose_amd/csrc/handle.hip
+++ b/easy_vitpose_amd/csrc/handle.hip
@@ -84,6 +84,7 @@
     if (const char* f = getenv("VP_CALLER_STREAM")) s.caller_stream_max_n = atoi(f) == 1 ? 16 : atoi(f);
     on("VP_FUSE_HEAD", s.fuse_head);
     if (const char* f = getenv("VP_FOLD_STATS")) { s.graph_max_n_stats = atoi(f); s.fold_rule = false; }
+    on("VP_MERGE_STATS", s.merge_stats);
     on("VP_BLOCKED_QKV", s.blocked_qkv);
     on("VP_FUSE_QKV_ATTN", s.fuse_qkv_attn);
     s.qa_min_set = getenv("VP_QA_MIN_TILES") != nullptr;
diff --git a/easy_vitpose_amd/csrc/kernels.h b/easy_vitpose_amd/csrc/kernels.h
--- a/easy_vitpose_amd/csrc/kernels.h
+++ b/easy_vitpose_amd/csrc/kernels.h
@@ -106,6 +106,9 @@
     const float* bh;
     const float* sh;
     const float* rowstat;
+    const float* ln_part;
+    int ln_tiles;
+    float ln_inv_d;
     uint16_t* y;
     int npairs, heads, D;
     int ncrops;
diff --git a/easy_vitpose_amd/csrc/qkvattn.hip b/easy_vitpose_amd/csrc/qkvattn.hip
--- a/easy_vitpose_amd/csrc/qkvattn.hip
+++ b/easy_vitpose_amd/csrc/qkvattn.hip
@@ -16,6 +16,8 @@
     static constexpr int VSUB = 192 * 32;
     static constexpr int V_BASE = 4 * XS;
     static_assert(6 * XS == RING && BUF <= 3 * XS && BUF + XS <= 4 * XS, "the attention phase reuses exactly the ring; buffer 0 + X0 of buffer 1 inside Q0 K0 Q1 K1");
+    static constexpr int STAT_OFF = RING, STAT_BYTES = 384 * 8;
+    static_assert(RING + STAT_BYTES <= 160 * 1024, "operand ring + statistics area within the CU's LDS");
 };
 
 __device__ __forceinline__ u32x2 lds_read_tr16(const char* p) {
@@ -195,8 +197,22 @@
         }
         const bool twin = 2 * pair + 1 >= g.ncrops;
         const float* rs0 = g.rowstat + 2 * ((size_t)pair * 384 + wr * 96 + frow_e);
-#pragma unroll
-        for (int j = 0; j < 6; ++j) stat[j] = *(const float2*)(rs0 + 32 * j);
+        if (g.ln_part) {
+            if (!wr) {
+                float2* area = (float2*)(smem + QA::STAT_OFF);
+                const float* p0 = g.ln_part + (size_t)pair * 384 * g.ln_tiles * 2;
+                const int r0 = tid, r1 = 256 + (tid & 127);
+                const int s0 = (twin && r0 >= 192) ? r0 - 192 : r0, s1 = twin ? r1 - 192 : r1;
+                float2 ma, mb;
+                ln_merge_tiles2(p0 + (size_t)s0 * g.ln_tiles * 2, p0 + (size_t)s1 * g.ln_tiles * 2, g.ln_tiles, g.ln_inv_d, ma, mb);
+                area[r0] = ma;
+                area[r1] = mb;
+                wait_lgkm<0>();
+            }
+        } else {
+#pragma unroll
+            for (int j = 0; j < 6; ++j) stat[j] = *(const float2*)(rs0 + 32 * j);
+        }
         wait_vm<0>();
         if (!wr) bar();
         __syncthreads();
@@ -208,13 +224,19 @@
             const int v_sub = 2 * (wc >> 1) + (fg_e & 1);
             const int v_byte = ((wc & 1) * 2 + (fg_e >> 1)) * 8;
             (void)dcol;
-#pragma unroll
-            for (int j = 6; j < 12; ++j) stat[j] = *(const float2*)(rs0 + (twin ? 0 : 384) + 32 * (j - 6));
+            auto hand_over = [&](auto Mc) {
+            constexpr bool MERGED = decltype(Mc)::value;
+            if constexpr (!MERGED) {
+#pragma unroll
+                for (int j = 6; j < 12; ++j) stat[j] = *(const float2*)(rs0 + (twin ? 0 : 384) + 32 * (j - 6));
+            }
 #pragma unroll
             for (int j = 0; j < 12; ++j) {
                 const int crop = j / 6;
                 const int row = wr * 96 + (j % 6) * 16 + frow_e;
-                const float2 st = stat[j];
+                float2 st;
+                if constexpr (MERGED) st = *(const float2*)(smem + QA::STAT_OFF + (crop * 192 + row) * 8);
+                else st = stat[j];
                 char* cb_ = smem + crop * 2 * QA::XS;
                 const int rsw = (row >> 1) & 7;
 #pragma unroll
@@ -227,6 +249,9 @@
                     else *(u32x2*)(smem + QA::V_BASE + crop * QA::XS + v_sub * QA::VSUB + row * 32 + v_byte) = o;
                 }
             }
+            };
+            if (g.ln_part) hand_over(std::true_type{});
+            else hand_over(std::false_type{});
         }
         __syncthreads();
 
@@ -385,12 +410,13 @@
 
 bool qkvattn_supported(const QkvAttnArgs& a) {
     if (a.D % 128 || a.D < 256 || a.heads * 64 != a.D || a.npairs <= 0 || (a.ncrops != 2 * a.npairs && a.ncrops != 2 * a.npairs - 1)) return false;
+    if (a.ln_part && a.ln_tiles * 64 != a.D) return false;
     if ((size_t)a.npairs * 384 * a.D * 2 >= (1ull << 32)) return false;
     return a.npairs * a.heads >= 8;
 }
 
 hipError_t qkvattn_launch(int dtype, const QkvAttnArgs& a, hipStream_t s, char* desc, int desc_cap) {
-    if (!qkvattn_supported(a)) return hipErrorInvalidValue;
+    if (!qkvattn_supported(a) || (!a.rowstat && !a.ln_part)) return hipErrorInvalidValue;
     const int tiles = a.npairs * a.heads;
     const int grid = tiles < 256 ? tiles : 256;
     static bool attr_done[2][64] = {};
@@ -399,12 +425,12 @@
     const int di = dtype == DT_F16 ? 0 : 1;
     auto kern = dtype == DT_F16 ? qkvattn_kernel<F16> : qkvattn_kernel<BF16>;
     if (dev < 0 || dev >= 64 || !attr_done[di][dev]) {
-        hipError_t e = hipFuncSetAttribute((const void*)kern, hipFuncAttributeMaxDynamicSharedMemorySize, QA::RING);
+        hipError_t e = hipFuncSetAttribute((const void*)kern, hipFuncAttributeMaxDynamicSharedMemorySize, QA::RING + QA::STAT_BYTES);
         if (e != hipSuccess) return e;
         if (dev >= 0 && dev < 64) attr_done[di][dev] = true;
     }
     if (desc) snprintf(desc, desc_cap, "qkvattn_kernel<%s>", dtype == DT_F16 ? "F16" : "BF16");
-    hipLaunchKernelGGL(kern, dim3(grid), dim3(QA::NT), QA::RING, s, a);
+    hipLaunchKernelGGL(kern, dim3(grid), dim3(QA::NT), QA::RING + (a.ln_part ? QA::STAT_BYTES : 0), s, a);
     return hipGetLastError();
 }
 
diff --git a/easy_vitpose_amd/csrc/tile_rules.hip b/easy_vitpose_amd/csrc/tile_rules.hip
--- a/easy_vitpose_amd/csrc/tile_rules.hip
+++ b/easy_vitpose_amd/csrc/tile_rules.hip
@@ -260,6 +260,9 @@
     }
     p.gemm[VP_PROF_GEMM_QKV] = gemm(VP_PROF_GEMM_QKV, vp::EPI_BIAS, 3 * D, D, p.fold1);
     p.gemm[VP_PROF_GEMM_FC1] = gemm(VP_PROF_GEMM_FC1, vp::EPI_BIAS_GELU, 4 * D, D, p.fold2);
+    const bool merge_ok = n > 64 && s.fold_rule && s.merge_stats;
+    p.merge1 = merge_ok && !p.fold1 && (p.qkv_path != QKV_GEMM || is_gemm8(p.gemm[VP_PROF_GEMM_QKV].variant));
+    p.merge2 = merge_ok && !p.fold2 && is_gemm8(p.gemm[VP_PROF_GEMM_FC1].variant);
     return p;
 }
 
@@ -295,6 +298,17 @@
     return (int)v.size();
 }
 
+VP_API int vp_dbg_chunk_merge(const vp_config* cfg, int32_t n, int32_t* out) {
+    if (!cfg || cfg->embed_dim <= 0 || cfg->num_heads <= 0 || cfg->embed_dim % cfg->num_heads || cfg->num_keypoints <= 0 || cfg->max_batch <= 0 ||
+        n <= 0 || n > cfg->max_batch || !out)
+        return VP_ERR_INVALID;
+    Switches s;
+    read_switches(s);
+    const ChunkPlan p = plan_chunk(s, cfg->embed_dim, cfg->num_heads, cfg->max_batch, cfg->dtype == VP_DTYPE_FP8, n, final_rows((size_t)cfg->num_keypoints));
+    out[0] = p.merge1;
+    out[1] = p.merge2;
+    return VP_OK;
+}
 
 VP_API int vp_dbg_gemm8_pick(int32_t M, int32_t N, int32_t wide, int32_t bm192_mask, int32_t* tiles) {
     if (M <= 0 || N <= 0) return VP_ERR_INVALID;
diff --git a/include/vitpose_hip.h b/include/vitpose_hip.h
--- a/include/vitpose_hip.h
+++ b/include/vitpose_hip.h
@@ -198,6 +198,11 @@
 VP_API int vp_dbg_run_batch(int32_t n, int32_t D, int32_t limit);
 VP_API int vp_dbg_expert_tile(int32_t variant, int32_t M, int32_t N, int32_t gemm8_ok, const int32_t* bounds, int32_t n_bounds);
 VP_API int vp_dbg_chunk_plan(const vp_config* cfg, int32_t n, int32_t* out, int32_t cap);
+VP_API int vp_dbg_chunk_merge(const vp_config* cfg, int32_t n, int32_t* out);
+VP_API int vp_dbg_gemm8_stats(int32_t device_id, int32_t dtype, int32_t epi, int32_t variant, int32_t group_m, int32_t M, int32_t N, int32_t K, const float* A,
+                              const float* W, const float* bias, const float* ln_s, const float* partials, int32_t merged, float* out);
+VP_API int vp_dbg_qkvattn_stats(int32_t device_id, int32_t dtype, int32_t ncrops, int32_t D, int32_t heads, const float* x, const float* W, const float* bias,
+                                const float* ln_s, const float* partials, int32_t merged, float* out);
 VP_API int vp_dbg_group_trace(int32_t n, int32_t w, int32_t maxb, int32_t* trace, int32_t cap);
 VP_API int vp_dbg_fp8_gemm(int32_t device_id, int32_t M, int32_t N, int32_t K, const float* A, const float* a_scale, const float* W,
                            const float* w_scale, float* out, uint8_t* a_codes, uint8_t* w_codes);
```

Measured after the change: 25600 persons/s. No clear change (-0.8%).
